# nanleij/ClusteredLowRankSolver.jl

Hardware: AMD Instinct MI355X
Metric: interior-point iterations/sec (higher is better)
Workload: dtype f64x5 (multi-word fp64: 5 limbs per number, ~262 bits; problem data f64x5); 1 GPU; SpherePacking cohnelkies(8,15): d=8, 2d=30; 2 clusters P=32, blocks 16x16 r1 + 1x1 dense, N=31; whole interior-point iterations with the reference's default options at its precision (prec=256 -> 5 limbs), 55 per solve; clusters=2, n_free=31, limbs=5, data_limbs=5, multi_gpu=single GPU

## Files before the change

### clusteredlowranksolver.jl_amd/csrc/clrs_hip.hip

```cpp
#include <hip/hip_runtime.h>

#include <algorithm>
#include <array>
#include <climits>
#include <cmath>
#include <cstdio>
#include <cstdlib>
#include <cstring>
#include <map>
#include <memory>
#include <string>
#include <vector>

#include "../../include/clrs_hip.h"
#include "clrs_kernels.hip.h"
#include "clrs_fused.hip.h"
#include "clrs_assemble_w3.hip.h"
#include "clrs_assemble_w4.hip.h"
#include "clrs_assemble_w5.hip.h"
#include "clrs_solve_small.hip.h"
#include "clrs_factor_small.hip.h"
#include "clrs_ipm.hip.h"

using namespace clrs;
typedef long long i64;

static thread_local std::string g_last_error;
static int fail(int code, const std::string &msg) {
    g_last_error = msg;
    return code;
}
extern "C" void clrs_set_last_error(const char *msg) { g_last_error = msg ? msg : ""; }
#define HIPCHECK(expr)                                                                                   \
    do {                                                                                                 \
        hipError_t e_ = (expr);                                                                          \
        if (e_ != hipSuccess)                                                                            \
            return fail(CLRS_ERR_HIP, std::string(#expr) + ": " + hipGetErrorString(e_));                \
    } while (0)

static const int INFO_NONE = 0x7f7f7f7f;

static int g_cfg_fused_assemble = 1;
static int g_cfg_split_blocks = 1;
static int g_cfg_fused_factor = 1;
static int g_cfg_wave_assemble = 1;
static int g_cfg_wave2_assemble = 1;
static int g_cfg_wave5_assemble = 1;
static int g_cfg_wave4_assemble = 1;
static int g_cfg_wave3_assemble = 1;
static int g_cfg_dense_block = 1;
static int g_cfg_trsm_blockinv = 1;
static int g_cfg_potrf_levels = 1;
static int g_cfg_pairing_tri = 1;
static int g_cfg_factor_aug = 1;
static int g_cfg_dense_wave = 1;
static int g_cfg_factor_small = 1;
static int g_cfg_solve_small_max = 32768;
static int g_cfg_ipm_wmfma = 3;
int g_cfg_mw_stream_words = 1;
int g_cfg_mw_pipeline64 = 1;
int g_cfg_mw_zt_small_maxn = 64;
int g_cfg_modp_minors_chunk_bytes = 0;
int g_cfg_zz_gemm_chunk_bytes = 0;
int g_cfg_liftm_chunk_bytes = 0;
int g_cfg_lrsys_chunk_bytes = 0;
int g_cfg_mw_zi_narrow = 1;
int g_cfg_mw_xinv_product = 1;
int g_cfg_mw_chain_hop = 1;
int g_cfg_mw_y_riders = 1;
int g_cfg_mw_skip_xfb = 1;
int g_cfg_mw_pipeline_x = 1;
int g_cfg_mw_pipeline_x_min = 24;
int g_cfg_mw_sharded_factor_limbs = 1;
int g_cfg_mw_pipeline = 1;
int g_cfg_mw_refine_predictor = 0;
int g_cfg_mw_refine = 1;
int g_cfg_mw_affine_corrector = 1;
int g_cfg_mw_factor_limbs = 0;
int g_cfg_mw_exact_products = 1;
static int g_cfg_solve_small2 = 1;
static const int LDS_BUDGET_DOUBLES = 20000;

enum StepKind { STEP_MEMCPY, STEP_GEMM, STEP_TRSM, STEP_POTRF, STEP_GATHER_S, STEP_GATHER_SCALAR, STEP_SUB, STEP_MEMSET_INFO, STEP_ZERO_UPPER, STEP_FUSED_ASSEMBLE, STEP_SMALL_POTRF, STEP_CLUSTER_FACTOR, STEP_GEMV_T, STEP_CSOLVE_FWD, STEP_Q_SOLVE, STEP_CSOLVE_BWD, STEP_SUM_SLABS, STEP_ASSEMBLE_W1, STEP_GRAM_SMALL, STEP_ASSEMBLE_W2, STEP_SOLVE_SMALL, STEP_DENSE_BLOCK, STEP_ASSEMBLE_W3, STEP_FACTOR_SMALL, STEP_SUM_S_SLABS, STEP_TRTRI32, STEP_DENSE_T32, STEP_TRTRI_DIAG, STEP_COPY2D, STEP_CHOL_LEVEL, STEP_CHOL_PACK, STEP_CHOL_UNPACK, STEP_ASSEMBLE_W4, STEP_ASSEMBLE_W5, STEP_NKINDS };
static const char *const STEP_NAMES[STEP_NKINDS] = {"hipMemcpyAsync(D2D)", "k_gemm_f64_t", "k_trsm_diag", "k_potrf_diag", "k_schur_gather",
                                                    "k_gather_scalar", "k_sub", "hipMemsetAsync", "k_zero_upper", "k_cluster_assemble", "k_small_potrf", "k_cluster_factor", "k_gemv_t",
                                                    "k_cluster_solve_fwd", "k_q_solve", "k_cluster_solve_bwd", "k_sum_slabs", "k_cluster_assemble_w1", "k_gram_small", "k_cluster_assemble_w2", "k_solve_small", "k_dense_block", "k_cluster_assemble_w3", "k_factor_small", "k_sum_S_slabs", "k_trtri32", "k_dense_T32", "k_trtri_diag", "k_copy2d", "k_chol_level", "k_chol_pack", "k_chol_unpack", "k_cluster_assemble_w4", "k_cluster_assemble_w5"};
static const int KT_MAX_EVENTS = 8192;

struct Step {
    StepKind kind;
    int grid = 0;
    void *d0 = nullptr, *d1 = nullptr, *d2 = nullptr;
    void *dst = nullptr;
    const void *src = nullptr;
    size_t bytes = 0;
    i64 n = 0;
    int nmax = 0;
    int aux0 = 0, aux1 = 0;
    bool s_inverse = false;
};

struct Plan {
    std::vector<Step> steps;
    hipGraphExec_t graph = nullptr;
    const void *captured[8] = {nullptr, nullptr, nullptr, nullptr, nullptr, nullptr, nullptr, nullptr};
    int launches() const { return (int)steps.size(); }
};

struct DeviceArena {
    char *base = nullptr;
    size_t size = 0, used = 0;
};

struct TrsmJob {
    const double *L;
    int ldl, n;
    double *B;
    int ldb, nrhs;
};
struct PotrfJob {
    double *A;
    int lda, n, code;
    int stop = 0;
};

struct BlockInfo {
    int j = 0, m = 1, delta = 1, n = 1, kind = 0;
    i64 xyoff = 0, t0 = 0, t1 = 0, d0 = 0, d1 = 0;
    std::vector<int> UR, UL, offR, offL;
    int URt = 0, ULt = 0;
    bool sym = false;
    bool sd_tri = false;
    i64 zr_off = -1, zl_off = -1, ty_off = -1, g_off = -1;
    int cnt = 0;
    i64 w_off = -1, tt_off = -1, sd_off = -1;
    int *d_tptr = nullptr;
    bool fused = false;
};

struct IpmState;

struct clrs_ctx {
    int device = 0;
    int *h_info = nullptr;
    char *pin = nullptr;
    size_t pin_cap = 0, pin_used = 0, pin_demand = 0;
    struct PinOut { void *user; const void *pinned; size_t bytes; };
    std::vector<PinOut> pin_out;
    IpmState *ipm = nullptr;
    std::vector<int> h_term_p, h_dense_p;
    std::vector<double> h_term_lambda;
    int *d_ayL = nullptr, *d_ayR = nullptr;
    hipStream_t stream = nullptr;
    bool own_stream = true;
    int kt_kind = -2;
    std::vector<hipEvent_t> kt_ev;
    std::vector<int> kt_kinds;
    double kt_total[STEP_NKINDS] = {0};
    long long kt_count[STEP_NKINDS] = {0};
    int J = 0, N = 0, NB = 0;
    i64 T = 0, D = 0;
    std::vector<int> P;
    std::vector<i64> coff, Soff;
    i64 xylen = 0, xlen = 0, Slen = 0;
    std::vector<BlockInfo> blk;
    std::vector<void *> allocs;
    std::vector<CholLevelJob> chol_jobs;
    std::map<const double *, std::pair<double *, double *>> s_inv;
    std::vector<std::pair<i64, double *>> trsm_y_pool;
    bool s_inv_valid = false;
    std::vector<CholAugDesc> chol_aug;
    double *d_Xc = nullptr, *d_Y = nullptr;
    double *d_static = nullptr, *d_work = nullptr;
    i64 solve_arena_len = 0;
    double *d_TY = nullptr, *d_G = nullptr, *d_TT = nullptr, *d_Sd = nullptr;
    double *d_S = nullptr, *d_B = nullptr, *d_LB = nullptr, *d_Q = nullptr;
    double *d_t = nullptr, *d_u = nullptr, *d_dy = nullptr, *d_rhsy = nullptr, *d_dx = nullptr, *d_rhsx = nullptr;
    double *d_AY = nullptr;
    i64 *d_ayidx = nullptr;
    int *d_info = nullptr;
    double *d_X = nullptr;
    Plan p_assemble, p_cholS, p_linvB, p_Q, p_cholQ, p_fwd, p_bwd, p_cholX;
    FTables ftables = {};
    W3Tables w3tables = {};
    W4Tables w4tables = {};
    W5Tables w5tables = {};
    CSolve8 solve8 = {};
    struct SolveSmall2 {
        StageJobs jobs = {};
        int rx_job[16] = {0, 0, 0, 0, 0, 0, 0, 0, 0, 0, 0, 0, 0, 0, 0, 0}, ry_job[2] = {-1, -1};
        bool ok = false;
    } ss2[3];
    Plan p_fwd_small, p_bwd_small;
    Plan p_factor_small;
    FSmallArgs fsmall = {};
    StageJobs fsmall_jobs = {};
    const double *bind_X = nullptr, *bind_rhsx = nullptr, *bind_rhsy = nullptr;
    double *bind_Xchol = nullptr, *bind_dx = nullptr, *bind_dy = nullptr;
    double *d_dinvS = nullptr, *d_dinvQ = nullptr, *d_Qslabs = nullptr;
    bool q_slabs = false;
    Plan p_cholQ_slabs, p_solve_all;
    bool fused_fs = false, fused_q = false, fused_x = false, all_assemble_fused = false;
    bool factored = false, assembled = false, local_factored = false;
    bool timing = false, graph_mode = false;
    hipEvent_t ev[10] = {nullptr, nullptr, nullptr, nullptr, nullptr, nullptr, nullptr, nullptr, nullptr, nullptr};
    double times[6] = {0, 0, 0, 0, 0, 0};
    bool times_pending = false, solve_time_pending = false;
    double cnt_bytes = 0, cnt_flops = 0, cnt_factor_flops = 0, cnt_solve_flops = 0;
    std::vector<char> cluster_fused;
    int n_fused_clusters = 0, n_wave_clusters = 0, n_wave2_clusters = 0, n_wave4_clusters = 0, n_wave5_clusters = 0;
    std::vector<int> host_UR, host_UL;
    std::vector<i64> host_U_off;
};

template <class T>
static int upload(clrs_ctx *c, const std::vector<T> &h, T **d) {
    *d = nullptr;
    size_t bytes = std::max<size_t>(h.size(), 1) * sizeof(T);
    HIPCHECK(hipMalloc((void **)d, bytes));
    c->allocs.push_back(*d);
// ... 950 lines not shown
    if (c->N > 0 && (rc = d2h_staged(c, dy, c->d_dy, sizeof(double) * c->N))) return rc;
    return d2h_finish(c);
}

extern "C" int clrs_cholesky_blocks_dev(clrs_ctx *c, const double *d_X, double *d_Xchol) {
    if (!c || !d_X || !d_Xchol) return fail(CLRS_ERR_INVALID, "null argument");
    HIPCHECK(hipSetDevice(c->device));
    if (c->fused_x) {
        c->bind_X = d_X; c->bind_Xchol = d_Xchol;
        return run_plan(c, c->p_cholX);
    }
    if (d_X != c->d_X) HIPCHECK(hipMemcpyAsync(c->d_X, d_X, sizeof(double) * c->xylen, hipMemcpyDeviceToDevice, c->stream));
    int rc = run_plan(c, c->p_cholX);
    if (rc) return rc;
    if (d_Xchol != c->d_X) HIPCHECK(hipMemcpyAsync(d_Xchol, c->d_X, sizeof(double) * c->xylen, hipMemcpyDeviceToDevice, c->stream));
    return 0;
}

extern "C" int clrs_cholesky_blocks(clrs_ctx *c, const double *X, double *Xchol) {
    if (!c || !X || !Xchol) return fail(CLRS_ERR_INVALID, "null argument");
    HIPCHECK(hipSetDevice(c->device));
    int rc;
    pin_reset(c);
    if ((rc = h2d_staged(c, c->d_X, X, sizeof(double) * c->xylen))) return rc;
    if ((rc = clrs_cholesky_blocks_dev(c, c->d_X, c->d_X))) return rc;
    if ((rc = d2h_staged(c, Xchol, c->d_X, sizeof(double) * c->xylen))) return rc;
    int st = 0;
    if ((rc = read_info(c, &st, 1))) return rc;
    if ((rc = d2h_finish(c))) return rc;
    return st;
}

extern "C" double *clrs_q_buffer_dev(clrs_ctx *c) { return c ? c->d_Q : nullptr; }
extern "C" double *clrs_u_buffer_dev(clrs_ctx *c) { return c ? c->d_u : nullptr; }
extern "C" double *clrs_S_buffer_dev(clrs_ctx *c) { return c ? c->d_S : nullptr; }
extern "C" double *clrs_AY_buffer_dev(clrs_ctx *c) { return c ? c->d_AY : nullptr; }
extern "C" void *clrs_stream(clrs_ctx *c) { return c ? (void *)c->stream : nullptr; }

extern "C" int clrs_set_timing(clrs_ctx *c, int enabled) {
    if (!c) return fail(CLRS_ERR_INVALID, "null argument");
    c->timing = enabled != 0;
    return 0;
}
extern "C" int clrs_get_timings(clrs_ctx *c, double t[6]) {
    if (!c || !t) return fail(CLRS_ERR_INVALID, "null argument");
    HIPCHECK(hipStreamSynchronize(c->stream));
    collect_times(c);
    for (int i = 0; i < 6; i++) t[i] = c->times[i];
    return 0;
}
extern "C" int clrs_get_counters(const clrs_ctx *c, double *ab, double *af, double *ff, double *sf) {
    if (!c) return fail(CLRS_ERR_INVALID, "null argument");
    if (ab) *ab = c->cnt_bytes;
    if (af) *af = c->cnt_flops;
    if (ff) *ff = c->cnt_factor_flops;
    if (sf) *sf = c->cnt_solve_flops;
    return 0;
}
extern "C" int clrs_set_graph_mode(clrs_ctx *c, int enabled) {
    if (!c) return fail(CLRS_ERR_INVALID, "null argument");
    c->graph_mode = enabled != 0;
    return 0;
}
extern "C" int clrs_plan_info(const clrs_ctx *c, int32_t *na, int32_t *nf, int32_t *ns) {
    if (!c) return fail(CLRS_ERR_INVALID, "null argument");
    if (na) *na = c->p_assemble.launches();
    if (nf) *nf = c->p_cholS.launches() + c->p_linvB.launches() + c->p_Q.launches() + c->p_cholQ.launches();
    if (ns) *ns = c->p_fwd.launches() + c->p_bwd.launches();
    return 0;
}

extern "C" int clrs_set_stream(clrs_ctx *c, void *stream) {
    if (!c) return fail(CLRS_ERR_INVALID, "null argument");
    HIPCHECK(hipSetDevice(c->device));
    HIPCHECK(hipStreamSynchronize(c->stream));
    Plan *plans[] = {&c->p_assemble, &c->p_cholS, &c->p_linvB, &c->p_Q, &c->p_cholQ, &c->p_fwd, &c->p_bwd, &c->p_cholX, &c->p_cholQ_slabs, &c->p_solve_all, &c->p_fwd_small, &c->p_bwd_small, &c->p_factor_small};
    for (Plan *p : plans)
        if (p->graph) { hipGraphExecDestroy(p->graph); p->graph = nullptr; }
    if (c->own_stream) HIPCHECK(hipStreamDestroy(c->stream));
    c->stream = (hipStream_t)stream;
    c->own_stream = false;
    return 0;
}

static int kt_collect(clrs_ctx *c) {
    if (c->kt_kinds.empty()) return 0;
    HIPCHECK(hipStreamSynchronize(c->stream));
    for (size_t i = 0; i < c->kt_kinds.size(); i++) {
        float ms = 0;
        if (hipEventElapsedTime(&ms, c->kt_ev[2 * i], c->kt_ev[2 * i + 1]) == hipSuccess) {
            c->kt_total[c->kt_kinds[i]] += ms * 1e-3;
            c->kt_count[c->kt_kinds[i]]++;
        }
    }
    c->kt_kinds.clear();
    return 0;
}

extern "C" int clrs_set_kernel_timing(clrs_ctx *c, int kind) {
    if (!c || kind < -2 || kind >= STEP_NKINDS) return fail(CLRS_ERR_INVALID, "bad kernel kind");
    int rc = kt_collect(c);
    if (rc) return rc;
    c->kt_kind = kind;
    for (int k = 0; k < STEP_NKINDS; k++) { c->kt_total[k] = 0; c->kt_count[k] = 0; }
    return 0;
}

extern "C" int clrs_get_kernel_times(clrs_ctx *c, int max_kinds, double *seconds, int64_t *launches) {
    if (!c || !seconds || !launches) return fail(CLRS_ERR_INVALID, "null argument");
    int rc = kt_collect(c);
    if (rc) return rc;
    for (int k = 0; k < max_kinds && k < STEP_NKINDS; k++) { seconds[k] = c->kt_total[k]; launches[k] = c->kt_count[k]; }
    return STEP_NKINDS;
}

extern "C" int clrs_config_set(const char *key, int value) {
    if (!key) return fail(CLRS_ERR_INVALID, "null argument");
    if (!std::strcmp(key, "fused_assemble")) { g_cfg_fused_assemble = value; return 0; }
    if (!std::strcmp(key, "split_blocks")) { g_cfg_split_blocks = value; return 0; }
    if (!std::strcmp(key, "fused_factor")) { g_cfg_fused_factor = value; return 0; }
    if (!std::strcmp(key, "wave_assemble")) { g_cfg_wave_assemble = value; return 0; }
    if (!std::strcmp(key, "wave2_assemble")) { g_cfg_wave2_assemble = value; return 0; }
    if (!std::strcmp(key, "wave3_assemble")) { g_cfg_wave3_assemble = value; return 0; }
    if (!std::strcmp(key, "wave4_assemble")) { g_cfg_wave4_assemble = value; return 0; }
    if (!std::strcmp(key, "wave5_assemble")) { g_cfg_wave5_assemble = value; return 0; }
    if (!std::strcmp(key, "dense_block")) { g_cfg_dense_block = value; return 0; }
    if (!std::strcmp(key, "dense_wave")) { g_cfg_dense_wave = value; return 0; }
    if (!std::strcmp(key, "factor_aug")) { g_cfg_factor_aug = value; return 0; }
    if (!std::strcmp(key, "pairing_tri")) { g_cfg_pairing_tri = value; return 0; }
    if (!std::strcmp(key, "potrf_levels")) { g_cfg_potrf_levels = value; return 0; }
    if (!std::strcmp(key, "trsm_blockinv")) { g_cfg_trsm_blockinv = value; return 0; }
    if (!std::strcmp(key, "solve_small2")) { g_cfg_solve_small2 = value; return 0; }
    if (!std::strcmp(key, "factor_small")) { g_cfg_factor_small = value; return 0; }
    if (!std::strcmp(key, "pin_limit")) { PIN_LIMIT = (size_t)std::max(value, 0); return 0; }
    if (!std::strcmp(key, "ipm_wmfma")) { g_cfg_ipm_wmfma = value; return 0; }
    if (!std::strcmp(key, "solve_small_max")) { g_cfg_solve_small_max = value; return 0; }
    if (!std::strcmp(key, "mw_exact_products")) { g_cfg_mw_exact_products = value; return 0; }
    if (!std::strcmp(key, "mw_refine")) { g_cfg_mw_refine = value; return 0; }
    if (!std::strcmp(key, "mw_factor_limbs")) { g_cfg_mw_factor_limbs = value; return 0; }
    if (!std::strcmp(key, "mw_affine_corrector")) { g_cfg_mw_affine_corrector = value; return 0; }
    if (!std::strcmp(key, "mw_pipeline")) { g_cfg_mw_pipeline = value; return 0; }
    if (!std::strcmp(key, "mw_pipeline64")) { g_cfg_mw_pipeline64 = value; return 0; }
    if (!std::strcmp(key, "mw_zt_small_maxn")) { g_cfg_mw_zt_small_maxn = value; return 0; }
    if (!std::strcmp(key, "mw_pipeline_x")) { g_cfg_mw_pipeline_x = value; return 0; }
    if (!std::strcmp(key, "mw_pipeline_x_min")) { g_cfg_mw_pipeline_x_min = value; return 0; }
    if (!std::strcmp(key, "mw_sharded_factor_limbs")) { g_cfg_mw_sharded_factor_limbs = value; return 0; }
    if (!std::strcmp(key, "mw_stream_words")) { g_cfg_mw_stream_words = value; return 0; }
    if (!std::strcmp(key, "mw_zi_narrow")) { g_cfg_mw_zi_narrow = value; return 0; }
    if (!std::strcmp(key, "modp_minors_chunk_bytes")) { g_cfg_modp_minors_chunk_bytes = value < 0 ? 0 : value; return 0; }
    if (!std::strcmp(key, "zz_gemm_chunk_bytes")) { g_cfg_zz_gemm_chunk_bytes = value < 0 ? 0 : value; return 0; }
    if (!std::strcmp(key, "liftm_chunk_bytes")) { g_cfg_liftm_chunk_bytes = value < 0 ? 0 : value; return 0; }
    if (!std::strcmp(key, "lrsys_chunk_bytes")) { g_cfg_lrsys_chunk_bytes = value < 0 ? 0 : value; return 0; }
    if (!std::strcmp(key, "mw_xinv_product")) { g_cfg_mw_xinv_product = value; return 0; }
    if (!std::strcmp(key, "mw_chain_hop")) { g_cfg_mw_chain_hop = value; return 0; }
    if (!std::strcmp(key, "mw_skip_xfb")) { g_cfg_mw_skip_xfb = value; return 0; }
    if (!std::strcmp(key, "mw_y_riders")) { g_cfg_mw_y_riders = value; return 0; }
    if (!std::strcmp(key, "mw_refine_predictor")) { g_cfg_mw_refine_predictor = value; return 0; }
    return fail(CLRS_ERR_INVALID, std::string("unknown configuration key ") + key);
}

#ifdef CLRS_W3_STAMPS
extern "C" int clrs_debug_cf_stamps(clrs_ctx *c, uint64_t out[16]) {
    if (!c || !out) return fail(CLRS_ERR_INVALID, "null argument");
    HIPCHECK(hipStreamSynchronize(c->stream));
    HIPCHECK(hipMemcpyFromSymbol(out, HIP_SYMBOL(g_cf_stamps), 16 * sizeof(uint64_t)));
    return 0;
}
extern "C" int clrs_debug_ss2_stamps(clrs_ctx *c, uint64_t out[16]) {
    if (!c || !out) return fail(CLRS_ERR_INVALID, "null argument");
    HIPCHECK(hipStreamSynchronize(c->stream));
    HIPCHECK(hipMemcpyFromSymbol(out, HIP_SYMBOL(g_ss2_stamps), 16 * sizeof(uint64_t)));
    return 0;
}
extern "C" int clrs_debug_w3_stamps(clrs_ctx *c, uint64_t out[16]) {
    if (!c || !out) return fail(CLRS_ERR_INVALID, "null argument");
    HIPCHECK(hipStreamSynchronize(c->stream));
    HIPCHECK(hipMemcpyFromSymbol(out, HIP_SYMBOL(g_w3_stamps), 16 * sizeof(uint64_t)));
    return 0;
}
#endif

extern "C" int clrs_debug_stamps(clrs_ctx *c, uint64_t out[64]) {
    if (!c || !out) return fail(CLRS_ERR_INVALID, "null argument");
    if (!c->ftables.stamps) { std::memset(out, 0, 64 * sizeof(uint64_t)); return 0; }
    HIPCHECK(hipStreamSynchronize(c->stream));
    HIPCHECK(hipMemcpy(out, c->ftables.stamps, 64 * sizeof(uint64_t), hipMemcpyDeviceToHost));
    return 0;
}

extern "C" int clrs_fused_clusters(const clrs_ctx *c) { return c ? c->n_fused_clusters : 0; }
extern "C" int clrs_wave_clusters(const clrs_ctx *c) { return c ? c->n_wave_clusters + c->n_wave2_clusters : 0; }
extern "C" int clrs_wave2_clusters(const clrs_ctx *c) { return c ? c->n_wave2_clusters : 0; }
extern "C" int clrs_wave4_clusters(const clrs_ctx *c) { return c ? c->n_wave4_clusters : 0; }
extern "C" int clrs_wave5_clusters(const clrs_ctx *c) { return c ? c->n_wave5_clusters : 0; }

extern "C" const char *clrs_kernel_name(int kind) { return (kind >= 0 && kind < STEP_NKINDS) ? STEP_NAMES[kind] : ""; }

extern "C" const char *clrs_strerror(int code) {
    switch (code) {
        case CLRS_OK: return "ok";
        case CLRS_ERR_INVALID: return "invalid argument or malformed SDP description";
        case CLRS_ERR_HIP: return "HIP runtime error";
        case CLRS_ERR_NO_DEVICE: return "no usable HIP device";
        case CLRS_ERR_STATE: return "call order violated";
        default: return code > 0 ? "factorisation failure (non-positive pivot)" : "unknown error";
    }
}
extern "C" const char *clrs_last_error(void) { return g_last_error.c_str(); }
extern "C" const char *clrs_version(void) { return "clrs-hip 0.1.0 (gfx950)"; }

#include "clrs_ipm_host.inc"

static CtxOwner mini_ctx(int device) {
    CtxOwner c(new clrs_ctx(), clrs_ctx_destroy);
    c->device = device;
    if (hipSetDevice(device) != hipSuccess || hipStreamCreateWithFlags(&c->stream, hipStreamNonBlocking) != hipSuccess) c.reset();
    if (!c) return c;
    (void)hipFuncSetAttribute((const void *)k_gemm_f64_t<128, 128, 0, 0>, hipFuncAttributeMaxDynamicSharedMemorySize, (int)gemm_lds_bytes(128, 128));
    (void)hipFuncSetAttribute((const void *)k_gemm_f64_t<128, 128, 0, 1>, hipFuncAttributeMaxDynamicSharedMemorySize, (int)gemm_lds_bytes(128, 128));
    (void)hipFuncSetAttribute((const void *)k_gemm_f64_t<128, 128, 1, 0>, hipFuncAttributeMaxDynamicSharedMemorySize, (int)gemm_lds_bytes(128, 128));
    (void)hipFuncSetAttribute((const void *)k_gemm_f64_t<128, 128, 1, 1>, hipFuncAttributeMaxDynamicSharedMemorySize, (int)gemm_lds_bytes(128, 128));
    std::vector<int> hi(1, INFO_NONE);
    if (upload(c.get(), hi, &c->d_info)) c.reset();
    return c;
}

extern "C" int clrs_test_gemm(int device, int ta, int tb, int M, int N, int K, double alpha, const double *A, int lda, const double *B,
                              int ldb, double beta, double *C, int ldc) {
    const CtxOwner own = mini_ctx(device);
    clrs_ctx *c = own.get();
    if (!c) return fail(CLRS_ERR_NO_DEVICE, "no device");
    int rc = 0;
    i64 na = (i64)lda * (ta ? M : K), nb = (i64)ldb * (tb ? K : N), nc = (i64)ldc * N;
    std::vector<double> hA(A, A + na), hB(B, B + nb), hC(C, C + nc);
    double *dA, *dB, *dC;
    if ((rc = upload(c, hA, &dA)) || (rc = upload(c, hB, &dB)) || (rc = upload(c, hC, &dC))) return rc;
    Plan pl;
    std::vector<GemmDesc> g;
    g.push_back(mk_gemm(ta, tb, M, N, K, alpha, dA, lda, dB, ldb, beta, dC, ldc));
    if (!(rc = add_gemm_stage(c, pl, g)) && !(rc = run_steps(c, pl))) {
        if (hipStreamSynchronize(c->stream) != hipSuccess || hipMemcpy(C, dC, sizeof(double) * nc, hipMemcpyDeviceToHost) != hipSuccess)
            rc = fail(CLRS_ERR_HIP, "copy back failed");
    }
    return rc;
}

extern "C" int clrs_test_potrf(int device, int n, double *A, int lda) {
    const CtxOwner own = mini_ctx(device);
    clrs_ctx *c = own.get();
    if (!c) return fail(CLRS_ERR_NO_DEVICE, "no device");
    int rc = 0, st = 0;
    std::vector<double> hA(A, A + (i64)lda * n);
    double *dA;
    if ((rc = upload(c, hA, &dA))) return rc;
    Plan pl;
    std::vector<PotrfJob> pj;
    pj.push_back(PotrfJob{dA, lda, n, 1});
    if (!(rc = plan_potrf(c, pl, pj)) && !(rc = run_steps(c, pl)) && !(rc = read_info(c, &st))) {
        if (hipMemcpy(A, dA, sizeof(double) * (i64)lda * n, hipMemcpyDeviceToHost) != hipSuccess) rc = fail(CLRS_ERR_HIP, "copy back failed");
    }
    return rc ? rc : st;
}

typedef double v2d_stream __attribute__((ext_vector_type(2)));
__global__ __launch_bounds__(256) void k_stream_probe(const v2d_stream *__restrict__ a, const v2d_stream *__restrict__ b, v2d_stream *__restrict__ w,
                                                      long long nr, long long nw) {
    const long long stride = (long long)gridDim.x * 256, n = nr > nw ? nr : nw;
    for (long long i = (long long)blockIdx.x * 256 + threadIdx.x; i < n; i += 4 * stride) {
        v2d_stream x[4], y[4];
#pragma unroll
        for (int u = 0; u < 4; u++) {
            const long long k = i + u * stride;
            x[u] = y[u] = (v2d_stream){0.0, 0.0};
            if (k < nr) { x[u] = a[k]; y[u] = b[k]; }
        }
#pragma unroll
        for (int u = 0; u < 4; u++) {
            const long long k = i + u * stride;
            if (k < nw) __builtin_nontemporal_store(x[u] + y[u], w + k);
        }
    }
}

extern "C" int clrs_test_stream(int device, long long read_bytes, long long write_bytes, int reps, double *avg_us) {
    if (read_bytes < 32 || write_bytes < 16 || reps < 1 || !avg_us) return fail(CLRS_ERR_INVALID, "clrs_test_stream: bad arguments");
    if (hipSetDevice(device) != hipSuccess) return fail(CLRS_ERR_NO_DEVICE, "no device");
    const long long nr = read_bytes / 32, nw = write_bytes / 16;
    v2d_stream *a = nullptr, *b = nullptr, *w = nullptr;
    hipEvent_t e0 = nullptr, e1 = nullptr;
    hipStream_t st = nullptr;
    int rc = 0;
    auto ok = [&](hipError_t e, const char *what) { if (e != hipSuccess && !rc) rc = fail(CLRS_ERR_HIP, std::string(what) + ": " + hipGetErrorString(e)); return e == hipSuccess; };
    if (ok(hipMalloc(&a, nr * 16), "hipMalloc") && ok(hipMalloc(&b, nr * 16), "hipMalloc") && ok(hipMalloc(&w, nw * 16), "hipMalloc") &&
        ok(hipMemset(a, 0, nr * 16), "hipMemset") && ok(hipMemset(b, 0, nr * 16), "hipMemset") && ok(hipMemset(w, 0, nw * 16), "hipMemset") &&
        ok(hipStreamSynchronize(nullptr), "hipStreamSynchronize") &&
        ok(hipStreamCreateWithFlags(&st, hipStreamNonBlocking), "hipStreamCreate") && ok(hipEventCreate(&e0), "hipEventCreate") && ok(hipEventCreate(&e1), "hipEventCreate")) {
        hipDeviceProp_t prop;
        int cus = 256;
        if (hipGetDeviceProperties(&prop, device) == hipSuccess) cus = prop.multiProcessorCount;
        const int grid = 2 * cus;
        for (int r = 0; r < 3; r++) hipLaunchKernelGGL(k_stream_probe, dim3(grid), dim3(256), 0, st, a, b, w, nr, nw);
        ok(hipEventRecord(e0, st), "hipEventRecord");
        for (int r = 0; r < reps; r++) hipLaunchKernelGGL(k_stream_probe, dim3(grid), dim3(256), 0, st, a, b, w, nr, nw);
        ok(hipEventRecord(e1, st), "hipEventRecord");
        ok(hipEventSynchronize(e1), "hipEventSynchronize");
        float ms = 0.f;
// ... 29 lines not shown
```

### clusteredlowranksolver.jl_amd/csrc/clrs_mw.hip

```cpp
#include <hip/hip_runtime.h>

#include <dlfcn.h>

#include <algorithm>
#include <condition_variable>
#include <cstdio>
#include <cstring>
#include <memory>
#include <mutex>
#include <string>
#include <vector>

#include "../../include/clrs_hip.h"
#include "clrs_mw_kernels.hip.h"
#include "clrs_mw_pipe.hip.h"
#include "clrs_mw_exact.hip.h"
#include "clrs_mw_ipm.hip.h"
#include "clrs_mw_rank.hip.h"
#include "clrs_mw_gemm.hip.h"
#include "clrs_mw_kernel_vectors.hip.h"
#include "clrs_mw_rational.hip.h"
#include "clrs_mw_inst.h"
#include "clrs_mw_tables.h"
#ifdef MW_SPLIT_UNITS
MW_KERNELS_ALL(extern template, 4)
MW_KERNELS_ALL(extern template, 5)
MW_KERNELS_ALL(extern template, 6)
MW_KERNELS_ALL(extern template, 8)
MW_KERNELS_ALL(extern template, 10)
#endif

typedef long long i64;

extern int g_cfg_mw_zi_narrow;
extern int g_cfg_mw_xinv_product;
extern int g_cfg_mw_chain_hop, g_cfg_mw_skip_xfb, g_cfg_mw_y_riders;
extern int g_cfg_mw_stream_words;
extern int g_cfg_mw_pipeline64;
extern int g_cfg_mw_zt_small_maxn;
extern int g_cfg_mw_pipeline_x, g_cfg_mw_pipeline_x_min;
extern int g_cfg_mw_sharded_factor_limbs;
extern int g_cfg_mw_pipeline;
extern int g_cfg_mw_refine_predictor;
extern int g_cfg_mw_refine;
extern int g_cfg_mw_exact_products;
extern int g_cfg_mw_affine_corrector;
extern int g_cfg_mw_factor_limbs;
extern "C" void clrs_set_last_error(const char *msg);

static int mw_fail(int code, const std::string &msg) {
    clrs_set_last_error(msg.c_str());
    return code;
}
#define MWCHECK(expr)                                                                                    \
    do {                                                                                                 \
        hipError_t e_ = (expr);                                                                          \
        if (e_ != hipSuccess) return mw_fail(CLRS_ERR_HIP, std::string(#expr) + ": " + hipGetErrorString(e_)); \
    } while (0)

typedef struct { char internal[128]; } mw_nccl_id;
struct MwNccl {
    void *lib = nullptr;
    int (*GetUniqueId)(mw_nccl_id *) = nullptr;
    int (*CommInitRank)(void **, int, mw_nccl_id, int) = nullptr;
    int (*CommDestroy)(void *) = nullptr;
    int (*AllGather)(const void *, void *, size_t, int, void *, hipStream_t) = nullptr;
    const char *(*GetErrorString)(int) = nullptr;
};
static MwNccl g_nccl;
static int mw_nccl_load() {
    if (g_nccl.lib) return 0;
    const char *names[] = {"librccl.so.1", "librccl.so", "/opt/rocm/lib/librccl.so.1"};
    void *h = nullptr;
    for (const char *n : names) if ((h = dlopen(n, RTLD_NOW | RTLD_NOLOAD))) break;
    for (const char *n : names) { if (h) break; h = dlopen(n, RTLD_NOW | RTLD_GLOBAL); }
    if (!h) return mw_fail(CLRS_ERR_INVALID, std::string("RCCL is not available: ") + dlerror());
    g_nccl.GetUniqueId = (int (*)(mw_nccl_id *))dlsym(h, "ncclGetUniqueId");
    g_nccl.CommInitRank = (int (*)(void **, int, mw_nccl_id, int))dlsym(h, "ncclCommInitRank");
    g_nccl.CommDestroy = (int (*)(void *))dlsym(h, "ncclCommDestroy");
    g_nccl.AllGather = (int (*)(const void *, void *, size_t, int, void *, hipStream_t))dlsym(h, "ncclAllGather");
    g_nccl.GetErrorString = (const char *(*)(int))dlsym(h, "ncclGetErrorString");
    if (!g_nccl.GetUniqueId || !g_nccl.CommInitRank || !g_nccl.CommDestroy || !g_nccl.AllGather) return mw_fail(CLRS_ERR_INVALID, "RCCL symbols missing");
    g_nccl.lib = h;
    return 0;
}
#define NCCLCHECK(expr)                                                                                                          \
    do {                                                                                                                         \
        int r_ = (expr);                                                                                                         \
        if (r_ != 0) return mw_fail(CLRS_ERR_HIP, std::string(#expr) + ": " + (g_nccl.GetErrorString ? g_nccl.GetErrorString(r_) : "RCCL error")); \
    } while (0)
static const int MW_NCCL_FLOAT64 = 8;

struct clrs_mw_local_group {
    int world = 0;
    int attached = 0;
    std::mutex m;
    std::condition_variable cv;
    struct Chan {
        int arrived = 0;
        long gen = 0;
        std::vector<double *> base;
        std::vector<hipEvent_t> ready, copied;
    } ch[2];
    void barrier(int k) {
        std::unique_lock<std::mutex> lk(m);
        Chan &c = ch[k];
        const long g = c.gen;
        if (++c.arrived == world) { c.arrived = 0; c.gen++; cv.notify_all(); }
        else cv.wait(lk, [&] { return c.gen != g; });
    }
};

static const size_t MW_LDS_MAX = 160 * 1024 - 2048;

struct clrs_mw_ctx {
    int device = 0, K = 4, DK = 1;
    hipStream_t stream = nullptr;
    bool own_stream = true;
    MwDev d = {};
    std::vector<MwBlk> blk;
    std::vector<MwClu> clu;
    std::vector<void *> allocs;
    int maxU = 0, maxP = 0, maxn = 0, maxn_dense = 0;
    bool all_inv = false;
    bool xinv_valid = false;
    bool lds_x = false, lds_q = false, lds_zt_L = false, dense_two = false;
    int nw_factor = 1;
    int maxcnt = 0;
    double *vz = nullptr;
    bool wide_solve = false;
    const double *ride_fwd = nullptr;
    const int *ride_wait = nullptr;
    int ride_wait_value = 0;
    bool fwd_rode = false;
    int n_one_term = 0, n_many_term = 0;
    int sa_lanes = MW_SA_W;
    int maxTb = 0;
    size_t sm_x = 0, sm_zt = 0, sm_dense = 0, sm_factor = 0, sm_q = 0, sm_fwd = 0, sm_mid = 0, sm_bwd = 0;
    int *h_info = nullptr;
    double *d_Xin = nullptr, *d_Xc = nullptr, *d_Y = nullptr, *d_rx = nullptr, *d_ry = nullptr, *d_dx = nullptr, *d_dy = nullptr;
    bool assembled = false, factored = false;
    bool timing = false;
    hipEvent_t ev[8] = {nullptr, nullptr, nullptr, nullptr, nullptr, nullptr, nullptr, nullptr};
    double times[6] = {0, 0, 0, 0, 0, 0};
    double cnt_mul = 0;
    double cnt_factor = 0, cnt_solve = 0;
    struct MwIpm *ipm = nullptr;
    size_t sm_bp_diag = 0, sm_bp_panel = 0, sm_bp_inv = 0;
    std::vector<MwBp> bp_S, bp_Q;
    const MwBp *d_bp = nullptr;
    bool any_lds_cluster = false;
    void *comm = nullptr;
    void *comm_side = nullptr;
    clrs_mw_local_group *lgroup = nullptr;
    bool local_factored = false, fwd_done = false;
    const double *split_rhs_x = nullptr;
    bool refine_ready = false;
    MwdDev mwd = {};
    int mwd_blocks = 0, mwd_tasks = 0;
    size_t sm_mwd = 0;
    MwxDev mwx = {};
    int mwx_blocks = 0, mwx_maxU16 = 0;
    MwsDev mws = {};
    int mws_blocks = 0;
    int mws_turns = 1;
    size_t sm_mws = 0;
    bool pipe_bp = false;
    bool pipe_S64 = false;
    bool pipe_X = false;
    unsigned long long *pipe_pcx = nullptr;
    double *xpipe_L = nullptr, *xpipe_rd = nullptr;
    int *xpipe_info = nullptr;
    bool pipe_S = false, pipe_Q = false;
    unsigned long long *pipe_pc64 = nullptr;
    int pipe_pcQ = 0;
    unsigned pipe_epoch = 0;
    bool stream_words = true;
    bool y_riders = true;
    const double *ride_y = nullptr;
    bool zi_narrow = true;
    bool xinv_product = true;
    int chain_hop = 1;
    bool refine_skip_next = false;
    int refine_predictor = 0;
    int refine = 1;
    bool ipm_arms_info = false;
    int kf_low = 0, kf_entry = 0;
};

template <class T>
static int mw_upload(clrs_mw_ctx *c, const std::vector<T> &h, const T **d) {
    T *p = nullptr;
    size_t bytes = std::max<size_t>(h.size(), 1) * sizeof(T);
    MWCHECK(hipMalloc((void **)&p, bytes));
    c->allocs.push_back(p);
    if (!h.empty()) MWCHECK(hipMemcpy(p, h.data(), h.size() * sizeof(T), hipMemcpyHostToDevice));
    *d = p;
    return 0;
}
static int mw_dmalloc(clrs_mw_ctx *c, double **d, i64 n) {
    size_t bytes = (size_t)std::max<i64>(n, 1) * sizeof(double);
    MWCHECK(hipMalloc((void **)d, bytes));
    c->allocs.push_back(*d);
    MWCHECK(hipMemset(*d, 0, bytes));
    return 0;
}

#define MW_CASE(Kc, Dc, ...) if (c_K_ == Kc && c_D_ == Dc) { constexpr int KK = Kc; constexpr int DD = Dc; __VA_ARGS__; } else
#define MW_DISPATCH(ctx, ...)                                                                                       \
    do {                                                                                                            \
        const int c_K_ = (ctx)->K, c_D_ = (ctx)->DK;                                                                \
        MW_CASE(2, 1, __VA_ARGS__) MW_CASE(2, 2, __VA_ARGS__) MW_CASE(3, 1, __VA_ARGS__) MW_CASE(3, 2, __VA_ARGS__)  \
        MW_CASE(4, 1, __VA_ARGS__) MW_CASE(4, 2, __VA_ARGS__) MW_CASE(5, 1, __VA_ARGS__) MW_CASE(5, 2, __VA_ARGS__)  \
        MW_CASE(6, 1, __VA_ARGS__) MW_CASE(6, 2, __VA_ARGS__) MW_CASE(8, 1, __VA_ARGS__) MW_CASE(8, 2, __VA_ARGS__)  \
        MW_CASE(10, 1, __VA_ARGS__) MW_CASE(10, 2, __VA_ARGS__)                                                      \
        MW_CASE(3, 3, __VA_ARGS__) MW_CASE(4, 4, __VA_ARGS__) MW_CASE(5, 5, __VA_ARGS__) MW_CASE(6, 6, __VA_ARGS__)  \
        MW_CASE(8, 8, __VA_ARGS__) MW_CASE(10, 10, __VA_ARGS__)                                                      \
        return mw_fail(CLRS_ERR_INVALID, "limbs must be 2..6, 8 or 10 and data limbs 1, 2 or the limbs");           \
    } while (0)

template <class F>
static int mw_set_lds(F kernel, size_t bytes) {
    if (bytes > 48 * 1024) MWCHECK(hipFuncSetAttribute((const void *)kernel, hipFuncAttributeMaxDynamicSharedMemorySize, (int)bytes));
    return 0;
}

extern "C" void clrs_mw_destroy(clrs_mw_ctx *c);
static void mw_ipm_free(clrs_mw_ctx *c);
static int mw_launch_xrd(clrs_mw_ctx *c, const double *d_Xc);

extern "C" int clrs_mw_create_opts(const clrs_sdp_desc *d, int data_limbs, int device, int limbs, const clrs_mw_options *opts, clrs_mw_ctx **out);
extern "C" int clrs_mw_create(const clrs_sdp_desc *d, int device, int limbs, clrs_mw_ctx **out) {
    return clrs_mw_create_opts(d, 1, device, limbs, nullptr, out);
}
extern "C" int clrs_mw_create_ex(const clrs_sdp_desc *d, int data_limbs, int device, int limbs, clrs_mw_ctx **out) {
    return clrs_mw_create_opts(d, data_limbs, device, limbs, nullptr, out);
}

#define MW_RET(call) do { if (int rc_ = (call)) return rc_; } while (0)
static int mw_hip(hipError_t e, const char *what) {
    return e == hipSuccess ? 0 : mw_fail(CLRS_ERR_HIP, std::string(what) + ": " + hipGetErrorString(e));
}
template <class T>
static int mw_alloc_fill(clrs_mw_ctx *c, T **p, size_t count, int byte) {
    if (hipMalloc((void **)p, count * sizeof(T)) != hipSuccess) return mw_fail(CLRS_ERR_HIP, "hipMalloc failed");
    c->allocs.push_back(*p);
    if (hipMemset(*p, byte, count * sizeof(T)) != hipSuccess) return mw_fail(CLRS_ERR_HIP, "hipMemset failed");
    return 0;
}

struct MwOpts { int exact, refine, pipe, refine_pred, factor_limbs, km; };
static int mw_resolve_opts(const clrs_mw_options *opts, int limbs, int data_limbs, MwOpts &o) {
    o.exact = opts && opts->exact_products >= 0 ? opts->exact_products : g_cfg_mw_exact_products;
    o.refine = opts && opts->refine >= 0 ? opts->refine : g_cfg_mw_refine;
    o.pipe = opts && opts->pipeline >= 0 ? opts->pipeline : g_cfg_mw_pipeline;
    o.refine_pred = opts && opts->refine_predictor >= 0 ? opts->refine_predictor : g_cfg_mw_refine_predictor;
    o.factor_limbs = opts && opts->factor_limbs >= 0 ? opts->factor_limbs : g_cfg_mw_factor_limbs;
    o.km = opts && opts->matmul_limbs > 0 ? opts->matmul_limbs : limbs;
    if (o.km > limbs) o.km = limbs;
    while (o.km < limbs && !mw_km_ok(limbs, o.km)) o.km++;
    if (data_limbs > 2) o.exact = 0;
    if (o.km < limbs) o.exact = 0;
    if (o.exact > 2 || o.refine > 2) return mw_fail(CLRS_ERR_INVALID, "clrs_mw_options: exact_products and refine are 0, 1 or 2 (or < 0 for the default)");
    if (limbs < 2 || limbs > 10 || limbs == 7 || limbs == 9) return mw_fail(CLRS_ERR_INVALID, "limbs must be 2..6, 8 or 10");
    if (data_limbs < 1 || data_limbs > limbs || (data_limbs > 2 && data_limbs != limbs))
        return mw_fail(CLRS_ERR_INVALID, "data limbs must be 1, 2 or the context's limbs (the problem data at the working precision: src/interface.jl:1078-1112)");
    return 0;
}

static int mw_stage_stream(clrs_mw_ctx *c) {
    {
        int least = 0, greatest = 0;
        if (hipDeviceGetStreamPriorityRange(&least, &greatest) != hipSuccess) { least = greatest = 0; (void)hipGetLastError(); }
        if (hipStreamCreateWithPriority(&c->stream, hipStreamNonBlocking, greatest) != hipSuccess) return mw_fail(CLRS_ERR_HIP, "hipStreamCreateWithPriority failed");
    }
    if (hipHostMalloc((void **)&c->h_info, 2 * sizeof(int), hipHostMallocDefault) != hipSuccess) return mw_fail(CLRS_ERR_HIP, "hipHostMalloc failed");
    return 0;
}

static void mw_adopt_tables(clrs_mw_ctx *c, MwTables &t) {
    c->blk.swap(t.blk); c->clu.swap(t.clu);
    c->maxU = t.maxU; c->maxP = t.maxP; c->maxn = t.maxn; c->maxn_dense = t.maxn_dense; c->maxTb = t.maxTb; c->maxcnt = t.maxcnt;
    c->sa_lanes = t.sa_lanes; c->n_one_term = t.n_one_term; c->n_many_term = t.n_many_term;
    c->cnt_mul = t.cnt_mul; c->cnt_factor = t.cnt_factor; c->cnt_solve = t.cnt_solve;
    c->wide_solve = c->maxP > 64 || t.N > 64;
}

static int mw_stage_lds(clrs_mw_ctx *c, const MwTables &t) {
    const int K = c->K, J = t.J, N = t.N;
    const size_t lim = MW_LDS_MAX / sizeof(double);
    {
        size_t nn = (size_t)c->maxn * c->maxn * K;
        size_t bcw = MW_POTRF_SCR(K, (size_t)c->maxn);
        c->lds_x = nn + bcw <= lim;
        size_t xneed = (c->lds_x ? nn : 0) + bcw;
        for (auto &k : c->blk) {
            const size_t one = (size_t)k.n * k.n * K + MW_POTRF_SCR(K, (size_t)k.n) + (size_t)K * k.n;
            const size_t two = one + (size_t)MW_TRI(k.n) * K;
            k.inv = !c->lds_x ? 0 : two <= lim ? 1 : one <= lim ? 2 : 0;
            if (k.inv) xneed = std::max(xneed, k.inv == 1 ? two : one);
        }
        c->all_inv = !c->blk.empty();
        for (auto &k : c->blk) c->all_inv = c->all_inv && (k.kind != 0 || k.inv != 0);
        c->sm_x = xneed * 8;
        size_t zt = (size_t)c->maxn * MW_CT * K;
        c->lds_zt_L = zt + nn <= lim;
        c->sm_zt = (zt + (c->lds_zt_L ? nn : 0)) * 8;
        if (zt > lim) return mw_fail(CLRS_ERR_INVALID, "PSD block too large for the multi-word kernels");
        size_t maxnd = 0;
        for (auto &k : c->blk) if (k.kind != 0 && k.n > 1) maxnd = std::max(maxnd, (size_t)k.n);
        if (maxnd * maxnd * K > lim) return mw_fail(CLRS_ERR_INVALID, "dense block too large for the multi-word kernels");
        c->dense_two = 2 * maxnd * maxnd * K <= lim;
        c->sm_dense = (c->dense_two ? 2 : 1) * maxnd * maxnd * K * 8;
        size_t fmax = 0;
        for (auto &q : c->clu) {
            const size_t need = ((size_t)q.P * q.P + (size_t)MW_TRI(q.P)) * K + MW_POTRF_SCR(K, (size_t)q.P);
            q.lds = need <= lim ? 1 : 0;
            if (q.lds) fmax = std::max(fmax, need);
        }
        c->sm_factor = std::max<size_t>(fmax, 1) * 8;
        c->nw_factor = std::max(1, std::min(MW_INV_WG, 256 / std::max(J, 1)));
        c->sm_fwd = 2 * (size_t)c->maxP * K * 8;
        c->sm_bwd = 3 * (size_t)c->maxP * K * 8;
        const size_t qn = (size_t)N * N * K;
        const size_t qneed = qn + (size_t)MW_TRI(N) * K + MW_POTRF_SCR(K, (size_t)N);
        c->lds_q = qneed <= lim;
        c->sm_q = (c->lds_q ? qneed : 1) * 8;
        c->sm_mid = 2 * (size_t)std::max(N, 1) * K * 8;
        if (c->sm_fwd > MW_LDS_MAX || c->sm_mid > MW_LDS_MAX) return mw_fail(CLRS_ERR_INVALID, "cluster too large for the multi-word solve kernels");
    }
    MW_DISPATCH(c, {
        MW_RET(mw_set_lds(k_mw_potrf_x<KK>, c->sm_x)); MW_RET(mw_set_lds((k_mw_potrf_x_ride<KK, DD>), c->sm_x)); MW_RET(mw_set_lds(k_mw_zt<KK, DD>, c->sm_zt)); MW_RET(mw_set_lds((k_mw_dense_t<KK, DD>), c->sm_dense));
        constexpr int KC = mw_kc(KK);
        const size_t bw = std::min(c->sm_mid + c->sm_bwd, MW_LDS_MAX);
// ... 7 lines not shown

template <class DATA, class PUT>
static void mw_cut_column(int n, int DK, int S, DATA &&data, int *e_out, PUT &&put) {
    double mx = 0;
    for (int i = 0; i < n; i++) mx = std::max(mx, std::fabs(data(0, i)));
    const int e = *e_out = mwk::mws_exponent(mx);
    for (int i = 0; i < n; i++)
        mw_cut_digits(data(0, i), DK > 1 ? data(1, i) : 0.0, e, S, [&](int s, float dgt) { put(i, s, dgt); });
}

static int mw_stage_mws(clrs_mw_ctx *c, const MwTables &t, const MwOpts &o, std::vector<long long> &mws_off) {
    const int K = c->K, DK = c->DK, NB = t.NB;
    mws_off.assign((size_t)std::max(NB, 1), -1);
    const int S = mws_slices(K);
    std::vector<float> hVs;
    std::vector<int> hVe, hve_off((size_t)std::max(NB, 1), 0), hsv((size_t)std::max(NB, 1), 0);
    for (int b = 0; b < NB; b++) {
        const MwBlk &k = c->blk[b];
        if (k.kind != 0 || !k.inv || k.n > 32) continue;
        const int n = k.n, U = k.U, np = (n + 3) & ~3, n16 = (n + 15) & ~15, U16 = (U + 15) & ~15, rV = mws_rowstride(U16);
        if ((n16 / 16) * (U16 / 16) > 4 || mws_lds_bytes(S, mws_sv_class(S, 1), n, U) > MW_LDS_MAX) continue;
        if (2 * (n16 / 16) * (U16 / 16) > 4) c->mws_turns = 2;
        mws_off[b] = (long long)hVs.size();
        hve_off[b] = (int)hVe.size();
        hVs.resize(hVs.size() + (size_t)S * np * rV, 0.0f);
        hVe.resize(hVe.size() + U16, 0);
        float *dst = hVs.data() + mws_off[b];
        int sv = 0;
        for (int u = 0; u < U; u++)
            mw_cut_column(n, DK, S, [&](int l, int i) { return t.V[(size_t)l * t.Vp + k.v_off + (i64)u * n + i]; }, &hVe[hve_off[b] + u], [&](int i, int s, float dgt) {
                dst[(size_t)s * np * rV + (size_t)i * rV + mws_col(i, u, U16)] = dgt;
                if (dgt != 0.0f) sv = std::max(sv, s + 1);
            });
        if (mws_lds_bytes(S, mws_sv_class(S, sv), n, U) > MW_LDS_MAX) {
            hVs.resize((size_t)mws_off[b]); hVe.resize((size_t)hve_off[b]);
            mws_off[b] = -1;
            continue;
        }
        hsv[b] = sv;
        c->mws_blocks++;
        c->sm_mws = std::max(c->sm_mws, mws_lds_bytes(S, mws_sv_class(S, sv), n, U));
    }
    const bool on = o.exact == 2 ? c->mws_blocks > 0 : (o.exact == 1 && c->mws_blocks >= 256);
    if (!on) { c->mws_blocks = 0; std::fill(mws_off.begin(), mws_off.end(), -1); }
    else {
        MW_RET(mw_upload(c, hVs, &c->mws.Vs)); MW_RET(mw_upload(c, hVe, &c->mws.Vexp));
        MW_RET(mw_upload(c, hve_off, &c->mws.ve_off)); MW_RET(mw_upload(c, hsv, &c->mws.sv));
        MW_DISPATCH(c, { if constexpr (DD <= 2) { MW_RET(mw_set_lds((k_mws_pair<KK, DD, 1>), c->sm_mws)); MW_RET(mw_set_lds((k_mws_pair<KK, DD, 2>), c->sm_mws)); } });
    }
    return mw_upload(c, mws_off, &c->mws.vs_off);
}

static int mw_stage_mwx(clrs_mw_ctx *c, const MwTables &t, const MwOpts &o, const std::vector<long long> &mws_off) {
    const int K = c->K, DK = c->DK, NB = t.NB;
    std::vector<long long> mwx_off((size_t)std::max(NB, 1), -1);
    if (o.exact == 0) return mw_upload(c, mwx_off, &c->mwx.d_off);
    const int S = mws_slices(K);
    std::vector<float> hVd;
    std::vector<int> heV, he_off((size_t)std::max(NB, 1), 0), hsv((size_t)std::max(NB, 1), 0);
    for (int b = 0; b < NB; b++) {
        const MwBlk &k = c->blk[b];
        if (k.kind != 0 || k.m != 1 || mws_off[b] >= 0) continue;
        if (k.U < (o.exact == 2 ? 16 : 64) || k.n < 8) continue;
        const int n = k.n, U = k.U, np = (n + 3) & ~3, U16 = (U + 15) & ~15;
        mwx_off[b] = (long long)hVd.size();
        he_off[b] = (int)heV.size();
        hVd.resize(hVd.size() + (size_t)S * np * U16, 0.0f);
        heV.resize(heV.size() + U16, 0);
        float *dst = hVd.data() + mwx_off[b];
        int sv = 0;
        for (int u = 0; u < U; u++)
            mw_cut_column(n, DK, S, [&](int l, int i) { return t.V[(size_t)l * t.Vp + k.v_off + (i64)u * n + i]; }, &heV[he_off[b] + u], [&](int i, int s, float dgt) {
                dst[(size_t)s * np * U16 + (size_t)i * U16 + u] = dgt;
                if (dgt != 0.0f) sv = std::max(sv, s + 1);
            });
        hsv[b] = sv;
        c->mwx_blocks++;
        c->mwx_maxU16 = std::max(c->mwx_maxU16, U16);
    }
    if (c->mwx_blocks > 0) {
        MW_RET(mw_upload(c, hVd, &c->mwx.Vd)); MW_RET(mw_upload(c, heV, &c->mwx.eV));
        MW_RET(mw_upload(c, he_off, &c->mwx.e_off)); MW_RET(mw_upload(c, hsv, &c->mwx.sv));
        double *zd = nullptr, *td = nullptr, *ez = nullptr, *et = nullptr;
        MW_RET(mw_dmalloc(c, &zd, (i64)(hVd.size() + 1) / 2)); MW_RET(mw_dmalloc(c, &td, (i64)(hVd.size() + 1) / 2));
        MW_RET(mw_dmalloc(c, &ez, (i64)(heV.size() + 1) / 2)); MW_RET(mw_dmalloc(c, &et, (i64)(heV.size() + 1) / 2));
        c->mwx.Zd = (float *)zd; c->mwx.Td = (float *)td; c->mwx.eZ = (int *)ez; c->mwx.eT = (int *)et;
        MW_RET(mw_hip(hipMemset(zd, 0, hVd.size() * sizeof(float)), "hipMemset")); MW_RET(mw_hip(hipMemset(td, 0, hVd.size() * sizeof(float)), "hipMemset"));
        MW_RET(mw_hip(hipMemset(ez, 0, heV.size() * sizeof(int)), "hipMemset")); MW_RET(mw_hip(hipMemset(et, 0, heV.size() * sizeof(int)), "hipMemset"));
    }
    return mw_upload(c, mwx_off, &c->mwx.d_off);
}

static int mw_stage_mwd(clrs_mw_ctx *c, const MwTables &t, const MwOpts &o) {
    const int K = c->K, DK = c->DK, NB = t.NB;
    std::vector<long long> mwd_off((size_t)std::max(NB, 1), -1);
    if (o.exact == 0 || K > 6) return mw_upload(c, mwd_off, &c->mwd.a_off);
    const int S = mws_slices(K), S1 = (S + 1) / 2, sN = 32 * 32;
    std::vector<float> hAd;
    std::vector<int> heA, he_off((size_t)std::max(NB, 1), 0);
    for (int b = 0; b < NB; b++) {
        const MwBlk &k = c->blk[b];
        if (k.kind == 0 || !k.inv || k.n <= 16 || k.n > 32 || k.cnt <= 0) continue;
        const int n = k.n;
        const size_t base = hAd.size(), ebase = heA.size();
        hAd.resize(base + (size_t)k.cnt * S1 * sN, 0.0f);
        heA.resize(ebase + (size_t)k.cnt * 32, 0);
        bool fits = true;
        for (int e = 0; e < k.cnt && fits; e++) {
            float *dst = hAd.data() + base + (size_t)e * S1 * sN;
            const i64 a0 = k.a_off + (i64)e * n * n;
            for (int col = 0; col < n; col++)
                mw_cut_column(n, DK, S, [&](int l, int kk) { return t.dA[(size_t)l * t.dAp + a0 + kk + (i64)col * n]; }, &heA[ebase + (size_t)e * 32 + col], [&](int kk, int s, float dgt) {
                    if (s < S1) dst[(size_t)s * sN + (size_t)kk * 32 + mws_col(kk, col, 32)] = dgt;
                    else if (dgt != 0.0f) fits = false;
                });
        }
        if (!fits) { hAd.resize(base); heA.resize(ebase); continue; }
        mwd_off[b] = (long long)base;
        he_off[b] = (int)ebase;
        c->mwd_blocks++;
    }
    if (c->mwd_blocks > 0) {
        std::vector<int> tasks;
        for (size_t di = 0; di < t.dn_list.size(); di++) {
            const int b = t.dn_list[di];
            if (mwd_off[b] < 0) continue;
            for (int e = 0; e < c->blk[b].cnt; e++) { tasks.push_back((int)di); tasks.push_back(e); }
        }
        c->mwd_tasks = (int)tasks.size() / 2;
        MW_RET(mw_upload(c, tasks, &c->mwd.tasks));
        MW_RET(mw_upload(c, hAd, &c->mwd.Ad)); MW_RET(mw_upload(c, heA, &c->mwd.eA)); MW_RET(mw_upload(c, he_off, &c->mwd.e_off));
        c->sm_mwd = (size_t)2 * S * sN * sizeof(float) + 128 * sizeof(int);
        MW_DISPATCH(c, { if constexpr (DD <= 2) { MW_RET(mw_set_lds((k_mwx_dense<KK, DD>), c->sm_mwd)); } });
    }
    return mw_upload(c, mwd_off, &c->mwd.a_off);
}

static int mw_stage_upload(clrs_mw_ctx *c, const MwTables &t) {
    MwDev &q = c->d;
    q.mws_off = c->mws.vs_off; q.mws_on = c->mws_blocks > 0 ? 1 : 0;
    q.mwx_off = c->mwx.d_off; q.mwx_on = c->mwx_blocks > 0 ? 1 : 0;
    q.mwd_off = c->mwd.a_off; q.mwd_on = 0;
    q.J = t.J; q.N = t.N; q.NB = t.NB; q.nlr = (int)t.lr_list.size(); q.ndn = (int)t.dn_list.size();
    q.xylen = t.xylen; q.xlen = t.xlen; q.Slen = t.Slen; q.T = t.T; q.xrdlen = t.xrdlen;
    q.zlen = std::max<i64>(t.zlen, 1); q.glen = std::max<i64>(t.glen, 1); q.wlen = std::max<i64>(t.wlen, 1); q.sdlen = std::max<i64>(t.sdlen, 1);
    q.Vp = t.Vp; q.dAp = t.dAp; q.lamp = t.lamp; q.Bp = t.Bp;
    MW_RET(mw_upload(c, c->blk, &q.blk)); MW_RET(mw_upload(c, c->clu, &q.clu));
    MW_RET(mw_upload(c, t.lr_list, &q.lr_list)); MW_RET(mw_upload(c, t.dn_list, &q.dn_list));
    MW_RET(mw_upload(c, t.V, &q.V)); MW_RET(mw_upload(c, t.vrow, &q.vrow));
    MW_RET(mw_upload(c, t.st_a, &q.st_a)); MW_RET(mw_upload(c, t.st_b, &q.st_b)); MW_RET(mw_upload(c, t.st_lam, &q.st_lam));
    MW_RET(mw_upload(c, t.tptr, &q.tptr));
    MW_RET(mw_upload(c, t.st_orig, &q.st_orig)); MW_RET(mw_upload(c, t.st_p, &q.st_p)); MW_RET(mw_upload(c, t.st_war, &q.st_war)); MW_RET(mw_upload(c, t.st_wac, &q.st_wac));
    MW_RET(mw_upload(c, t.st_trl, &q.st_trl)); MW_RET(mw_upload(c, t.st_trd, &q.st_trd)); MW_RET(mw_upload(c, t.st_flag, &q.st_flag));
    MW_RET(mw_upload(c, t.ay_a, &q.ay_a)); MW_RET(mw_upload(c, t.ay_b, &q.ay_b)); MW_RET(mw_upload(c, t.ay_blk, &q.ay_blk));
    MW_RET(mw_upload(c, t.dA, &q.dA)); MW_RET(mw_upload(c, t.dmap, &q.dmap)); MW_RET(mw_upload(c, t.dense_p, &q.dense_p));
    MW_RET(mw_upload(c, t.drow_ptr, &q.drow_ptr)); MW_RET(mw_upload(c, t.drow_blk, &q.drow_blk)); MW_RET(mw_upload(c, t.drow_en, &q.drow_en));
    q.dn_big = t.dn_big;
    q.maxcnt = c->maxcnt;
    return mw_upload(c, t.B, &q.B);
}

static int mw_stage_buffers(clrs_mw_ctx *c) {
    MwDev &q = c->d;
    const int K = c->K, J = q.J, N = q.N;
    const i64 xlen = q.xlen, Slen = q.Slen, xyoff = q.xylen, rdoff = q.xrdlen, T = q.T;
    MW_RET(mw_dmalloc(c, &q.Z, q.zlen * K)); MW_RET(mw_dmalloc(c, &q.Tm, q.zlen * K));
    MW_RET(mw_dmalloc(c, &q.GX, q.glen * K)); MW_RET(mw_dmalloc(c, &q.GY, q.glen * K));
    MW_RET(mw_dmalloc(c, &q.W, q.wlen * K)); MW_RET(mw_dmalloc(c, &q.Sd, q.sdlen * K));
    MW_RET(mw_dmalloc(c, &q.S, Slen * K)); MW_RET(mw_dmalloc(c, &q.LB, xlen * (i64)N * K)); MW_RET(mw_dmalloc(c, &q.Q, (i64)N * N * K));
    MW_RET(mw_dmalloc(c, &q.Si, Slen * K)); MW_RET(mw_dmalloc(c, &q.Qi, (i64)N * N * K));

    MW_RET(mw_dmalloc(c, &q.Xf, xyoff * K)); MW_RET(mw_dmalloc(c, &q.Xb, xyoff * K)); MW_RET(mw_dmalloc(c, &q.Xi, xyoff * K));
    MW_RET(mw_dmalloc(c, &q.xrd, rdoff * K)); MW_RET(mw_dmalloc(c, &q.srd, xlen * K)); MW_RET(mw_dmalloc(c, &q.qrd, (i64)N * K));
    MW_RET(mw_dmalloc(c, &q.t, xlen * K)); MW_RET(mw_dmalloc(c, &q.u, (i64)J * N * K)); MW_RET(mw_dmalloc(c, &q.AY, T * K));
    q.AX = nullptr;
    q.aff_mu = q.aff_rhs = q.aff_t = q.aff_u = nullptr; q.aff_wait = nullptr; q.ride2_rhs = nullptr; q.ride2_t = q.ride2_u = nullptr;
    MW_RET(mw_dmalloc(c, &c->vz, 2 * (i64)N * K));
    MW_RET(mw_dmalloc(c, &q.S0, Slen * K)); MW_RET(mw_dmalloc(c, &q.ub, (i64)J * N * K));
    MW_RET(mw_dmalloc(c, &q.rx2, xlen * K)); MW_RET(mw_dmalloc(c, &q.dx2, xlen * K));
    MW_RET(mw_dmalloc(c, &q.u2, (i64)N * K)); MW_RET(mw_dmalloc(c, &q.dy2, (i64)N * K));
    q.uadd = nullptr;
    MW_RET(mw_dmalloc(c, &c->d_Xin, xyoff * K)); MW_RET(mw_dmalloc(c, &c->d_Xc, xyoff * K)); MW_RET(mw_dmalloc(c, &c->d_Y, xyoff * K));
    MW_RET(mw_dmalloc(c, &c->d_rx, xlen * K)); MW_RET(mw_dmalloc(c, &c->d_dx, xlen * K));
    MW_RET(mw_dmalloc(c, &c->d_ry, (i64)N * K)); MW_RET(mw_dmalloc(c, &c->d_dy, (i64)N * K));
    int *info = nullptr;
    MW_RET(mw_hip(hipMalloc((void **)&info, 2 * sizeof(int)), "hipMalloc"));
    c->allocs.push_back(info);
    q.info = info;
    int init[2] = {MW_INFO_NONE, MW_INFO_NONE};
    MW_RET(mw_hip(hipMemcpy(info, init, sizeof(init), hipMemcpyHostToDevice), "hipMemcpy"));
    return mw_alloc_fill(c, &q.pcnt, (size_t)(2 * J + 3), 0);
}

static int mw_stage_blocked(clrs_mw_ctx *c) {
    MwDev &q = c->d;
    const int K = c->K, J = q.J, N = q.N;
    for (int j = 0; j < J; j++) {
        const MwClu &cl = c->clu[j];
        if (cl.lds) { c->any_lds_cluster = true; continue; }
        c->bp_S.push_back(MwBp{q.S + cl.Soff, q.Si + cl.Soff, q.srd + cl.coff, q.Slen, q.xlen, cl.P, cl.P, j + 1, 0, (int)c->bp_S.size(), 0});
    }
    if (N > 0) c->bp_Q.push_back(MwBp{q.Q, q.Qi, q.qrd, (i64)N * N, (i64)N, N, N, J + 1, 0, (int)c->bp_S.size(), 0});
    std::vector<MwBp> all = c->bp_S;
    all.insert(all.end(), c->bp_Q.begin(), c->bp_Q.end());
    MW_RET(mw_upload(c, all, &c->d_bp));
    const int MW_PB = MW_PB_OF(K);
    c->sm_bp_diag = ((size_t)MW_POTRF_SCR(K, MW_PB) + (size_t)K * MW_PB * MW_PB + (size_t)K * MW_TRI(MW_PB) + (size_t)K * MW_PB) * 8;
    c->sm_bp_panel = (size_t)K * MW_BP_PR * MW_PB * 8;
    c->sm_bp_inv = (size_t)K * MW_PB * MW_BP_IC * 8;
    MW_DISPATCH(c, { MW_RET(mw_set_lds(k_mw_bp_diag<KK>, std::max(c->sm_bp_diag, c->sm_factor))); MW_RET(mw_set_lds(k_mw_bp_panel<KK>, c->sm_bp_panel)); MW_RET(mw_set_lds(k_mw_bp_inv<KK>, c->sm_bp_inv)); MW_RET(mw_set_lds(k_mw_bp_inv_row<KK>, c->sm_bp_inv)); });
    return 0;
}

static int mw_stage_pipelines(clrs_mw_ctx *c, const MwOpts &o) {
    MwDev &q = c->d;
    const int K = c->K, J = q.J, N = q.N, cfg_pipe = o.pipe;
    bool small = c->maxP <= MWP_N;
    for (auto &cl : c->clu) small = small && cl.lds;
    c->pipe_S = cfg_pipe != 0 && (K <= 6 || cfg_pipe >= 2) && small && (i64)J * ((MWP_N / MWP_W) + MWP_WW) <= 256;
    c->pipe_Q = (cfg_pipe >= 2 || (cfg_pipe == 1 && K <= 6 && N > MWP_W)) && N > 0 && N <= MWP_N;
    bool lds_all = !c->clu.empty();
    for (auto &cl : c->clu) lds_all = lds_all && cl.lds;
    c->pipe_S64 = cfg_pipe != 0 && K <= 6 && lds_all && c->maxP > MWP_N && c->maxP <= MWP_N64 && (i64)J * 16 <= 256 && g_cfg_mw_pipeline64 != 0 &&
                  (cfg_pipe >= 2 || c->maxP >= 48);
    const size_t nbp = c->bp_S.size() + c->bp_Q.size();
    const bool any_bp = !c->bp_S.empty() || (N > 0 && !c->lds_q);
    c->pipe_bp = cfg_pipe != 0 && any_bp && (i64)std::max<size_t>(c->bp_S.size(), 1) * ((MWP_N / MWP_W) + MWP_WW) <= 256;
    q.pipe_pc = nullptr;
    q.pipe_stamps = nullptr;
    q.pipe_bp = 0;
    {
        bool all_inv = c->d.NB > 0 && c->lds_x;
        int maxn_x = 0;
        i64 working = 0;
        for (auto &kb : c->blk) {
            all_inv = all_inv && kb.inv == 1;
            maxn_x = std::max(maxn_x, kb.n);
            working += 2 * ((kb.n + MWP_W - 1) / MWP_W + (kb.n > MWP_N ? MWP_N64 / MWP_W : MWP_WW));
        }
        q.no_xfb = (all_inv && (!q.dn_big || c->dense_two) && g_cfg_mw_skip_xfb != 0) ? 1 : 0;
        c->pipe_X = cfg_pipe != 0 && K <= 6 && all_inv && maxn_x <= MWP_N64 && g_cfg_mw_pipeline_x != 0 &&
                    (cfg_pipe >= 2 || (maxn_x >= g_cfg_mw_pipeline_x_min && working <= 256));
        if (c->pipe_X) {
            double *pcx = nullptr, *ti = nullptr;
            MW_RET(mw_dmalloc(c, &pcx, (i64)2 * c->d.NB * MWP_PC_WORDS_N(K, MWP_N64)));
            c->pipe_pcx = (unsigned long long *)pcx;
            MW_RET(mw_dmalloc(c, &c->xpipe_L, c->d.xylen * K));
            MW_RET(mw_dmalloc(c, &c->xpipe_rd, c->d.xrdlen * K));
            MW_RET(mw_dmalloc(c, &ti, c->d.NB + 1));
            c->xpipe_info = (int *)ti;
            MW_DISPATCH(c, { if constexpr (KK <= 6) { MW_RET(mw_set_lds(k_mw_potrf_x_pipe<KK>, MWP_LDS_ALONE64)); } });
        }
    }
    if (c->pipe_S64) {
        MW_RET(mw_alloc_fill(c, &c->pipe_pc64, (size_t)J * MWP_PC_WORDS_N(K, MWP_N64), 0xff));
        MW_DISPATCH(c, { if constexpr (KK <= 6) { MW_RET(mw_set_lds(k_mw_factor_pipe64<KK>, MWP_LDS_ALONE64)); } });
    }
    if (c->pipe_S || c->pipe_Q || c->pipe_bp) {
        const size_t own = (size_t)(c->pipe_S ? J : 0) + 1;
        MW_RET(mw_alloc_fill(c, &q.pipe_pc, (own + (c->pipe_bp ? nbp : 0)) * MWP_PC_WORDS(K), 0xff));
        c->pipe_pcQ = c->pipe_S ? J : 0;
        q.pipe_q = c->pipe_pcQ;
        q.pipe_bp = (int)own;
        MW_DISPATCH(c, {
            MW_RET(mw_set_lds(k_mw_factor_pipe<KK>, MWP_LDS_ALONE));
            MW_RET(mw_set_lds(k_mw_potrf_q_pipe<KK>, std::max<size_t>(MWP_LDS_ALONE, c->sm_fwd)));
            MW_RET(mw_set_lds(k_mw_bp_diag_pipe<KK>, std::max<size_t>(MWP_LDS_ALONE, c->sm_factor)));
        });
    }
    return 0;
}

static int mw_stage_reduced_limbs(clrs_mw_ctx *c, const MwOpts &o) {
    MwDev &q = c->d;
    const int K = c->K, N = q.N;
    q.rank = 0; q.world = 1; q.gathered = 0;
    MW_RET(mw_dmalloc(c, &q.Qg, (i64)N * N * K)); MW_RET(mw_dmalloc(c, &q.ug, (i64)N * K));
    const bool may = mw_kf_of(K) < K && c->refine == 1;
    c->kf_low = may ? mw_kf_of(K) : K;
    if (o.factor_limbs != 0 && o.factor_limbs != K && o.factor_limbs != c->kf_low) return mw_fail(CLRS_ERR_INVALID, "factor_limbs: 0 (automatic), the context's limbs, or the reduced count of this limb count where the LDS-resident refined solve runs");
    if (o.factor_limbs == K) c->kf_low = K;
    c->kf_entry = o.factor_limbs == 0 ? K : o.factor_limbs;
    q.kf = c->kf_entry;
    q.km = o.km;
    return mw_alloc_fill(c, &q.refstat, 4, 0);
}

extern "C" int clrs_mw_create_opts(const clrs_sdp_desc *d, int data_limbs, int device, int limbs, const clrs_mw_options *opts, clrs_mw_ctx **out) {
    if (!d || !out) return mw_fail(CLRS_ERR_INVALID, "null argument");
    MwOpts o;
    MW_RET(mw_resolve_opts(opts, limbs, data_limbs, o));
    *out = nullptr;
    int ndev = 0;
    if (hipGetDeviceCount(&ndev) != hipSuccess || ndev <= 0 || device >= ndev) return mw_fail(CLRS_ERR_NO_DEVICE, "no usable HIP device");
    MW_RET(mw_hip(hipSetDevice(device), "hipSetDevice(device)"));
    if (d->n_clusters <= 0 || d->n_free < 0 || d->n_blocks < 0) return mw_fail(CLRS_ERR_INVALID, "bad sizes");
    std::unique_ptr<clrs_mw_ctx, void (*)(clrs_mw_ctx *)> guard(new clrs_mw_ctx(), clrs_mw_destroy);
    clrs_mw_ctx *c = guard.get();
    c->device = device;
    c->K = limbs;
    c->DK = data_limbs;
    c->refine = o.refine;
    c->refine_predictor = o.refine_pred;
    {
        const char *e = std::getenv("CLRS_MW_STREAM_WORDS");
        c->stream_words = e && *e ? std::atoi(e) != 0 : g_cfg_mw_stream_words != 0;
        c->chain_hop = std::min(std::max(g_cfg_mw_chain_hop, 0), 2);
        c->y_riders = g_cfg_mw_y_riders != 0;
        c->zi_narrow = g_cfg_mw_zi_narrow != 0;
        c->xinv_product = g_cfg_mw_xinv_product != 0;
    }
    MW_RET(mw_stage_stream(c));
    MwTables t;
    std::string err;
    if (mw_build_tables(d, data_limbs, t, err)) return mw_fail(CLRS_ERR_INVALID, err);
    mw_adopt_tables(c, t);
    MW_RET(mw_stage_lds(c, t));
    std::vector<long long> mws_off;
    MW_RET(mw_stage_mws(c, t, o, mws_off));
    MW_RET(mw_stage_mwx(c, t, o, mws_off));
    MW_RET(mw_stage_mwd(c, t, o));
    MW_RET(mw_stage_upload(c, t));
    MW_RET(mw_stage_buffers(c));
    MW_RET(mw_stage_blocked(c));
    MW_RET(mw_stage_pipelines(c, o));
    MW_RET(mw_stage_reduced_limbs(c, o));
    for (auto &e : c->ev) MW_RET(mw_hip(hipEventCreate(&e), "hipEventCreate(&e)"));
    *out = guard.release();
    return 0;
}
#undef MW_RET

extern "C" void clrs_mw_destroy(clrs_mw_ctx *c) {
    if (!c) return;
    (void)hipSetDevice(c->device);
    if (c->stream) (void)hipStreamSynchronize(c->stream);
    mw_ipm_free(c);
    if (c->comm && g_nccl.CommDestroy) { (void)g_nccl.CommDestroy(c->comm); c->comm = nullptr; }
    if (c->comm_side && g_nccl.CommDestroy) { (void)g_nccl.CommDestroy(c->comm_side); c->comm_side = nullptr; }
    if (c->lgroup) { std::lock_guard<std::mutex> lk(c->lgroup->m); c->lgroup->attached--; c->lgroup = nullptr; }
    for (void *p : c->allocs) (void)hipFree(p);
    for (auto &e : c->ev) if (e) (void)hipEventDestroy(e);
    if (c->h_info) (void)hipHostFree(c->h_info);
    if (c->stream && c->own_stream) (void)hipStreamDestroy(c->stream);
    delete c;
}

extern "C" int clrs_mw_limbs(const clrs_mw_ctx *c) { return c ? c->K : 0; }
extern "C" void *clrs_mw_stream(clrs_mw_ctx *c) { return c ? (void *)c->stream : nullptr; }
extern "C" int clrs_mw_set_stream(clrs_mw_ctx *c, void *stream) {
    if (!c) return mw_fail(CLRS_ERR_INVALID, "null context");
    if (c->own_stream && c->stream) { (void)hipStreamSynchronize(c->stream); (void)hipStreamDestroy(c->stream); }
    c->stream = (hipStream_t)stream;
    c->own_stream = false;
    return 0;
}
extern "C" int clrs_mw_get_dims(const clrs_mw_ctx *c, clrs_dims *o) {
    if (!c || !o) return mw_fail(CLRS_ERR_INVALID, "null argument");
    o->xy_len = c->d.xylen; o->x_len = c->d.xlen; o->S_len = c->d.Slen; o->n_terms = c->d.T;
    o->n_free = c->d.N; o->n_clusters = c->d.J; o->n_blocks = c->d.NB; o->reserved = c->K;
    return 0;
}
extern "C" int clrs_mw_get_unique_count(const clrs_mw_ctx *c, int32_t block, int32_t *n_unique) {
    if (!c || !n_unique || block < 0 || block >= c->d.NB) return mw_fail(CLRS_ERR_INVALID, "bad argument");
    *n_unique = c->blk[block].U;
    return 0;
}
extern "C" int clrs_mw_set_timing(clrs_mw_ctx *c, int on) {
    if (!c) return mw_fail(CLRS_ERR_INVALID, "null context");
    c->timing = on != 0;
    return 0;
}
extern "C" int clrs_mw_get_counters(const clrs_mw_ctx *c, double *assemble_muladds, double *factor_muladds, double *solve_muladds) {
    if (!c) return mw_fail(CLRS_ERR_INVALID, "null context");
    if (assemble_muladds) *assemble_muladds = c->cnt_mul;
    if (factor_muladds) *factor_muladds = c->cnt_factor;
    if (solve_muladds) *solve_muladds = c->cnt_solve;
    return 0;
}

static bool mw_zt_small(const clrs_mw_ctx *c) { return c->all_inv && (i64)c->d.nlr * c->maxU <= 2048 && c->maxn <= g_cfg_mw_zt_small_maxn; }
static bool mw_y_riders_ok(const clrs_mw_ctx *c) {
    return c->y_riders && mw_zt_small(c) && c->d.nlr > 0 && c->mws_blocks == 0 && c->mwx_blocks == 0 && !c->pipe_X && !c->d.gathered && c->d.world <= 1;
}
static int mw_reset_info(clrs_mw_ctx *c, int which) {
    if (c->ipm_arms_info) return 0;
    MWCHECK(hipMemsetAsync(c->d.info + which, 0x7f, sizeof(int), c->stream));
    return 0;
}
static int mw_read_info(clrs_mw_ctx *c, int which, int *status) {
    MWCHECK(hipMemcpyAsync(c->h_info + which, c->d.info + which, sizeof(int), hipMemcpyDeviceToHost, c->stream));
    MWCHECK(hipStreamSynchronize(c->stream));
    *status = c->h_info[which] == MW_INFO_NONE ? 0 : c->h_info[which];
    return 0;
}

static int mw_cholesky_blocks_dev2(clrs_mw_ctx *c, const double *d_X, double *d_Xchol, const double *d_Y2, double *d_Yi, int *d_yfail) {
    if (!c || !d_X || !d_Xchol) return mw_fail(CLRS_ERR_INVALID, "null argument");
    MWCHECK(hipSetDevice(c->device));
    int rc;
    if ((rc = mw_reset_info(c, 1))) return rc;
    if (c->d.NB == 0) return 0;
    const int grid = d_Y2 ? 2 * c->d.NB : c->d.NB;
    bool in_mem = false;
    for (auto &k : c->blk) in_mem = in_mem || k.inv == 2 || mw_x_shares(k);
    if (c->pipe_X) {
        c->pipe_epoch = (c->pipe_epoch + 1) & 0x3ffffff;
        MW_DISPATCH(c, { if constexpr (KK <= 6) { hipLaunchKernelGGL(k_mw_potrf_x_pipe<KK>, dim3(mwp_blocks64(grid)), dim3(MWP_NT64), MWP_LDS_ALONE64, c->stream, c->d, d_X, d_Xchol, d_Y2, d_Yi, d_yfail,
                                                                     c->xpipe_L, c->xpipe_rd, c->xpipe_info, c->pipe_pcx, c->pipe_epoch); } });
    } else if (c->ride_y && mw_y_riders_ok(c)) {
        const int ntile = (c->maxU + 1) / 2;
        MW_DISPATCH(c, hipLaunchKernelGGL((k_mw_potrf_x_ride<KK, DD>), dim3(grid + c->d.nlr * ntile, in_mem && c->lds_x ? MW_INV_WG : 1), dim3(MW_PT), c->sm_x, c->stream, c->d, d_X, d_Xchol,
                                          c->lds_x ? 1 : 0, d_Y2, d_Yi, d_yfail, c->ride_y, grid, ntile));
    } else
    MW_DISPATCH(c, hipLaunchKernelGGL(k_mw_potrf_x<KK>, dim3(grid, in_mem && c->lds_x ? MW_INV_WG : 1), dim3(MW_PT), c->sm_x, c->stream, c->d, d_X, d_Xchol, c->lds_x ? 1 : 0, d_Y2, d_Yi, d_yfail));
    MWCHECK(hipGetLastError());
    c->xinv_valid = true;
    return 0;
}
extern "C" int clrs_mw_cholesky_blocks_dev(clrs_mw_ctx *c, const double *d_X, double *d_Xchol) { return mw_cholesky_blocks_dev2(c, d_X, d_Xchol, nullptr, nullptr, nullptr); }
extern "C" int clrs_mw_sync_status_cholesky(clrs_mw_ctx *c) {
    if (!c) return mw_fail(CLRS_ERR_INVALID, "null context");
    int st = 0, rc;
    if ((rc = mw_read_info(c, 1, &st))) return rc;
    return st;
}

extern "C" int clrs_mw_schur_assemble_dev(clrs_mw_ctx *c, const double *d_Xchol, const double *d_Y) {
    if (!c || !d_Xchol || !d_Y) return mw_fail(CLRS_ERR_INVALID, "null argument");
    MWCHECK(hipSetDevice(c->device));
    const MwDev &q = c->d;
    if (c->timing) MWCHECK(hipEventRecord(c->ev[0], c->stream));
    MW_DISPATCH(c, {
        const bool exact = c->mws_blocks > 0 && c->xinv_valid;
        bool dense_done = exact && q.ndn && !q.dn_big;
        const int pair_grid = q.nlr + (dense_done ? q.ndn : 0);
        if constexpr (DD <= 2) {
            if (exact && c->mws_turns == 1) hipLaunchKernelGGL((k_mws_pair<KK, DD, 1>), dim3(pair_grid), dim3(MWS_NT), c->sm_mws, c->stream, q, c->mws, d_Y);
            else if (exact) hipLaunchKernelGGL((k_mws_pair<KK, DD, 2>), dim3(pair_grid), dim3(MWS_NT), c->sm_mws, c->stream, q, c->mws, d_Y);
        }
        if (q.nlr && !(exact && c->mws_blocks == q.nlr)) {
            MwDev q2 = q;
            q2.mws_on = exact ? 1 : 0;
            const int gper = MW_NT / MW_GRAM_W;
            const int zt_ct = (c->xinv_valid && mw_zt_small(c)) ? 2 : MW_CT;
            hipLaunchKernelGGL((k_mw_zt<KK, DD>), dim3((c->maxU + zt_ct - 1) / zt_ct, q.nlr), dim3(MW_NT), c->sm_zt, c->stream, q2, d_Y, c->lds_zt_L ? 1 : 0, c->xinv_valid ? 1 : 0, zt_ct);
            const bool ride_gram = !dense_done && q.ndn && !q.dn_big;
            dense_done = dense_done || ride_gram;
            q2.mwx_on = c->mwx_blocks > 0 ? 1 : 0;
            hipLaunchKernelGGL((k_mw_gram<KK, DD>), dim3((c->maxU * (c->maxU + 1) / 2 + gper - 1) / gper, q.nlr + (ride_gram ? q.ndn : 0)), dim3(MW_NT), 0, c->stream, q2, d_Y);
            if (q2.mwx_on) {
                const int nt = c->mwx_maxU16 / 16;
                hipLaunchKernelGGL(k_mwx_slice<KK>, dim3(nt, 2, q.nlr), dim3(MWS_NT), 0, c->stream, q2, c->mwx);
                hipLaunchKernelGGL(k_mwx_gram<KK>, dim3((nt * (nt + 1) / 2 + MWS_NT / 64 - 1) / (MWS_NT / 64), 2, q.nlr), dim3(MWS_NT), 0, c->stream, q2, c->mwx);
            }
        }
        if (q.ndn && !dense_done) {
            const bool panels = c->xinv_valid && c->maxn_dense > 16 && c->maxn_dense <= MW_NT;
            MwDev q3 = q;
            q3.mwd_on = (panels && c->mwd_blocks > 0) ? 1 : 0;
            hipLaunchKernelGGL((k_mw_dense_t<KK, DD>), dim3(q.ndn, q.dn_big ? c->maxcnt : 1), dim3(MW_NT), c->sm_dense, c->stream, q3, d_Y, c->xinv_valid ? 1 : 0, c->dense_two ? 1 : 0, panels ? 1 : 0);
            if (panels) {
                const int pcmin = std::max(1, MW_NT / c->maxn_dense);
// ... 989 lines not shown
```

### clusteredlowranksolver.jl_amd/csrc/clrs_mw_inst.h

```cpp
#ifndef CLRS_MW_INST_H
#define CLRS_MW_INST_H

#define MW_KERNELS_K(X, K)                                                                                             \
    X __global__ void k_mw_potrf_x<K>(const MwDev, const double *, double *, int, const double *, double *, int *);    \
    X __global__ void k_mw_factor<K>(const MwDev);                                                                     \
    X __global__ void k_mw_qgram<K>(const MwDev, int);                                                                 \
    X __global__ void k_mw_potrf_q<K>(const MwDev, int, const double *, const int *, int);                             \
    X __global__ void k_mw_factor_pipe<K>(const MwDev, unsigned);                                                      \
    X __global__ void k_mw_factor_pipe64<K>(const MwDev, unsigned);                                                    \
    X __global__ void k_mw_potrf_x_pipe<K>(const MwDev, const double *, double *, const double *, double *, int *, double *, double *, int *, unsigned long long *, unsigned); \
    X __global__ void k_mw_potrf_q_pipe<K>(const MwDev, unsigned, const double *, const int *, int);                   \
    X __global__ void k_mw_bp_diag_pipe<K>(const MwDev, const MwBp *, int, int, unsigned, int, int);                   \
    X __global__ void k_mw_bp_inv_row<K>(const MwDev, const MwBp *, int);                                               \
    X __global__ void k_mw_qsum<K>(const MwDev);                                                                       \
    X __global__ void k_mw_bp_diag<K>(const MwDev, const MwBp *, int, int);                                             \
    X __global__ void k_mw_bp_panel<K>(const MwDev, const MwBp *, int);                                                \
    X __global__ void k_mw_bp_syrk<K>(const MwDev, const MwBp *, int);                                                 \
    X __global__ void k_mw_bp_inv<K>(const MwDev, const MwBp *, int);                                                  \
    X __global__ void k_mw_bp_finish<K>(const MwDev, const MwBp *);                                                    \
    X __global__ void k_mw_usum<K>(const MwDev);                                                                       \
    X __global__ void k_mw_keep_S<K>(const MwDev);                                                                     \
    X __global__ void k_mw_solve_fwd<K>(const MwDev, const double *);                                                  \
    X __global__ void k_mw_solve_mid<K, K>(const MwDev, const double *, double *);                                     \
    X __global__ void k_mw_solve_mid<K, mw_kc(K)>(const MwDev, const double *, double *);                              \
    X __global__ void k_mw_solve_wide<K>(const MwDev, int, const double *, const double *, double *, double *, double *);\
    X __global__ void k_mw_xrd<K>(const MwDev, const double *);                                                        \
    X __global__ void k_mwi_R<K>(const MwDev, const MwIpmDev, int);                                                    \
    X __global__ void k_mwi_Z<K>(const MwDev, const MwIpmDev, int, int);                                               \
    X __global__ void k_mwi_Zi<K>(const MwDev, const MwIpmDev, int);                                                   \
    X __global__ void k_mwi_Xv<K>(const MwDev, const MwIpmDev);                                                        \
    X __global__ void k_mwi_bmm<K>(const MwDev, const MwIpmDev, int, int);                                             \
    X __global__ void k_mwx_slice<K>(const MwDev, const MwxDev);                                                       \
    X __global__ void k_mwx_gram<K>(const MwDev, const MwxDev);                                                        \
    X __global__ void k_mwi_update<K>(const MwDev, const MwIpmDev);                                                    \
    X __global__ void k_mwi_init<K>(const MwDev, const MwIpmDev, double, double);                                      \
    X __global__ void k_mw_rank_reveal<K>(const MwRankMat *, double *, double *, mwi64, double *, int *, int *, double *, mwi64);     \
    X __global__ void k_mw_gemm<K>(const MwGemmJob *, const int *, const double *, mwi64, const double *, mwi64, double *, mwi64);  \
    X __global__ void k_mw_kv_scatter<K>(const MwKvBlk *, const int *, const double *, double *, mwi64);           \
    X __global__ void k_mw_rationalize<K>(const double *, mwi64, const mwi64 *, int, double, double *, double *, int *, double *);

#define MW_KERNELS_KD(X, K, DK)                                                                                        \
    X __global__ void k_mw_zt<K, DK>(const MwDev, const double *, int, int, int);                                      \
    X __global__ void k_mw_gram<K, DK>(const MwDev, const double *);                                                                   \
    X __global__ void k_mw_potrf_x_ride<K, DK>(const MwDev, const double *, double *, int, const double *, double *, int *, const double *, int, int); \
    X __global__ void k_mw_dense_t<K, DK>(const MwDev, const double *, int, int, int);                                 \
    X __global__ void k_mw_dense_tp<K, DK>(const MwDev, const double *);                                               \
    X __global__ void k_mw_dense_s<K, DK>(const MwDev, int);                                                           \
    X __global__ void k_mw_saccum<K, DK>(const MwDev, int);                                                                 \
    X __global__ void k_mw_saccum_one<K, DK>(const MwDev, int);                                                             \
    X __global__ void k_mw_linvb<K, DK>(const MwDev);                                                                  \
    X __global__ void k_mw_refine<K, DK>(const MwDev, int, const double *, double *, double *);                        \
    X __global__ void k_mw_solve_bwd<K, K, DK, 0>(const MwDev, const double *, double *, const double *, double *, const double *);        \
    X __global__ void k_mw_solve_bwd<K, K, DK, 1>(const MwDev, const double *, double *, const double *, double *, const double *);        \
    X __global__ void k_mw_solve_bwd<K, K, DK, 2>(const MwDev, const double *, double *, const double *, double *, const double *);        \
    X __global__ void k_mw_solve_bwd<K, mw_kc(K), DK, 1>(const MwDev, const double *, double *, const double *, double *, const double *); \
    X __global__ void k_mw_solve_bwd<K, mw_kc(K), DK, 2>(const MwDev, const double *, double *, const double *, double *, const double *); \
    X __global__ void k_mwi_scalar<K, DK>(const MwDev, const MwIpmDev, int, int);                                      \
    X __global__ void k_mwi_dots<K, DK>(const MwDev, const MwIpmDev, int, int);                                             \
    X __global__ void k_mwi_coef<K, DK>(const MwDev, const MwIpmDev, const double *);                                  \
    X __global__ void k_mwi_wA<K, DK>(const MwDev, const MwIpmDev, int, int, int);                                          \
    X __global__ void k_mwi_wB<K, DK>(const MwDev, const MwIpmDev, int);                                                    \
    X __global__ void k_mwi_MV<K, DK>(const MwDev, const double *);                                                    \
    X __global__ void k_mwi_rows_dn<K, DK>(const MwDev, const MwIpmDev, int);                                          \
    X __global__ void k_mwi_rows<K, DK>(const MwDev, const MwIpmDev, int, int);                                        \
    X __global__ void k_mwi_rows_fwd<K, DK>(const MwDev, const MwIpmDev);                                              \
    X __global__ void k_mwi_pv<K, DK>(const MwDev, const MwIpmDev, int);                                               \
    X __global__ void k_mwi_pvfin<K, DK>(const MwDev, const MwIpmDev);                                                 \
    X __global__ void k_mwi_gpack<K, DK>(const MwDev, const MwIpmDev, int);                                               \
    X __global__ void k_mwi_step<K, DK>(const MwDev, const MwIpmDev, int, int, int, int);

#define MW_KERNELS_KDX(X, K, DK)                                                                                       \
    X __global__ void k_mws_pair<K, DK, 1>(const MwDev, const MwsDev, const double *);                                 \
    X __global__ void k_mws_pair<K, DK, 2>(const MwDev, const MwsDev, const double *);                                 \
    X __global__ void k_mwx_dense<K, DK>(const MwDev, const MwdDev, const double *);

#define MW_KERNELS_ALL(X, K) MW_KERNELS_K(X, K) MW_KERNELS_KD(X, K, 1) MW_KERNELS_KDX(X, K, 1) MW_KERNELS_KD(X, K, 2) MW_KERNELS_KDX(X, K, 2) MW_KERNELS_KD(X, K, K)

#endif
```

### clusteredlowranksolver.jl_amd/csrc/clrs_mw_ipm.hip.h

```cpp
#include "clrs_mw_zi_panels.h"

enum { MSC_MU = 0, MSC_MUS, MSC_XY, MSC_XdY, MSC_dXY, MSC_dXdY, MSC_CY, MSC_DOBJ, MSC_POBJ, MSC_GAP, MSC_COUNT = 16 };
enum { MREC_ITER = 0, MREC_MU, MREC_DOBJ, MREC_POBJ, MREC_GAP, MREC_DERR, MREC_PERR, MREC_AD, MREC_AP, MREC_BETA, MREC_MAXP, MREC_MAXp, MREC_MAXd,
       MREC_PDFEAS, MREC_ERR, MREC_FSTAT, MREC_XSTAT, MREC_REFB, MREC_COUNT = 24 };

struct MwIpmDev {
    double *x, *y, *X, *Y, *dx, *dy, *dX, *dY, *R, *Xc, *Pm, *d, *rhsx, *pv, *coef;
    double *Yi;
    int *yfail;
    int wBn;
    double *Zs;
    double *Zt;
    double *Xv;
    double *wB;
    int *zcnt;
    unsigned long long *stamps;
    double *dtr;
    double *sc, *part;
    unsigned long long *fmax;
    double *eig;
    double *Wd;
    int *wcnt;
    double *rec;
    int *flags;
    int klow, hop;
    double *tau, *ttau, *utau;
    int *sync;
    const double *C, *c, *b;
    const int *row_clu;
    double sgn, constant;
    int Ktot, pad;
    double beta_infeasible, beta_feasible, gamma, dual_thr, primal_thr, max_gap, step_thr;
    int safe_step, corrector_only;
    double gap_thr;
    int stop_on, need_dual, need_primal, pad3;
    double *gsM, *gsS;
    int GL, Jglob;
    const int *clu_gid, *blk_gid;
};
#define MWG_S1(K, N) 0
#define MWG_S2(K, N) (K)
#define MWG_BX(K, N) (2 * (K))
#define MWG_D(K, N) (2 * (K) + (K) * (N))
#define MWG_XY(K, N) (MWG_D(K, N) + 8)
#define MWG_LEN(K, N) (MWG_D(K, N) + 8 + (K))

namespace mwk {

template <int K> __device__ __noinline__ mw<K> s_div(const mw<K> a, const mw<K> b) { return div<K>(a, b); }
template <int K> __device__ __noinline__ mw<K> s_mul(const mw<K> a, const mw<K> b) { return mul<K>(a, b); }
template <int K> __device__ __noinline__ mw<K> s_mul_d(const mw<K> a, double b) { return mul_d<K>(a, b); }
template <int K> __device__ __noinline__ mw<K> s_add(const mw<K> a, const mw<K> b) { return add<K>(a, b); }
template <int K> __device__ __noinline__ mw<K> s_sub(const mw<K> a, const mw<K> b) { return sub<K>(a, b); }
template <int K> __device__ __noinline__ mw<K> s_result(const acc<K> s) { return acc_result<K>(s); }
template <int K> __device__ __noinline__ mw<K> s_lanes64(const mw<K> v) { return lanes_sum<K, 64>(v); }
template <int K> __device__ __forceinline__ bool s_less(const mw<K> &a, const mw<K> &b) { return s_sub<K>(a, b).l[0] < 0.0; }

template <int K>
__device__ __noinline__ mw<K> wg_reduce_sum(const mw<K> &v, lds_d *red, int tid) {
    mw<K> w = lanes_sum<K, 64>(v);
    if ((tid & 63) == 0) stx<K>(red, MW_NT / 64, tid >> 6, w);
    __syncthreads();
    acc<K> s;
    acc_zero<K>(s);
#pragma unroll
    for (int i = 0; i < MW_NT / 64; i++) acc_add<K, K>(s, ldx<K>(red, MW_NT / 64, i));
    __syncthreads();
    return acc_result<K>(s);
}
__device__ __forceinline__ void atomic_max_abs(unsigned long long *slot, double v) {
    atomicMax(slot, (unsigned long long)__double_as_longlong(__builtin_fabs(v)));
}

__device__ __forceinline__ double wg_sum_d(double v, lds_d *red, int tid) {
#pragma unroll
    for (int off = 32; off > 0; off >>= 1) v += __shfl_xor(v, off, 64);
    if ((tid & 63) == 0) red[tid >> 6] = v;
    __syncthreads();
    double s = 0;
#pragma unroll
    for (int w = 0; w < MW_NT / 64; w++) s += red[w];
    return s;
}

__device__ double wg_min_eig(lds_d *A, int n, lds_d *work, int tid) {
    if (n == 1) return A[0];
    lds_d *dd = work, *ee = work + n, *v = work + 2 * n, *red = work + 3 * n, *pq = work + 3 * n + MW_NT;
    for (int k = 0; k < n - 2; k++) {
        const int m = n - k - 1;
        double part = 0;
        for (int i = tid; i < m; i += MW_NT) { double t = A[(k + 1 + i) + k * n]; part += t * t; }
        const double nrm2 = wg_sum_d(part, red, tid);
        const double x0 = A[(k + 1) + k * n];
        const double alpha = (x0 > 0 ? -1.0 : 1.0) * __builtin_sqrt(nrm2);
        if (tid == 0) { dd[k] = A[k + k * n]; ee[k] = (nrm2 == 0.0) ? 0.0 : alpha; }
        if (nrm2 == 0.0 || nrm2 == x0 * x0) {
            if (tid == 0) ee[k] = x0;
            __syncthreads();
            continue;
        }
        for (int i = tid; i < m; i += MW_NT) v[i] = A[(k + 1 + i) + k * n] - (i == 0 ? alpha : 0.0);
        __syncthreads();
        const double vtv = nrm2 - 2.0 * alpha * x0 + alpha * alpha;
        const double beta = 2.0 / vtv;
        part = 0;
        for (int i0 = 0; i0 < m; i0 += MW_NT / 4) {
            const int i = i0 + (tid >> 2);
            double sm = 0;
            if (i < m)
                for (int j = tid & 3; j < m; j += 4) sm += A[(k + 1 + i) + (k + 1 + j) * n] * v[j];
            sm += __shfl_xor(sm, 1, 64);
            sm += __shfl_xor(sm, 2, 64);
            if (i < m && (tid & 3) == 0) { pq[i] = beta * sm; part += v[i] * beta * sm; }
        }
        const double Kc = 0.5 * beta * wg_sum_d(part, red + MW_NT / 64, tid);
        for (int e = tid; e < m * m; e += MW_NT) {
            const int i = e % m, j = e / m;
            A[(k + 1 + i) + (k + 1 + j) * n] -= v[i] * (pq[j] - Kc * v[j]) + (pq[i] - Kc * v[i]) * v[j];
        }
        __syncthreads();
    }
    if (tid == 0) {
        dd[n - 2] = A[(n - 2) + (n - 2) * n];
        ee[n - 2] = A[(n - 1) + (n - 2) * n];
        dd[n - 1] = A[(n - 1) + (n - 1) * n];
    }
    __syncthreads();
    double lo = dd[0], hi = dd[0];
    for (int i = 0; i < n; i++) {
        const double r = (i > 0 ? __builtin_fabs(ee[i - 1]) : 0.0) + (i < n - 1 ? __builtin_fabs(ee[i]) : 0.0);
        lo = fmin(lo, dd[i] - r);
        hi = fmax(hi, dd[i] + r);
    }
    const double scale = fmax(__builtin_fabs(lo), __builtin_fabs(hi));
    if (scale == 0.0) return 0.0;
    lo -= 1e-14 * scale;
    hi += 1e-14 * scale;
    int *first = (int *)(double *)red;
    for (int round = 0; round < 8; round++) {
        const double h = (hi - lo) / MW_NT;
        const double sg = lo + (tid + 1) * h;
        int cnt = 0;
        double qv = dd[0] - sg;
        if (qv < 0) cnt++;
        for (int i = 1; i < n; i++) {
            if (qv == 0.0) qv = 1e-300;
            qv = dd[i] - sg - ee[i - 1] * ee[i - 1] / qv;
            if (qv < 0) cnt++;
        }
        if (tid == 0) *first = MW_NT - 1;
        __syncthreads();
        if (cnt >= 1) atomicMin(first, tid);
        __syncthreads();
        const int f = *first;
        __syncthreads();
        const double nlo = lo + f * h, nhi = lo + (f + 1) * h;
        lo = nlo;
        hi = nhi;
        if (hi - lo <= 4e-16 * scale) break;
    }
    return 0.5 * (lo + hi);
}


template <int CTRL>
__device__ __forceinline__ double dpp_mov_zero(double v) {
    int lo = __double2loint(v), hi = __double2hiint(v);
    lo = __builtin_amdgcn_update_dpp(0, lo, CTRL, 0xf, 0xf, true);
    hi = __builtin_amdgcn_update_dpp(0, hi, CTRL, 0xf, 0xf, true);
    return __hiloint2double(hi, lo);
}
__device__ __forceinline__ double readlane_f64(double v, int lane) {
    return __hiloint2double(__builtin_amdgcn_readlane(__double2hiint(v), lane), __builtin_amdgcn_readlane(__double2loint(v), lane));
}
__device__ __forceinline__ double wave_sum_d(double v) {
    v += dpp_mov_zero<0x111>(v);
    v += dpp_mov_zero<0x112>(v);
    v += dpp_mov_zero<0x114>(v);
    v += dpp_mov_zero<0x118>(v);
    return (readlane_f64(v, 15) + readlane_f64(v, 31)) + (readlane_f64(v, 47) + readlane_f64(v, 63));
}
template <int NC>
__device__ __forceinline__ void householder_regs(lds_d *A, int n, lds_d *dd, lds_d *ee, int lane) {
    double a[NC];
    const int r = lane < n ? lane : 0;
#pragma unroll
    for (int j = 0; j < NC; j++) a[j] = A[r * n + (j < n ? j : 0)];
    const bool rowok = lane < n;
#pragma unroll
    for (int j = 0; j < NC; j++) a[j] = (rowok && j < n) ? a[j] : 0.0;
#pragma unroll
    for (int c = 0; c < NC - 2; c++) {
// ... 256 lines not shown
        p.flags[0] = (q.info[1] == MW_INFO_NONE && fmax(maxp, maxP) < p.dual_thr && maxd < p.primal_thr) ? 1 : 0;
        p.fmax[0] = p.fmax[1] = p.fmax[2] = 0ull;
        q.info[0] = MW_INFO_NONE;
        q.info[1] = MW_INFO_NONE;
        return;
    }
    const bool xy_merged = stage == 10;
    if (xy_merged) stage = 0;
    if (stage == 0) {
        mw<K> xy = q.world > 1 ? mwi_gsum<K>(q, p.gsS, p.GL, xy_merged ? MWG_XY(K, q.N) : MWG_S1(K, q.N)) : mwi_sum_part<K>(q, p, 0);
        mw<K> mu = s_div<K>(xy, from_double<K>((double)p.Ktot));
        stx<K>(p.sc, SP, MSC_XY, xy);
        stx<K>(p.sc, SP, MSC_MU, mu);
        stx<K>(p.sc, SP, MSC_MUS, p.corrector_only ? mu : p.flags[0] ? zero<K>() : s_mul_d<K>(mu, p.beta_infeasible));
        p.flags[1] = 0;
        p.flags[2] = 0;
        p.fmax[0] = p.fmax[1] = p.fmax[2] = 0ull;
        for (int i = 0; i < MREC_COUNT; i++) p.rec[i] = 0.0;
        p.rec[MREC_ITER] = iter;
        p.rec[MREC_MU] = mu.l[0];
        if (mu.l[0] > p.max_gap) p.flags[1] = 3;
    }
    mw<K> pre_xy = zero<K>(), pre_mu = zero<K>(), pre_sum = zero<K>();
    int pre_flag0 = 0;
    if (stage == 2) {
        pre_xy = ldx<K>(p.sc, SP, MSC_XY);
        pre_mu = ldx<K>(p.sc, SP, MSC_MU);
        pre_flag0 = p.flags[0];
        if (q.world <= 1 && q.NB <= 8) {
            mw<K> part[8];
#pragma unroll
            for (int b = 0; b < 8; b++) part[b] = b < q.NB ? ldx<K>(p.part, 5L * q.NB, 1L * q.NB + b) : zero<K>();
            acc<K> s;
            acc_zero<K>(s);
#pragma unroll
            for (int b = 0; b < 8; b++) if (b < q.NB) acc_add<K, K>(s, part[b]);
            pre_sum = acc_result<K>(s);
        }
    }
    if (stage == 1 || stage == 2) {
        const double maxP = __longlong_as_double((long long)p.fmax[0]), maxp = __longlong_as_double((long long)p.fmax[2]);
        double maxd = __longlong_as_double((long long)p.fmax[1]);
        if (q.world > 1 && stage == 2) {
            for (int r = 0; r < q.world; r++) maxd = fmax(maxd, p.gsM[(long)r * p.GL + MWG_D(K, q.N) + 1]);
        }
        p.fmax[0] = 0ull;
        p.rec[MREC_MAXP] = maxP; p.rec[MREC_MAXd] = maxd; p.rec[MREC_MAXp] = maxp;
        p.rec[MREC_DERR] = fmax(maxp, maxP);
        p.rec[MREC_PERR] = maxd;
        int fs = q.info[0], xs = q.info[1];
        if (q.world > 1) {
            fs = xs = MW_INFO_NONE;
            for (int r = q.world - 1; r >= 0; r--) {
                const double *D = p.gsM + (long)r * p.GL + MWG_D(K, q.N);
                if ((int)D[4] != MW_INFO_NONE) fs = (int)D[4];
                if ((int)D[5] != MW_INFO_NONE) xs = (int)D[5];
            }
        }
        p.rec[MREC_FSTAT] = fs == MW_INFO_NONE ? 0 : fs;
        p.rec[MREC_XSTAT] = xs == MW_INFO_NONE ? 0 : xs;
        if ((fs != MW_INFO_NONE || xs != MW_INFO_NONE) && p.flags[1] == 0) p.flags[1] = (fs == MW_INFO_TIMEOUT || xs == MW_INFO_TIMEOUT) ? 5 : 1;
        q.info[0] = MW_INFO_NONE;
        q.info[1] = MW_INFO_NONE;
    }
    if (stage == 2) {
        acc<K> s;
        acc_zero<K>(s);
        acc_add<K, K>(s, pre_xy);
        acc_add<K, K>(s, q.world > 1 ? mwi_gsum<K>(q, p.gsM, p.GL, MWG_S1(K, q.N)) : q.NB <= 8 ? pre_sum : mwi_sum_part<K>(q, p, 1));
        mw<K> mu = pre_mu;
        mw<K> r = s_div<K>(s_result<K>(s), s_mul_d<K>(mu, (double)p.Ktot));
        mw<K> beta = s_less<K>(r, from_double<K>(1.0)) ? s_mul<K>(r, r) : r;
        mw<K> beta_c;
        if (pre_flag0) {
            beta_c = s_less<K>(from_double<K>(p.beta_feasible), beta) ? beta : from_double<K>(p.beta_feasible);
            if (s_less<K>(from_double<K>(1.0), beta_c)) beta_c = from_double<K>(1.0);
        } else {
            beta_c = s_less<K>(from_double<K>(p.beta_infeasible), beta) ? beta : from_double<K>(p.beta_infeasible);
        }
        stx<K>(p.sc, SP, MSC_MUS, s_mul<K>(beta_c, mu));
        p.rec[MREC_BETA] = beta_c.l[0];
        p.flags[0] = (p.rec[MREC_DERR] < p.dual_thr && p.rec[MREC_PERR] < p.primal_thr) ? 1 : 0;
        p.rec[MREC_PDFEAS] = p.flags[0];
    }
    if (stage == 3) mwi_scalar_stage3<K>(q, p);
}
template <int K, int DK>
__global__ void k_mwi_scalar(const MwDev q, const MwIpmDev p, int stage, int iter) {
    if (blockIdx.x == 0 && threadIdx.x < 64) mwi_scalar_stage<K, DK>(q, p, stage, iter);
}


#define MWI_EW 4
template <int K, int EW>
__device__ __forceinline__ void mwi_R_body(const MwDev &q, const MwIpmDev &p, int corrector, int bx, int by) {
    using namespace mwk;
    const MwBlk &k = q.blk[by];
    const int n = k.n;
    if (bx * (MW_NT / EW) >= n * n) return;
    const int e = bx * (MW_NT / EW) + threadIdx.x / EW, sub = threadIdx.x % EW;
    const bool live = e < n * n;
    const int ee = live ? e : 0, i = ee % n, c = ee / n;
    acc<K> s;
    acc_zero<K>(s);
    for (int kk = sub; kk < n; kk += EW) acc_fma<K, K, K>(s, ldx<K>(p.X + k.xyoff, q.xylen, i + (long)kk * n), ldx<K>(p.Y + k.xyoff, q.xylen, kk + (long)c * n), -1.0);
    if (corrector)
        for (int kk = sub; kk < n; kk += EW) acc_fma<K, K, K>(s, ldx<K>(p.dX + k.xyoff, q.xylen, i + (long)kk * n), ldx<K>(p.dY + k.xyoff, q.xylen, kk + (long)c * n), -1.0);
    const mw<K> v = lanes_sum<K, EW>(acc_result<K>(s));
    if (live && sub == 0) stx<K>(p.R + k.xyoff, q.xylen, e, v);
}
template <int K>
__global__ __launch_bounds__(MW_NT) void k_mwi_R(const MwDev q, const MwIpmDev p, int corrector) { mwi_R_body<K, MWI_EW>(q, p, corrector, blockIdx.x, blockIdx.y); }

template <int K, int KA, int DK>
__device__ __forceinline__ void mwi_dots_body(const MwDev &q, const MwIpmDev &p, int sel) {
    using namespace mwk;
    const MwBlk &k = q.blk[blockIdx.x];
    const int tid = threadIdx.x;
    const long nn = (long)k.n * k.n;
    acc<KA> a0, a1, a4;
    acc_zero<KA>(a0); acc_zero<KA>(a1); acc_zero<KA>(a4);
    for (long i = tid; i < nn; i += MW_NT) {
        const long e = k.xyoff + i;
        mw<KA> Y = ldx<KA>(p.Y, q.xylen, e);
        if (sel & 1) acc_fma<KA, KA, KA>(a0, ldx<KA>(p.X, q.xylen, e), Y);
        if (sel & 2) {
            mw<KA> X = ldx<KA>(p.X, q.xylen, e), dX = ldx<KA>(p.dX, q.xylen, e), dY = ldx<KA>(p.dY, q.xylen, e);
            acc_fma<KA, KA, KA>(a1, X, dY);
            acc_fma<KA, KA, KA>(a1, dX, Y);
            acc_fma<KA, KA, KA>(a1, dX, dY);
        }
        if (sel & 4) acc_fma<KA, KA, DK>(a4, Y, ldx<DK>(p.C, q.xylen, e));
    }
    lds_d *red = MW_LDS;
    if (sel & 1) { mw<KA> r = wg_reduce_sum<KA>(acc_result<KA>(a0), red, tid); if (tid == 0) stx<K>(p.part, 5L * q.NB, 0L * q.NB + blockIdx.x, cvt<K, KA>(r)); }
    if (sel & 2) {
        mw<KA> r = wg_reduce_sum<KA>(acc_result<KA>(a1), red, tid); if (tid == 0) stx<K>(p.part, 5L * q.NB, 1L * q.NB + blockIdx.x, cvt<K, KA>(r));
    }
    if (sel & 4) { mw<KA> r = wg_reduce_sum<KA>(acc_result<KA>(a4), red, tid); if (tid == 0) stx<K>(p.part, 5L * q.NB, 4L * q.NB + blockIdx.x, cvt<K, KA>(r)); }
}
template <int K, int DK>
__global__ __launch_bounds__(MW_NT) void k_mwi_dots(const MwDev q, const MwIpmDev p, int sel, int r_tiles) {
    using namespace mwk;
    if ((int)blockIdx.x >= q.NB) {
        const int w = blockIdx.x - q.NB;
        if (r_tiles < 0) mwi_R_body<K, 16>(q, p, 1, w % (-r_tiles), w / (-r_tiles));
        else mwi_R_body<K, MWI_EW>(q, p, 1, w % r_tiles, w / r_tiles);
        return;
    }
    if constexpr (mw_kf_of(K) < K) { if (p.klow < K) { mwi_dots_body<K, mw_kf_of(K), DK>(q, p, sel); return; } }
    mwi_dots_body<K, K, DK>(q, p, sel);
}


template <int K, int DK>
__global__ __launch_bounds__(MW_NT) void k_mwi_coef(const MwDev q, const MwIpmDev p, const double *__restrict__ a) {
    using namespace mwk;
    const mwi64 t = (mwi64)blockIdx.x * MW_NT + threadIdx.x;
    if (t >= q.T) return;
    const int b = q.ay_blk[t];
    if (b < 0) return;
    const MwClu &c = q.clu[q.blk[b].j];
    stx<K>(p.coef, q.T, t, mulx<K, K, DK>(ldx<K>(a, q.xlen, c.coff + q.st_p[t]), ldx<DK>(q.st_lam, q.lamp, t)));
}

template <int K, int KA, int DK, int EW>
__device__ __forceinline__ void mwi_wA_body_ka(const MwDev &q, const MwIpmDev &p, int mode, int coef_lds, int use_B) {
    using namespace mwk;
    const MwBlk &k = q.blk[blockIdx.y];
    const int n = k.n;
    if (blockIdx.x * (MW_NT / EW) >= n * n) return;
    lds_d *cf = MW_LDS;
    int t_first = 0, t_cnt = 0;
    if (coef_lds && k.kind == 0) {
        const int *tp0 = q.tptr + k.tptr_off;
        t_first = tp0[0]; t_cnt = tp0[k.P] - tp0[0];
        const double *av = mode == 0 ? p.x : p.dx;
        const MwClu &cl0 = q.clu[k.j];
        for (int t = threadIdx.x; t < t_cnt; t += MW_NT)
            stx<KA>(cf, t_cnt, t, mulx<KA, KA, DK>(ldx<KA>(av, q.xlen, cl0.coff + q.st_p[t_first + t]), ldx<DK>(q.st_lam, q.lamp, t_first + t)));
        __syncthreads();
    }
    const int e = blockIdx.x * (MW_NT / EW) + threadIdx.x / EW, sub = threadIdx.x % EW;
    const int ee = e < n * n ? e : 0, i = ee % n, c = ee / n;
    const double *a = mode == 0 ? p.x : p.dx;
    const bool mirror = (k.kind == 0 && k.m > 1);
    const bool live = e < n * n && !(mirror && c > i);
    acc<KA> s;
    acc_zero<KA>(s);
    if (k.kind == 0) {
        const double *V = q.V + k.v_off;
        const int *tp = q.tptr + k.tptr_off;
        for (int t = tp[0] + sub; t < tp[k.P]; t += EW) {
            if (!(q.st_flag[t] & 1)) continue;
            if (use_B) {
                const mw<DK> vi = ldx<DK>(V, q.Vp, i + (long)q.st_war[t] * n);
                if (vi.l[0] == 0.0) continue;
                acc_fma<KA, KA, DK>(s, ldx<KA>(p.wB, q.T * (long)p.wBn, (long)t * p.wBn + c), vi);
                continue;
            }
            const mw<DK> vi = ldx<DK>(V, q.Vp, i + (long)q.st_war[t] * n), vc = ldx<DK>(V, q.Vp, c + (long)q.st_wac[t] * n);
            if (vi.l[0] == 0.0 || vc.l[0] == 0.0) continue;
            constexpr int LL = (2 * DK + 1 < KA) ? 2 * DK + 1 : KA;
            acc_fma<KA, KA, LL>(s, coef_lds ? ldx<KA>(cf, t_cnt, t - t_first) : ldx<KA>(p.coef, q.T, t), mulx<LL, DK, DK>(vi, vc));
        }
    } else {
        const MwClu &cl = q.clu[k.j];
        const long nn = (long)n * n;
        for (int en = sub; en < k.cnt; en += EW)
            acc_fma<KA, KA, DK>(s, ldx<KA>(a, q.xlen, cl.coff + q.dense_p[k.d0 + en]), ldx<DK>(q.dA, q.dAp, k.a_off + en * nn + ee));
    }
    if (sub == 0) {
        if (mode == 0) {
            acc_add<KA, KA>(s, ldx<KA>(p.X + k.xyoff, q.xylen, ee), -1.0);
            acc_add<KA, DK>(s, ldx<DK>(p.C, q.xylen, k.xyoff + ee), -p.sgn);
        } else {
            acc_add<KA, KA>(s, ldx<KA>(p.Pm + k.xyoff, q.xylen, ee));
        }
    }
    const mw<K> v = cvt<K, KA>(lanes_sum<KA, EW>(acc_result<KA>(s)));
    if (!live || sub != 0) return;
    if (mode == 0) {
        atomic_max_abs(&p.fmax[0], v.l[0]);
        stx<K>(p.Pm + k.xyoff, q.xylen, e, v);
        if (mirror && c != i) stx<K>(p.Pm + k.xyoff, q.xylen, c + (long)i * n, v);
    } else {
        stx<K>(p.dX + k.xyoff, q.xylen, e, v);
        if (mirror && c != i) stx<K>(p.dX + k.xyoff, q.xylen, c + (long)i * n, v);
    }
}
template <int K, int DK, int EW>
__device__ __forceinline__ void mwi_wA_body(const MwDev &q, const MwIpmDev &p, int mode, int coef_lds, int use_B) {
    if constexpr (mw_kf_of(K) < K) { if (p.klow < K) { mwi_wA_body_ka<K, mw_kf_of(K), DK, EW>(q, p, mode, coef_lds, use_B); return; } }
    mwi_wA_body_ka<K, K, DK, EW>(q, p, mode, coef_lds, use_B);
}
template <int K, int DK>
__global__ __launch_bounds__(MW_NT) void k_mwi_wA(const MwDev q, const MwIpmDev p, int mode, int coef_lds, int ew) {
    if (ew == 17) mwi_wA_body<K, DK, 16>(q, p, mode, 0, 1);
    else if (ew == 16) mwi_wA_body<K, DK, 16>(q, p, mode, coef_lds, 0);
    else mwi_wA_body<K, DK, MWI_EW>(q, p, mode, coef_lds, 0);
}
template <int K, int DK>
__global__ __launch_bounds__(MW_NT) void k_mwi_wB(const MwDev q, const MwIpmDev p, int mode) {
    using namespace mwk;
    const mwi64 e = (mwi64)blockIdx.x * MW_NT + threadIdx.x;
    const mwi64 t = e / p.wBn;
    const int c = (int)(e % p.wBn);
    if (t >= q.T) return;
    const int b = q.ay_blk[t];
    if (b < 0 || !(q.st_flag[t] & 1)) return;
    const MwBlk &k = q.blk[b];
    if (c >= k.n) return;
    const MwClu &cl = q.clu[k.j];
    const double *a = mode == 0 ? p.x : p.dx;
    const mw<K> cf = mulx<K, K, DK>(ldx<K>(a, q.xlen, cl.coff + q.st_p[t]), ldx<DK>(q.st_lam, q.lamp, t));
    const mw<DK> vc = ldx<DK>(q.V + k.v_off, q.Vp, c + (long)q.st_wac[t] * k.n);
    stx<K>(p.wB, q.T * (long)p.wBn, t * p.wBn + c, mulx<K, K, DK>(cf, vc));
}

template <int K, int DK>
__global__ __launch_bounds__(MW_NT) void k_mwi_MV(const MwDev q, const double *__restrict__ M) {
    using namespace mwk;
    const MwBlk &k = q.blk[q.lr_list[blockIdx.y]];
    const int n = k.n, dl = k.delta;
    if (blockIdx.x * (MW_NT / MWI_EW) >= n * k.U) return;
    const int e = blockIdx.x * (MW_NT / MWI_EW) + threadIdx.x / MWI_EW, sub = threadIdx.x % MWI_EW;
    const bool live = e < n * k.U;
    const int ee = live ? e : 0, i = ee % n, c = ee / n;
    const double *V = q.V + k.v_off;
    const int r0 = q.vrow[k.vrow_off + c];
    acc<K> s;
    acc_zero<K>(s);
    for (int kk = r0 + sub; kk < r0 + dl; kk += MWI_EW) acc_fma<K, K, DK>(s, ldx<K>(M + k.xyoff, q.xylen, i + (long)kk * n), ldx<DK>(V, q.Vp, kk + (long)c * n));
    const mw<K> v = lanes_sum<K, MWI_EW>(acc_result<K>(s));
    if (live && sub == 0) stx<K>(q.Tm + k.z_off, q.zlen, e, v);
}

template <int K, int DK>
__global__ __launch_bounds__(MW_NT) void k_mwi_rows_dn(const MwDev q, const MwIpmDev p, int mode) {
    using namespace mwk;
    const mwi64 g = (mwi64)blockIdx.x * (MW_NT / 64) + (threadIdx.x >> 6);
    if (g >= q.xlen) return;
    const int lane = threadIdx.x & 63;
    const double *M = mode == 0 ? p.Y : p.dY;
    acc<K> s;
    acc_zero<K>(s);
    for (int t = q.drow_ptr[g]; t < q.drow_ptr[g + 1]; t++) {
        const MwBlk &k = q.blk[q.drow_blk[t]];
        const long nn = (long)k.n * k.n, a0 = k.a_off + (long)q.drow_en[t] * nn;
        for (long i = lane; i < nn; i += 64) acc_fma<K, K, DK>(s, ldx<K>(M + k.xyoff, q.xylen, i), ldx<DK>(q.dA, q.dAp, a0 + i));
    }
    const mw<K> v = lanes_sum<K, 64>(acc_result<K>(s));
    if (lane == 0) stx<K>(p.dtr, q.xlen, g, v);
}

#define MWI_RW 8
template <int K, int DK, int BG>
__device__ __forceinline__ void mwi_rows_body(const MwDev &q, const MwIpmDev &p, int mode, mwi64 g0, bool live) {
    using namespace mwk;
    constexpr int RWT = MWI_RW * BG;
    const int sub = threadIdx.x % MWI_RW, grp = (threadIdx.x % RWT) / MWI_RW, sub_all = threadIdx.x % RWT;
    const mwi64 g = live ? g0 : 0;
    const int j = p.row_clu[g];
    const MwClu &cl = q.clu[j];
    const int pp = (int)(g - cl.coff);
    const double *M = mode == 0 ? p.Y : p.dY;
    acc<K> s;
    acc_zero<K>(s);
    const bool with_tau = mode == 0 && p.tau != nullptr && q.AX != nullptr;
    acc<K> st;
    acc_zero<K>(st);
    for (int b = cl.b0 + grp; b < cl.b1; b += BG) {
        const MwBlk &k = q.blk[b];
        const int n = k.n;
        if (k.kind == 0) {
            const int *tp = q.tptr + k.tptr_off;
            if (mode == 0) {
                for (int t = tp[pp] + sub; t < tp[pp + 1]; t += MWI_RW) {
                    const int fl = q.st_flag[t];
                    if (!(fl & 1)) continue;
                    const mw<DK> w = mul_pow2<DK>(ldx<DK>(q.st_lam, q.lamp, t), (fl & 2) ? 2.0 : 1.0);
                    acc_fma<K, K, DK>(s, ldx<K>(q.AY, q.T, q.st_orig[t]), w, -1.0);
                    if (with_tau) acc_fma<K, K, DK>(st, ldx<K>(q.AX, q.T, q.st_orig[t]), w);
                }
            } else {
                const double *V = q.V + k.v_off;
                for (int t = tp[pp]; t < tp[pp + 1]; t++) {
                    const int fl = q.st_flag[t];
                    if (!(fl & 1)) continue;
                    const mw<DK> w = mul_pow2<DK>(ldx<DK>(q.st_lam, q.lamp, t), (fl & 2) ? 2.0 : 1.0);
                    const int l = q.st_trl[t], dcol = q.st_trd[t], r0 = q.vrow[k.vrow_off + l];
                    acc<K> z;
                    acc_zero<K>(z);
                    for (int ii = r0 + sub; ii < r0 + k.delta; ii += MWI_RW) acc_fma<K, K, DK>(z, ldx<K>(q.Tm + k.z_off, q.zlen, ii + (long)dcol * n), ldx<DK>(V, q.Vp, ii + (long)l * n));
                    acc_fma<K, K, DK>(s, acc_result<K>(z), w, -1.0);
                }
            }
        } else if (!q.dn_big) {
            const int en = q.dmap[k.dmap_off + pp];
            if (en >= 0) {
                const long nn = (long)n * n;
                for (long i = sub; i < nn; i += MWI_RW) acc_fma<K, K, DK>(s, ldx<K>(M + k.xyoff, q.xylen, i), ldx<DK>(q.dA, q.dAp, k.a_off + en * nn + i), -1.0);
                if (with_tau && sub == 0) {
                    const mw<K> xi = ldx<K>(q.Xi + k.xyoff, q.xylen, 0);
                    acc_fma<K, K, DK>(st, mul<K>(xi, xi), ldx<DK>(q.dA, q.dAp, k.a_off + en * nn));
                }
            }
        }
    }
    if (q.dn_big && sub_all == 0) acc_add<K, K>(s, ldx<K>(p.dtr, q.xlen, g), -1.0);
    if (mode == 0) {
        if (sub_all == 0) acc_add<K, DK>(s, ldx<DK>(p.c, q.xlen, g));
        for (int a = sub_all; a < q.N; a += RWT) acc_fma<K, K, DK>(s, ldx<K>(p.y, q.N, a), ldx<DK>(q.B, q.Bp, g + (long)a * q.xlen), -1.0);
        const mw<K> dv = lanes_sum<K, RWT>(acc_result<K>(s));
        if (live && sub_all == 0) {
            atomic_max_abs(&p.fmax[1], dv.l[0]);
            stx<K>(p.d, q.xlen, g, dv);
        }
        if (with_tau) {
            const mw<K> tv = lanes_sum<K, RWT>(acc_result<K>(st));
            if (live && sub_all == 0) stx<K>(p.tau, q.xlen, g, tv);
        }
    } else {
        if (sub_all == 0) acc_add<K, K>(s, ldx<K>(p.d, q.xlen, g), -1.0);
        const mw<K> r = lanes_sum<K, RWT>(acc_result<K>(s));
        if (live && sub_all == 0) stx<K>(p.rhsx, q.xlen, g, r);
    }
}
template <int K, int DK>
__global__ __launch_bounds__(MW_NT) void k_mwi_rows(const MwDev q, const MwIpmDev p, int mode, int groups) {
    if (groups == 8) { const mwi64 g0 = (mwi64)blockIdx.x * (MW_NT / (MWI_RW * 8)) + threadIdx.x / (MWI_RW * 8); mwi_rows_body<K, DK, 8>(q, p, mode, g0, g0 < q.xlen); }
    else { const mwi64 g0 = (mwi64)blockIdx.x * (MW_NT / MWI_RW) + threadIdx.x / MWI_RW; mwi_rows_body<K, DK, 1>(q, p, mode, g0, g0 < q.xlen); }
}
template <int K, int DK>
__global__ __launch_bounds__(MW_NT) void k_mwi_rows_fwd(const MwDev q, const MwIpmDev p) {
    const MwClu &c = q.clu[blockIdx.x];
    for (int r0 = 0; r0 < c.P; r0 += MW_NT / MWI_RW) {
        const int r = r0 + threadIdx.x / MWI_RW;
        mwi_rows_body<K, DK, 1>(q, p, 1, c.coff + r, r < c.P);
    }
    __threadfence_block();
    __syncthreads();
    mw_solve_fwd_cluster<K>(q, blockIdx.x, p.rhsx);
}

template <int UNIT>
__global__ void k_mwi_mark(int *word, int iter) {
    if (blockIdx.x == 0 && threadIdx.x == 0) {
        __builtin_amdgcn_fence(__ATOMIC_RELEASE, "agent");
        __hip_atomic_store(word, iter, __ATOMIC_RELAXED, __HIP_MEMORY_SCOPE_AGENT);
    }
}

template <int UNIT>
__global__ void k_mwi_wait(const int *word, int value, int *info, int code) {
    (void)code;
    if (blockIdx.x == 0 && threadIdx.x == 0) {
        unsigned spins = 0;
        unsigned long long t0 = 0;
        while (__hip_atomic_load(word, __ATOMIC_RELAXED, __HIP_MEMORY_SCOPE_AGENT) < value) {
            __builtin_amdgcn_s_sleep(32);
            if ((++spins & 1023u) == 0) {
                const unsigned long long now = wall_clock64();
                if (t0 == 0) t0 = now;
                else if (now - t0 > MW_WAIT_TICKS) { atomicMin(info, MW_INFO_TIMEOUT); break; }
            }
        }
    }
}

template <int K, int DK>
__global__ void k_mwi_gpack(const MwDev q, const MwIpmDev p, int stage) {
    using namespace mwk;
    if (blockIdx.x != 0 || threadIdx.x >= 64) return;
    const int lane = threadIdx.x, N = q.N;
    double *slot = ((stage == 2 || stage == 3) ? p.gsM : p.gsS) + (long)q.rank * p.GL, *D = slot + MWG_D(K, N);
    const bool with_xy = stage == 15;
    if (with_xy) stage = 4;
    if (stage == 4) {
        acc<K> s;
        acc_zero<K>(s);
        for (long i = lane; i < q.xlen; i += 64) acc_fma<K, K, DK>(s, ldx<K>(p.x, q.xlen, i), ldx<DK>(p.c, q.xlen, i), p.sgn);
        const mw<K> cx = s_lanes64<K>(s_result<K>(s));
        if (lane == 0) {
#pragma unroll
            for (int l = 0; l < K; l++) slot[MWG_S2(K, N) + l] = cx.l[l];
        }
    }
    if (lane != 0) return;
    if (stage == 0 || stage == 2 || stage == 4) {
        const mw<K> v = mwi_sum_part<K>(q, p, stage == 0 ? 0 : stage == 2 ? 1 : 4);
#pragma unroll
        for (int l = 0; l < K; l++) slot[MWG_S1(K, N) + l] = v.l[l];
    }
    if (with_xy) {
        const mw<K> v = mwi_sum_part<K>(q, p, 0);
#pragma unroll
        for (int l = 0; l < K; l++) slot[MWG_XY(K, N) + l] = v.l[l];
        D[0] = __longlong_as_double((long long)p.fmax[0]);
        D[1] = 0.0;
    }
    if (stage == 1) {
        D[0] = __longlong_as_double((long long)p.fmax[0]);
        D[1] = __longlong_as_double((long long)p.fmax[1]);
    }
    if (stage == 2) {
        D[1] = __longlong_as_double((long long)p.fmax[1]);
        const int fs = q.info[0], xs = q.info[1];
        D[4] = fs == MW_INFO_NONE ? MW_INFO_NONE : fs > q.J ? p.Jglob + 1 : p.clu_gid ? p.clu_gid[fs - 1] + 1 : fs;
        D[5] = xs == MW_INFO_NONE ? MW_INFO_NONE : p.blk_gid ? p.blk_gid[xs - 1] + 1 : xs;
    }
    if (stage == 3) {
        for (int w = 0; w < 2; w++) {
            double mn = p.eig[(long)w * q.NB];
            for (int b = 1; b < q.NB; b++) mn = fmin(mn, p.eig[(long)w * q.NB + b]);
            D[2 + w] = mn;
        }
        D[6] = p.flags[2];
        if (q.refstat) {
#pragma unroll
            for (int i = 0; i < 4; i++) slot[MWG_S1(K, N) + i] = __longlong_as_double((long long)q.refstat[i]);
        }
    }
}
template <int K, int DK>
__global__ __launch_bounds__(MW_NT) void k_mwi_pvfin(const MwDev q, const MwIpmDev p) {
    using namespace mwk;
    const int N = q.N;
    for (int a = blockIdx.x * MW_NT + threadIdx.x; a < N; a += gridDim.x * MW_NT) {
        acc<K> s;
        acc_zero<K>(s);
        acc_add<K, DK>(s, ldx<DK>(p.b, N, a), p.sgn);
        for (int r = 0; r < q.world; r++) acc_add<K, K>(s, ldx<K>(p.gsS + (long)r * p.GL + MWG_BX(K, N), N, a));
        const mw<K> v = acc_result<K>(s);
        atomic_max_abs(&p.fmax[2], v.l[0]);
        stx<K>(p.pv, N, a, v);
    }
    if (blockIdx.x == 0 && threadIdx.x == 0) {
        double mP = 0, md = 0;
        for (int r = 0; r < q.world; r++) {
            const double *D = p.gsS + (long)r * p.GL + MWG_D(K, N);
            mP = fmax(mP, D[0]); md = fmax(md, D[1]);
        }
        p.fmax[0] = (unsigned long long)__double_as_longlong(mP);
        p.fmax[1] = (unsigned long long)__double_as_longlong(md);
    }
}

template <int K, int DK>
__global__ __launch_bounds__(MW_NT) void k_mwi_pv(const MwDev q, const MwIpmDev p, int iter) {
    using namespace mwk;
    const int a = blockIdx.x * (MW_NT / 8) + threadIdx.x / 8, sub = threadIdx.x % 8;
    const bool live = a < q.N;
    const int aa = live ? a : 0;
    acc<K> s;
    acc_zero<K>(s);
    const bool part = q.world > 1;
    if (sub == 0 && !part) acc_add<K, DK>(s, ldx<DK>(p.b, q.N, aa), p.sgn);
    for (long g = sub; g < q.xlen; g += 8) acc_fma<K, K, DK>(s, ldx<K>(p.x, q.xlen, g), ldx<DK>(q.B, q.Bp, g + (long)aa * q.xlen), -1.0);
    mw<K> v = lanes_sum<K, 8>(acc_result<K>(s));
    if (live && sub == 0) {
        if (part) stx<K>(p.gsS + (long)q.rank * p.GL + MWG_BX(K, q.N), q.N, a, v);
        else {
            atomic_max_abs(&p.fmax[2], v.l[0]);
            stx<K>(p.pv, q.N, a, v);
        }
    }
    (void)iter;
}

template <int K>
__global__ __launch_bounds__(MW_NT) void k_mwi_Z(const MwDev q, const MwIpmDev p, int which, int lds_L) {
    using namespace mwk;
    const MwBlk &k = q.blk[blockIdx.x];
    if (k.inv) return;
    const int n = k.n, tid = threadIdx.x;
    const long nn = (long)n * n;
    lds_d *M = MW_LDS;
    const double *A = (which == 0 ? p.Pm : p.dX) + k.xyoff;
    const double sg = which == 0 ? 1.0 : -1.0;
    for (int e = tid; e < nn; e += MW_NT) {
        const int i = e % n, c = e / n;
        acc<K> s;
        acc_zero<K>(s);
        for (int kk = 0; kk < n; kk++) acc_fma<K, K, K>(s, ldx<K>(A, q.xylen, i + (long)kk * n), ldx<K>(p.Y + k.xyoff, q.xylen, kk + (long)c * n), sg);
        acc_add<K, K>(s, ldx<K>(p.R + k.xyoff, q.xylen, e), -sg);
        if (i == c) acc_add<K, K>(s, ldx<K>(p.sc, MSC_COUNT, MSC_MUS), -sg);
        stx<K>(M, nn, e, acc_result<K>(s));
    }
    if (lds_L) {
        lds_d *Lf = MW_LDS + (long)K * nn, *Lb = Lf + (long)K * nn;
        wg_copy<K>(Lf, nn, n, q.Xf + k.xyoff, q.xylen, n, n, n, tid);
// ... 456 lines not shown
```

### clusteredlowranksolver.jl_amd/csrc/clrs_mw_ipm_host.inc

```
struct MwIpm {
    MwIpmDev d = {};
    bool ready = false;
    int iter = 0;
    bool xy_with_tail = false;
    bool upd_recorded = false;
    int sync_seq = 0;
    bool global_set = false;
    int gs_world = 0;
    bool forked = false, tail_pending = false;
    bool frozen = false;
    int held_refine_bits = 0;
    bool aff_ok = false;
    double *AX = nullptr;
    int kf_now = 0;
    double *h_rec = nullptr;
    double *d_rec = nullptr;
    size_t sm_Z = 0, sm_Zi = 0, sm_step = 0;
    int zs = MWI_ZS;
    int zt = MW_PT;
    int zs_step = MWI_ZS;
    size_t sm_bmm = 0;
    bool z_tiled = false;
    size_t maxn_inv = 0;
    bool lds_ZL = false, step_w_lds = true, step_inv = false, y_with_x = false, any_xinv = false, any_xsub = false;
    hipStream_t side = nullptr;
    enum { E_ASM, E_PREP, E_UPD, E_REC0, E_REC1, E_COUNT };
    hipEvent_t ev[E_COUNT] = {};
    ~MwIpm() {
        if (h_rec) (void)hipHostFree(h_rec);
        for (auto &e : ev) if (e) (void)hipEventDestroy(e);
        if (side) (void)hipStreamDestroy(side);
    }
};

static void mw_ipm_free(clrs_mw_ctx *c) {
    delete c->ipm;
    c->ipm = nullptr;
}

extern "C" int clrs_mw_ipm_create_ex(clrs_mw_ctx *c, const clrs_ipm_data *data, int data_limbs);
extern "C" int clrs_mw_ipm_create(clrs_mw_ctx *c, const clrs_ipm_data *data) { return clrs_mw_ipm_create_ex(c, data, 1); }

extern "C" int clrs_mw_ipm_create_ex(clrs_mw_ctx *c, const clrs_ipm_data *data, int data_limbs) {
    if (!c || !data) return mw_fail(CLRS_ERR_INVALID, "null argument");
    if (data_limbs < 1 || data_limbs > c->DK) return mw_fail(CLRS_ERR_INVALID, "data limbs of the objective exceed those of the context");
    MWCHECK(hipSetDevice(c->device));
    const MwDev &q = c->d;
    const int K = c->K, N = q.N, NB = q.NB;
    if (NB == 0) return mw_fail(CLRS_ERR_INVALID, "no PSD blocks");
    if (!c->ipm) c->ipm = new MwIpm();
    MwIpm *st = c->ipm;
    MwIpmDev &p = st->d;
    int rc;
    if (!st->ready) {
        double **xy[] = {&p.X, &p.Y, &p.dX, &p.dY, &p.R, &p.Xc, &p.Pm};
        for (double **b : xy) if ((rc = mw_dmalloc(c, b, q.xylen * K))) return rc;
        double **xs[] = {&p.x, &p.dx, &p.d, &p.rhsx};
        for (double **b : xs) if ((rc = mw_dmalloc(c, b, q.xlen * K))) return rc;
        double **ys[] = {&p.y, &p.dy, &p.pv};
        for (double **b : ys) if ((rc = mw_dmalloc(c, b, (i64)N * K))) return rc;
        if ((rc = mw_dmalloc(c, &p.coef, q.T * K)) || (rc = mw_dmalloc(c, &p.dtr, q.xlen * K))) return rc;
        p.wBn = 0; p.wB = nullptr;
        if (c->maxTb >= 128) {
            int maxn_lr = 1;
            for (auto &k : c->blk) if (k.kind == 0) maxn_lr = std::max(maxn_lr, k.n);
            p.wBn = maxn_lr;
            if ((rc = mw_dmalloc(c, &p.wB, q.T * (i64)maxn_lr * K))) return rc;
        }
        if ((rc = mw_dmalloc(c, &p.Yi, q.xylen * K)) || (rc = mw_dmalloc(c, &p.Zs, q.xylen * K))) return rc;
        if ((rc = mw_dmalloc(c, &p.Zt, q.xylen * K))) return rc;
        { double *t3 = nullptr; if ((rc = mw_dmalloc(c, &t3, (NB + 1) / 2 + 1))) return rc; p.zcnt = (int *)t3; }
        { double *t2 = nullptr; if ((rc = mw_dmalloc(c, &t2, (NB + 1) / 2 + 1))) return rc; p.yfail = (int *)t2; }
        if ((rc = mw_dmalloc(c, &p.sc, (i64)MSC_COUNT * K))) return rc;
        if ((rc = mw_dmalloc(c, &p.part, 5LL * NB * K))) return rc;
        if ((rc = mw_dmalloc(c, &p.eig, 2LL * NB))) return rc;
        if ((rc = mw_dmalloc(c, &p.Wd, 2LL * q.xylen))) return rc;
        { double *t4 = nullptr; if ((rc = mw_dmalloc(c, &t4, NB + 1))) return rc; p.wcnt = (int *)t4; }
        if ((rc = mw_dmalloc(c, &st->d_rec, 2 * MREC_COUNT))) return rc;
        p.rec = st->d_rec;
        double *tmp = nullptr;
        if ((rc = mw_dmalloc(c, &tmp, 4))) return rc;
        p.fmax = (unsigned long long *)tmp;
        if ((rc = mw_dmalloc(c, &tmp, 4))) return rc;
        p.flags = (int *)tmp;
        if ((rc = mw_dmalloc(c, &tmp, 4))) return rc;
        p.sync = (int *)tmp;
        p.tau = p.ttau = p.utau = nullptr;
        p.klow = K;
        p.hop = c->chain_hop;
        std::vector<int> row_clu((size_t)q.xlen);
        for (int j = 0; j < q.J; j++)
            for (int r = 0; r < c->clu[j].P; r++) row_clu[c->clu[j].coff + r] = j;
        if ((rc = mw_upload(c, row_clu, &p.row_clu))) return rc;
        double *dC, *dc, *db;
        if ((rc = mw_dmalloc(c, &dC, q.xylen * c->DK)) || (rc = mw_dmalloc(c, &dc, q.xlen * c->DK)) || (rc = mw_dmalloc(c, &db, (i64)N * c->DK))) return rc;
        p.C = dC; p.c = dc; p.b = db;
        MWCHECK(hipHostMalloc((void **)&st->h_rec, sizeof(double) * 2 * MREC_COUNT, hipHostMallocDefault));
        MWCHECK(hipStreamCreateWithFlags(&st->side, hipStreamNonBlocking));
        for (int e = 0; e < MwIpm::E_COUNT; e++)
            MWCHECK(hipEventCreateWithFlags(&st->ev[e], e < MwIpm::E_REC0 ? (hipEventDisableTiming | hipEventDisableSystemFence) : hipEventDisableTiming));
        p.Ktot = 0;
        size_t maxn = 0;
        for (auto &k : c->blk) { p.Ktot += k.n; maxn = std::max(maxn, (size_t)k.n); }
        const size_t lim = MW_LDS_MAX / sizeof(double), nnK = maxn * maxn * K;
        if (nnK > lim) return mw_fail(CLRS_ERR_INVALID, "device-resident multi-word iteration needs PSD blocks that fit in LDS");
        st->lds_ZL = 3 * nnK <= lim;
        st->sm_Z = (st->lds_ZL ? 3 : 1) * nnK * 8;
        const size_t step_rest = (size_t)K * maxn + maxn * maxn + 3 * maxn + 2 * MW_NT + MW_POTRF_SCR(K, maxn) + 8;
        st->step_w_lds = 2 * nnK + step_rest <= lim;
        const size_t stepd = (st->step_w_lds ? 2 : 1) * nnK + step_rest;
        if (stepd > lim) return mw_fail(CLRS_ERR_INVALID, "device-resident multi-word iteration needs PSD blocks that fit in LDS");
        st->sm_step = stepd * 8;
        size_t &maxn_inv = st->maxn_inv;
        maxn_inv = 0;
        for (auto &k : c->blk) {
            if (k.inv) { st->any_xinv = true; maxn_inv = std::max(maxn_inv, (size_t)k.n); }
            else st->any_xsub = true;
        }
        {
            const MwZiPanels zp = mw_zi_panels((int)maxn_inv, q.NB, K, c->zi_narrow && maxn_inv <= 24);
            st->zs = zp.zs; st->zt = zp.threads; st->sm_Zi = zp.sm;
            const int old_rule = std::max<int>(MWI_ZS, (int)((maxn_inv + 7) / 8));
            {
                const int pcs = std::max<int>(1, 64 / (int)std::max<size_t>(maxn_inv, 1)), wants = ((int)maxn_inv + pcs - 1) / pcs;
                st->zs_step = std::max<int>(old_rule, std::min<int>(wants, 320 / std::max(q.NB, 1)));
            }
        }
        st->z_tiled = maxn_inv > 24;
        p.Xv = nullptr;
        if (st->any_xinv && !st->z_tiled && c->xinv_product && (rc = mw_dmalloc(c, &p.Xv, q.xylen * K))) return rc;
        st->sm_bmm = (size_t)2 * K * MWI_BT * maxn_inv * 8;
        const size_t step_inv_need = 3 * maxn_inv * maxn_inv * K + step_rest;
        bool all_lds_inv = st->any_xinv;
        for (auto &k : c->blk) all_lds_inv = all_lds_inv && k.inv == 1;
        st->step_inv = all_lds_inv && step_inv_need <= lim;
        const size_t step_need2 = nnK + maxn * maxn + 3 * maxn + 2 * MW_NT + 8;
        st->y_with_x = st->any_xinv && !st->any_xsub && step_need2 <= lim;
        if (!st->y_with_x && !st->step_inv) c->d.no_xfb = 0;
        if (st->step_inv) st->sm_step = std::max(st->sm_step, step_inv_need * 8);
        if (st->y_with_x) st->sm_step = std::max(st->sm_step, step_need2 * 8);
        MW_DISPATCH(c, {
            if ((rc = mw_set_lds(k_mwi_Zi<KK>, st->sm_Zi))) return rc;
            if ((rc = mw_set_lds((k_mwi_rows_fwd<KK, DD>), c->sm_fwd))) return rc;
            if ((rc = mw_set_lds(k_mwi_bmm<KK>, st->sm_bmm))) return rc;
            if ((rc = mw_set_lds(k_mwi_Z<KK>, st->sm_Z))) return rc;
            if ((rc = mw_set_lds((k_mwi_step<KK, DD>), st->sm_step))) return rc;
        });
        {
            int mostb = 1;
            for (int j = 0; j < q.J; j++) mostb = std::max(mostb, c->clu[j].b1 - c->clu[j].b0);
            st->aff_ok = N > 0 && !c->wide_solve && (c->lds_q || c->pipe_Q) && mostb < 16 && q.J <= 4 && !q.dn_big && st->any_xinv && !st->any_xsub && !st->z_tiled &&
                         !q.mws_on && !q.mwx_on && c->refine != 0 && g_cfg_mw_affine_corrector != 0;
            if (st->aff_ok) {
                if ((rc = mw_dmalloc(c, &st->AX, q.T * K)) || (rc = mw_dmalloc(c, &p.tau, q.xlen * K)) || (rc = mw_dmalloc(c, &p.ttau, q.xlen * K)) ||
                    (rc = mw_dmalloc(c, &p.utau, (i64)q.J * N * K))) return rc;
            }
        }
        p.beta_infeasible = 0.3; p.beta_feasible = 0.1; p.gamma = 0.9; p.dual_thr = 1e-30; p.primal_thr = 1e-30;
        p.max_gap = 1e100; p.step_thr = 1e-7; p.safe_step = 1; p.corrector_only = 0;
        p.gap_thr = 0.0; p.stop_on = 0; p.need_dual = 0; p.need_primal = 0;
        st->ready = true;
    }
    MWCHECK(hipMemset((void *)p.C, 0, sizeof(double) * q.xylen * c->DK));
    MWCHECK(hipMemset((void *)p.c, 0, sizeof(double) * q.xlen * c->DK));
    if (N) MWCHECK(hipMemset((void *)p.b, 0, sizeof(double) * N * c->DK));
    MWCHECK(hipMemcpy((void *)p.C, data->C, sizeof(double) * q.xylen * data_limbs, hipMemcpyHostToDevice));
    MWCHECK(hipMemcpy((void *)p.c, data->c, sizeof(double) * q.xlen * data_limbs, hipMemcpyHostToDevice));
    if (N) MWCHECK(hipMemcpy((void *)p.b, data->b, sizeof(double) * N * data_limbs, hipMemcpyHostToDevice));
    p.sgn = data->maximize ? 1.0 : -1.0;
    p.constant = data->constant;
    return 0;
}

extern "C" int clrs_mw_ipm_set_params(clrs_mw_ctx *c, const clrs_ipm_params *prm) {
    if (!c || !prm || !c->ipm || !c->ipm->ready) return mw_fail(CLRS_ERR_STATE, "clrs_mw_ipm_create first");
    MwIpmDev &p = c->ipm->d;
    p.beta_infeasible = prm->beta_infeasible; p.beta_feasible = prm->beta_feasible; p.gamma = prm->gamma;
    p.dual_thr = prm->dual_error_threshold; p.primal_thr = prm->primal_error_threshold; p.max_gap = prm->max_complementary_gap;
    p.step_thr = prm->step_length_threshold; p.safe_step = prm->safe_step; p.corrector_only = prm->corrector_only != 0;
    return 0;
}

static int mw_ipm_exchange(clrs_mw_ctx *c, hipStream_t stream, int stage) {
    const MwDev &q = c->d;
    if (q.world <= 1) return 0;
    MwIpm *st = c->ipm;
    const MwIpmDev &p = st->d;
    if (!st->global_set || st->gs_world != q.world) return mw_fail(CLRS_ERR_STATE, "sharded interior-point iteration: clrs_mw_ipm_set_global first");
    const bool onM = stage == 2 || stage == 3;
    MW_DISPATCH(c, hipLaunchKernelGGL((k_mwi_gpack<KK, DD>), dim3(1), dim3(64), 0, stream, q, p, stage));
    MWCHECK(hipGetLastError());
    return mw_allgather(c, stream == c->stream ? 0 : 1, onM ? p.gsM : p.gsS, (size_t)p.GL, stream);
}
static int mw_ipm_wA(clrs_mw_ctx *c, hipStream_t stream, int mode);
static int mw_ipm_objectives(clrs_mw_ctx *c, hipStream_t stream, bool with_xy = false) {
    const MwDev &q = c->d;
    const MwIpmDev &p = c->ipm->d;
    int rc;
    if (with_xy && q.world > 1) {
        if ((rc = mw_ipm_wA(c, stream, 0))) return rc;
        MW_DISPATCH(c, {
            if (q.N) hipLaunchKernelGGL((k_mwi_pv<KK, DD>), dim3((q.N + MW_NT / 8 - 1) / (MW_NT / 8)), dim3(MW_NT), 0, stream, q, p, c->ipm->iter);
        });
    }
    MW_DISPATCH(c, hipLaunchKernelGGL((k_mwi_dots<KK, DD>), dim3(q.NB), dim3(MW_NT), (size_t)KK * 8 * 8, stream, q, p, with_xy ? 5 : 4, 0));
    if ((rc = mw_ipm_exchange(c, stream, with_xy ? 15 : 4))) return rc;
    MW_DISPATCH(c, hipLaunchKernelGGL((k_mwi_scalar<KK, DD>), dim3(1), dim3(64), 0, stream, q, p, 4, c->ipm->iter));
    MWCHECK(hipGetLastError());
    return 0;
}
#define MW_KF_MARGIN 14
static void mw_ipm_reset_kf(clrs_mw_ctx *c) {
    c->ipm->kf_now = (c->kf_low < c->K && (!c->d.gathered || g_cfg_mw_sharded_factor_limbs != 0)) ? c->kf_low : c->K;
    c->ipm->held_refine_bits = 0;
    (void)hipMemsetAsync(c->d.refstat, 0, 4 * sizeof(unsigned long long), c->stream);
}
static void mw_ipm_note_bits(clrs_mw_ctx *c, int refine_bits) {
    MwIpm *st = c->ipm;
    if (st->kf_now < c->K && refine_bits > 0 && refine_bits < 53 * (c->K - st->kf_now) + MW_KF_MARGIN) st->kf_now = c->K;
}
static int mw_ipm_arm(clrs_mw_ctx *c) {
    MWCHECK(hipMemsetAsync(c->d.info, 0x7f, 2 * sizeof(int), c->stream));
    MWCHECK(hipMemsetAsync(c->ipm->d.flags, 0, 4 * sizeof(double), c->stream));
    return 0;
}

extern "C" int clrs_mw_ipm_init(clrs_mw_ctx *c, double omega_p, double omega_d) {
    if (!c || !c->ipm || !c->ipm->ready) return mw_fail(CLRS_ERR_STATE, "clrs_mw_ipm_create first");
    MWCHECK(hipSetDevice(c->device));
    const MwDev &q = c->d;
    MwIpm *st = c->ipm;
    const MwIpmDev &p = st->d;
    const int K = c->K;
    MWCHECK(hipMemsetAsync(p.x, 0, sizeof(double) * q.xlen * K, c->stream));
    if (q.N) MWCHECK(hipMemsetAsync(p.y, 0, sizeof(double) * q.N * K, c->stream));
    int rc;
    if ((rc = mw_ipm_arm(c))) return rc;
    MWCHECK(hipMemsetAsync(p.sc, 0, sizeof(double) * MSC_COUNT * K, c->stream));
    MW_DISPATCH(c, hipLaunchKernelGGL(k_mwi_init<KK>, dim3(q.NB), dim3(MW_NT), 0, c->stream, q, p, omega_p, omega_d));
    MWCHECK(hipGetLastError());
    st->iter = 0;
    st->forked = false; st->tail_pending = false;
    mw_ipm_reset_kf(c);
    if ((rc = mw_ipm_objectives(c, c->stream))) return rc;
    MWCHECK(hipStreamSynchronize(c->stream));
    return 0;
}

static int mw_ipm_rows(clrs_mw_ctx *c, hipStream_t stream, int mode);
static int mw_ipm_wA(clrs_mw_ctx *c, hipStream_t stream, int mode);
static int mw_ipm_drain(clrs_mw_ctx *c);
extern "C" int clrs_mw_ipm_set(clrs_mw_ctx *c, const double *x, const double *y, const double *X, const double *Y) {
    if (!c || !c->ipm || !c->ipm->ready) return mw_fail(CLRS_ERR_STATE, "clrs_mw_ipm_create first");
    MWCHECK(hipSetDevice(c->device));
    const MwDev &q = c->d;
    MwIpm *st = c->ipm;
    const MwIpmDev &p = st->d;
    const int K = c->K;
    { int rc_ = mw_ipm_drain(c); if (rc_) return rc_; }
    if (x) MWCHECK(hipMemcpy(p.x, x, sizeof(double) * q.xlen * K, hipMemcpyHostToDevice));
    if (y && q.N) MWCHECK(hipMemcpy(p.y, y, sizeof(double) * q.N * K, hipMemcpyHostToDevice));
    if (X) MWCHECK(hipMemcpy(p.X, X, sizeof(double) * q.xylen * K, hipMemcpyHostToDevice));
    if (Y) MWCHECK(hipMemcpy(p.Y, Y, sizeof(double) * q.xylen * K, hipMemcpyHostToDevice));
    int rc;
    if ((rc = mw_ipm_arm(c))) return rc;
    MWCHECK(hipMemsetAsync(p.fmax, 0, 3 * sizeof(unsigned long long), c->stream));
    hipStream_t M = c->stream;
    if ((rc = mw_cholesky_blocks_dev2(c, p.X, p.Xc, nullptr, nullptr, nullptr))) return rc;
    if ((rc = clrs_mw_schur_assemble_dev(c, p.Xc, p.Y))) return rc;
    if ((rc = mw_ipm_wA(c, M, 0))) return rc;
    MW_DISPATCH(c, {
        if (q.dn_big) hipLaunchKernelGGL((k_mwi_rows_dn<KK, DD>), dim3((unsigned)((q.xlen + MW_NT / 64 - 1) / (MW_NT / 64))), dim3(MW_NT), 0, M, q, p, 0);
    });
    if ((rc = mw_ipm_rows(c, M, 0))) return rc;
    MW_DISPATCH(c, {
        if (q.N) hipLaunchKernelGGL((k_mwi_pv<KK, DD>), dim3((q.N + MW_NT / 8 - 1) / (MW_NT / 8)), dim3(MW_NT), 0, M, q, p, 0);
    });
    if ((rc = mw_ipm_exchange(c, M, 1))) return rc;
    MW_DISPATCH(c, {
        if (q.world > 1) hipLaunchKernelGGL((k_mwi_pvfin<KK, DD>), dim3(1), dim3(MW_NT), 0, M, q, p);
        hipLaunchKernelGGL((k_mwi_scalar<KK, DD>), dim3(1), dim3(1), 0, M, q, p, 5, 0);
    });
    MWCHECK(hipGetLastError());
    c->assembled = false;
    st->iter = 0;
    st->forked = false; st->tail_pending = false; st->frozen = false;
    mw_ipm_reset_kf(c);
    if ((rc = mw_ipm_objectives(c, c->stream))) return rc;
    MWCHECK(hipStreamSynchronize(c->stream));
    return 0;
}

static int mw_ipm_rhs(clrs_mw_ctx *c, hipStream_t stream, int which) {
    const MwDev &q = c->d;
    MwIpm *st = c->ipm;
    st->d.stamps = c->mws.stamps;
    const MwIpmDev &p = st->d;
    MW_DISPATCH(c, {
        if (st->any_xinv && st->z_tiled) {
            const int nt = ((int)st->maxn_inv + MWI_BT - 1) / MWI_BT;
            for (int op = 0; op < 4; op++) hipLaunchKernelGGL(k_mwi_bmm<KK>, dim3(nt * nt, q.NB), dim3(MW_NT), st->sm_bmm, stream, q, p, op, which);
        } else if (st->any_xinv) hipLaunchKernelGGL(k_mwi_Zi<KK>, dim3(q.NB, st->zs), dim3(st->zt), st->sm_Zi, stream, q, p, which);
        if (st->any_xsub) hipLaunchKernelGGL(k_mwi_Z<KK>, dim3(q.NB), dim3(MW_NT), st->sm_Z, stream, q, p, which, st->lds_ZL ? 1 : 0);
    });
    MWCHECK(hipGetLastError());
    return 0;
}
static int mw_ipm_trace_rhs(clrs_mw_ctx *c, hipStream_t stream) {
    const MwDev &q = c->d;
    const MwIpmDev &p = c->ipm->d;
    MW_DISPATCH(c, {
        if (q.nlr) hipLaunchKernelGGL((k_mwi_MV<KK, DD>), dim3((c->maxn * c->maxU * MWI_EW + MW_NT - 1) / MW_NT, q.nlr), dim3(MW_NT), 0, stream, q, (const double *)p.dY);
        if (q.dn_big) hipLaunchKernelGGL((k_mwi_rows_dn<KK, DD>), dim3((unsigned)((q.xlen + MW_NT / 64 - 1) / (MW_NT / 64))), dim3(MW_NT), 0, stream, q, p, 1);
    });
    MWCHECK(hipGetLastError());
    return 0;
}
static int mw_ipm_rows(clrs_mw_ctx *c, hipStream_t stream, int mode) {
    const MwDev &q = c->d;
    const MwIpmDev &p = c->ipm->d;
    int mostb = 1;
    for (int j = 0; j < q.J; j++) mostb = std::max(mostb, c->clu[j].b1 - c->clu[j].b0);
    const int groups = mostb >= 16 ? 8 : 1;
    MW_DISPATCH(c, hipLaunchKernelGGL((k_mwi_rows<KK, DD>), dim3((unsigned)((q.xlen * MWI_RW * groups + MW_NT - 1) / MW_NT)), dim3(MW_NT), 0, stream, q, p, mode, groups));
    MWCHECK(hipGetLastError());
    return 0;
}
static int mw_ipm_wA(clrs_mw_ctx *c, hipStream_t stream, int mode) {
    const MwDev &q = c->d;
    const MwIpmDev &p = c->ipm->d;
    const int maxnn = c->maxn * c->maxn;
    const size_t sm = (size_t)c->maxTb * c->K * 8;
    const bool in_lds = sm <= 48 * 1024;
    MW_DISPATCH(c, {
        if (q.T && !in_lds) hipLaunchKernelGGL((k_mwi_coef<KK, DD>), dim3((unsigned)((q.T + MW_NT - 1) / MW_NT)), dim3(MW_NT), 0, stream, q, p, (const double *)(mode == 0 ? p.x : p.dx));
        const int ew = c->maxTb >= 24 ? 16 : MWI_EW;
        if (p.wBn) hipLaunchKernelGGL((k_mwi_wB<KK, DD>), dim3((unsigned)((q.T * (i64)p.wBn + MW_NT - 1) / MW_NT)), dim3(MW_NT), 0, stream, q, p, mode);
        hipLaunchKernelGGL((k_mwi_wA<KK, DD>), dim3((maxnn * ew + MW_NT - 1) / MW_NT, q.NB), dim3(MW_NT), in_lds && !p.wBn ? sm : 0, stream, q, p, mode, in_lds && !p.wBn ? 1 : 0, p.wBn ? 17 : ew);
    });
    MWCHECK(hipGetLastError());
    return 0;
}
static int mw_ipm_solve_dX(clrs_mw_ctx *c, bool predictor = false) {
    const MwIpmDev &p = c->ipm->d;
    int rc;
    c->refine_skip_next = predictor && !c->refine_predictor;
    if ((rc = clrs_mw_schur_solve_dev(c, p.rhsx, p.pv, p.dx, p.dy))) return rc;
    return mw_ipm_wA(c, c->stream, 1);
}

static int mw_ipm_tail(clrs_mw_ctx *c, int word_value = 0, bool with_next = false) {
    MwIpm *st = c->ipm;
    if (!st->tail_pending) return 0;
    const int par = st->iter & 1;
    int rc;
    if (word_value > 0) hipLaunchKernelGGL(k_mwi_wait<0>, dim3(1), dim3(64), 0, st->side, (const int *)(st->d.sync + 2), word_value, c->d.info, c->d.J + 1);
    else {
        if (!st->upd_recorded) MWCHECK(hipEventRecord(st->ev[MwIpm::E_UPD], c->stream));
        MWCHECK(hipStreamWaitEvent(st->side, st->ev[MwIpm::E_UPD], 0));
    }
    if ((rc = mw_ipm_objectives(c, st->side, word_value != 0 || with_next))) return rc;
    st->xy_with_tail = word_value != 0 || with_next;
    MWCHECK(hipMemcpyAsync(st->h_rec + (size_t)par * MREC_COUNT, st->d.rec, sizeof(double) * MREC_COUNT, hipMemcpyDeviceToHost, st->side));
    MWCHECK(hipEventRecord(st->ev[MwIpm::E_REC0 + par], st->side));
    st->tail_pending = false;
    return 0;
}
static int mw_ipm_enqueue_body(clrs_mw_ctx *c) {
    const MwDev &q = c->d;
    MwIpm *st = c->ipm;
    const int maxnn = c->maxn * c->maxn;
    const size_t sm_red = (size_t)c->K * 8 * 8;
    hipStream_t M = c->stream, S = st->side;
    int rc;
    const bool words = !q.gathered && c->stream_words;
    c->d.kf = st->kf_now;
    const int seq = ++st->sync_seq;
    const MwIpmDev &p = st->d;
    c->ipm_arms_info = true;
    c->d.mark_word = words ? p.sync + 2 : nullptr;
    c->d.mark_value = seq;
    const bool y_rides = mw_y_riders_ok(c);
    c->ride_y = y_rides ? p.Y : nullptr;
    rc = mw_cholesky_blocks_dev2(c, p.X, p.Xc, st->y_with_x ? p.Y : nullptr, p.Yi, p.yfail);
    c->ride_y = nullptr;
    c->d.mark_word = nullptr;
    if (rc) return rc;
    st->xy_with_tail = false;
    if ((rc = mw_ipm_tail(c, words ? seq : 0, true))) return rc;
    if (!st->forked) {
        MWCHECK(hipEventRecord(st->ev[MwIpm::E_UPD], M));
        MWCHECK(hipStreamWaitEvent(S, st->ev[MwIpm::E_UPD], 0));
        st->forked = true;
    }
    st->iter++;
    st->d.rec = st->d_rec + (size_t)(st->iter & 1) * MREC_COUNT;
    const bool aff = st->aff_ok && !q.gathered;
    c->d.AX = aff ? st->AX : nullptr;
    c->d.skip_y = y_rides ? 1 : 0;
    rc = clrs_mw_schur_assemble_dev(c, p.Xc, p.Y);
    c->d.skip_y = 0;
    if (rc) return rc;
    if (!words) MWCHECK(hipEventRecord(st->ev[MwIpm::E_ASM], M));
    c->d.mark_word = words ? p.sync + 1 : nullptr;
    const bool split_factor = q.N > 0;
    rc = split_factor ? clrs_mw_schur_factor_local_dev(c) : clrs_mw_schur_factor_dev(c);
    c->d.mark_word = nullptr;
    if (rc) return rc;
    if (split_factor && q.gathered && (rc = mw_allgather(c, 0, q.Qg, (size_t)q.N * q.N * c->K, M))) return rc;
    c->ipm_arms_info = false;
    if (!st->xy_with_tail) {
        MW_DISPATCH(c, hipLaunchKernelGGL((k_mwi_dots<KK, DD>), dim3(q.NB), dim3(MW_NT), sm_red, S, q, p, 1, 0));
        if ((rc = mw_ipm_exchange(c, S, 0))) return rc;
    }
    MW_DISPATCH(c, hipLaunchKernelGGL((k_mwi_scalar<KK, DD>), dim3(1), dim3(1), 0, S, q, p, st->xy_with_tail ? 10 : 0, st->iter));
    MWCHECK(hipGetLastError());
    const bool res_with_tail = st->xy_with_tail && q.world > 1;
    if (res_with_tail) {
        MW_DISPATCH(c, hipLaunchKernelGGL((k_mwi_pvfin<KK, DD>), dim3(1), dim3(MW_NT), 0, S, q, p));
        MWCHECK(hipGetLastError());
    } else if ((rc = mw_ipm_wA(c, S, 0))) return rc;
    MW_DISPATCH(c, hipLaunchKernelGGL(k_mwi_R<KK>, dim3((maxnn * MWI_EW + MW_NT - 1) / MW_NT, q.NB), dim3(MW_NT), 0, S, q, p, 0));
    MWCHECK(hipGetLastError());
    if (words) hipLaunchKernelGGL(k_mwi_wait<0>, dim3(1), dim3(64), 0, S, (const int *)(p.sync + 1), seq, q.info, q.J + 1);
    else MWCHECK(hipStreamWaitEvent(S, st->ev[MwIpm::E_ASM], 0));
    if (p.Xv) {
        const int xv_tiles = ((int)(st->maxn_inv * st->maxn_inv) * MWI_ZL + MW_NT - 1) / MW_NT;
        MW_DISPATCH(c, hipLaunchKernelGGL(k_mwi_Xv<KK>, dim3(xv_tiles, q.NB), dim3(MW_NT), 0, S, q, p));
        MWCHECK(hipGetLastError());
    }
    if ((rc = mw_ipm_rhs(c, S, 0))) return rc;
    if ((rc = mw_ipm_trace_rhs(c, S))) return rc;
    MW_DISPATCH(c, {
        if (q.dn_big) hipLaunchKernelGGL((k_mwi_rows_dn<KK, DD>), dim3((unsigned)((q.xlen + MW_NT / 64 - 1) / (MW_NT / 64))), dim3(MW_NT), 0, S, q, p, 0);
    });
    {
        double *const keep_tau = st->d.tau;
        if (!aff) st->d.tau = nullptr;
        rc = mw_ipm_rows(c, S, 0);
        st->d.tau = keep_tau;
        if (rc) return rc;
    }
    if (!res_with_tail) {
        MW_DISPATCH(c, {
            if (q.N) hipLaunchKernelGGL((k_mwi_pv<KK, DD>), dim3((q.N + MW_NT / 8 - 1) / (MW_NT / 8)), dim3(MW_NT), 0, S, q, p, st->iter);
        });
        if ((rc = mw_ipm_exchange(c, S, 1))) return rc;
    }
    MW_DISPATCH(c, {
        if (q.world > 1 && !res_with_tail) hipLaunchKernelGGL((k_mwi_pvfin<KK, DD>), dim3(1), dim3(MW_NT), 0, S, q, p);
        if (q.dn_big) hipLaunchKernelGGL((k_mwi_rows_dn<KK, DD>), dim3((unsigned)((q.xlen + MW_NT / 64 - 1) / (MW_NT / 64))), dim3(MW_NT), 0, S, q, p, 1);
    });
    MWCHECK(hipGetLastError());
    if ((rc = mw_ipm_rows(c, S, 1))) return rc;
    const bool word_sync = words && split_factor && !c->wide_solve && (c->lds_q || c->pipe_Q);
    if (word_sync) hipLaunchKernelGGL(k_mwi_mark<0>, dim3(1), dim3(1), 0, S, p.sync, seq);
    else {
        MWCHECK(hipEventRecord(st->ev[MwIpm::E_PREP], S));
        MWCHECK(hipStreamWaitEvent(M, st->ev[MwIpm::E_PREP], 0));
    }
    if (split_factor) {
        c->ride_wait = word_sync ? p.sync : nullptr;
        c->ride_wait_value = seq;
        c->ride_fwd = p.rhsx;
        c->ipm_arms_info = true;
        if (aff) { c->d.ride2_rhs = p.tau; c->d.ride2_t = p.ttau; c->d.ride2_u = p.utau; }
        rc = clrs_mw_schur_factor_finish_dev(c);
        c->d.ride2_rhs = nullptr;
        c->ipm_arms_info = false;
        c->ride_fwd = nullptr;
        c->ride_wait = nullptr;
        if (rc) return rc;
    }
    st->d.klow = c->refine_predictor ? c->K : c->d.kf;
    rc = mw_ipm_solve_dX(c, true);
    if (!rc) rc = mw_ipm_rhs(c, M, 1);
    if (rc) { st->d.klow = c->K; return rc; }
    const bool r16 = (i64)maxnn * 16 * q.NB <= 65536;
    const int r_tiles = (maxnn * (r16 ? 16 : MWI_EW) + MW_NT - 1) / MW_NT;
    MW_DISPATCH(c, hipLaunchKernelGGL((k_mwi_dots<KK, DD>), dim3(q.NB + r_tiles * q.NB), dim3(MW_NT), sm_red, M, q, p, 2, r16 ? -r_tiles : r_tiles));
    st->d.klow = c->K;
    if ((rc = mw_ipm_exchange(c, M, 2))) return rc;
    const bool aff_async = aff && word_sync;
    if (aff_async) {
        c->d.mark_word = p.sync + 3; c->d.mark_value = seq;
        rc = mw_ipm_rhs(c, M, 2);
        c->d.mark_word = nullptr;
        if (rc) return rc;
        hipLaunchKernelGGL(k_mwi_wait<0>, dim3(1), dim3(64), 0, S, (const int *)(p.sync + 3), seq, q.info, q.J + 1);
        MW_DISPATCH(c, hipLaunchKernelGGL((k_mwi_scalar<KK, DD>), dim3(1), dim3(1), 0, S, q, p, 2, st->iter));
        hipLaunchKernelGGL(k_mwi_mark<0>, dim3(1), dim3(1), 0, S, p.sync + 4, seq);
        MWCHECK(hipGetLastError());
    } else {
        MW_DISPATCH(c, hipLaunchKernelGGL((k_mwi_scalar<KK, DD>), dim3(1), dim3(1), 0, M, q, p, 2, st->iter));
        MWCHECK(hipGetLastError());
        if ((rc = mw_ipm_rhs(c, M, aff ? 2 : 0))) return rc;
    }
    if ((rc = mw_ipm_trace_rhs(c, M))) return rc;
    {
        int mostb = 1;
        for (int j = 0; j < q.J; j++) mostb = std::max(mostb, c->clu[j].b1 - c->clu[j].b0);
        if (!c->wide_solve && mostb < 16 && q.J <= 64) {
            MW_DISPATCH(c, hipLaunchKernelGGL((k_mwi_rows_fwd<KK, DD>), dim3(q.J), dim3(MW_NT), c->sm_fwd, M, q, p));
            MWCHECK(hipGetLastError());
            c->fwd_rode = true;
        } else if ((rc = mw_ipm_rows(c, M, 1))) return rc;
    }
    if (aff) {
        if (!c->fwd_rode) return mw_fail(CLRS_ERR_STATE, "affine corrector without the fused forward half");
        c->d.aff_mu = p.sc + MSC_MUS; c->d.aff_mu_plane = MSC_COUNT; c->d.aff_rhs = p.tau; c->d.aff_t = p.ttau; c->d.aff_u = p.utau;
        c->d.aff_wait = aff_async ? p.sync + 4 : nullptr; c->d.aff_wait_value = seq;
    }
    rc = mw_ipm_solve_dX(c);
    c->d.aff_mu = nullptr;
    if (rc) return rc;
    if ((rc = mw_ipm_rhs(c, M, 1))) return rc;
    const int ip = st->y_with_x ? 2 : st->step_inv ? 1 : 0, wl = st->step_w_lds ? 1 : 0;
    if (ip == 2 && st->z_tiled) {
        const int nt = ((int)st->maxn_inv + MWI_BT - 1) / MWI_BT;
        MW_DISPATCH(c, {
            hipLaunchKernelGGL(k_mwi_bmm<KK>, dim3(nt * nt, q.NB, 2), dim3(MW_NT), st->sm_bmm, M, q, p, 4, 0);
            hipLaunchKernelGGL(k_mwi_bmm<KK>, dim3(nt * nt, q.NB, 2), dim3(MW_NT), st->sm_bmm, M, q, p, 5, 0);
            hipLaunchKernelGGL((k_mwi_step<KK, DD>), dim3(q.NB, 2, 1), dim3(MW_NT), st->sm_step, M, q, p, wl, 3, st->iter, 0);
        });
    } else
    MW_DISPATCH(c, hipLaunchKernelGGL((k_mwi_step<KK, DD>), dim3(q.NB, 2, ip == 2 ? st->zs_step : 1), dim3(MW_NT), st->sm_step, M, q, p, wl, ip, st->iter, 0));
    if ((rc = mw_ipm_exchange(c, M, 3))) return rc;
    MW_DISPATCH(c, {
        if (q.world > 1) hipLaunchKernelGGL((k_mwi_scalar<KK, DD>), dim3(1), dim3(1), 0, M, q, p, 3, st->iter);
        hipLaunchKernelGGL(k_mwi_update<KK>, dim3((unsigned)std::min<i64>(1024, (q.xylen + q.xlen + q.N + MW_NT - 1) / MW_NT)), dim3(MW_NT), 0, M, q, p);
    });
    MWCHECK(hipGetLastError());
    if (!words) MWCHECK(hipEventRecord(st->ev[MwIpm::E_UPD], M));
    st->upd_recorded = !words;
    st->tail_pending = true;
    return 0;
}
static int mw_ipm_enqueue(clrs_mw_ctx *c) {
    const int rc = mw_ipm_enqueue_body(c);
    c->d.kf = c->kf_entry;
    c->ipm->d.klow = c->K;
    c->d.AX = nullptr; c->d.aff_mu = nullptr; c->d.ride2_rhs = nullptr;
    c->ipm_arms_info = false;
    c->ride_fwd = nullptr;
    c->ride_wait = nullptr;
    c->ride_y = nullptr;
    c->d.skip_y = 0;
    c->d.mark_word = nullptr;
    if (rc) { c->fwd_rode = false; c->ipm->tail_pending = false; }
    return rc;
}
static int mw_ipm_finish(clrs_mw_ctx *c) { return mw_ipm_tail(c); }
static void mw_ipm_read_record(const double *r, clrs_ipm_record *out) {
    out->iter = (int)r[MREC_ITER]; out->pd_feas = (int)r[MREC_PDFEAS]; out->error_code = (int)r[MREC_ERR];
    out->factor_status = (int)r[MREC_FSTAT]; out->cholesky_status = (int)r[MREC_XSTAT]; out->refine_bits = (int)r[MREC_REFB];
    out->mu = r[MREC_MU]; out->d_obj = r[MREC_DOBJ]; out->p_obj = r[MREC_POBJ]; out->gap = r[MREC_GAP];
    out->dual_error = r[MREC_DERR]; out->primal_error = r[MREC_PERR]; out->alpha_d = r[MREC_AD]; out->alpha_p = r[MREC_AP];
    out->beta_c = r[MREC_BETA]; out->max_P = r[MREC_MAXP]; out->max_p = r[MREC_MAXp]; out->max_d = r[MREC_MAXd];
}
static int mw_ipm_drain(clrs_mw_ctx *c) {
    MWCHECK(hipStreamSynchronize(c->stream));
    MWCHECK(hipStreamSynchronize(c->ipm->side));
    return 0;
}

extern "C" int clrs_mw_ipm_iterate(clrs_mw_ctx *c, clrs_ipm_record *out) {
    if (!c || !out || !c->ipm || !c->ipm->ready) return mw_fail(CLRS_ERR_STATE, "clrs_mw_ipm_create first");
    MWCHECK(hipSetDevice(c->device));
    MwIpm *st = c->ipm;
    st->d.stop_on = 0;
    int rc;
    if (st->frozen) { MWCHECK(hipMemsetAsync(st->d.flags + 6, 0, sizeof(int), c->stream)); st->frozen = false; }
    const int held = st->held_refine_bits;
    if ((rc = mw_ipm_enqueue(c))) return rc;
    mw_ipm_note_bits(c, held);
    if ((rc = mw_ipm_finish(c))) return rc;
    MWCHECK(hipEventSynchronize(st->ev[MwIpm::E_REC0 + (st->iter & 1)]));
    mw_ipm_read_record(st->h_rec + (size_t)(st->iter & 1) * MREC_COUNT, out);
    st->held_refine_bits = out->refine_bits;
    return 0;
}

static int mw_ipm_solve_body(clrs_mw_ctx *c, const clrs_ipm_stop *stop, clrs_ipm_record_fn on_record, void *user, clrs_ipm_record *records, int max_records, int *n_iter, int *error_code);
extern "C" int clrs_mw_ipm_solve_cb(clrs_mw_ctx *c, const clrs_ipm_stop *stop, clrs_ipm_record_fn on_record, void *user, clrs_ipm_record *records, int max_records,
                                    int *n_iter, int *error_code) {
    if (!c || !stop || !n_iter || !error_code || !c->ipm || !c->ipm->ready) return mw_fail(CLRS_ERR_STATE, "clrs_mw_ipm_create first");
    MWCHECK(hipSetDevice(c->device));
    const int rc = mw_ipm_solve_body(c, stop, on_record, user, records, max_records, n_iter, error_code);
    c->ipm->d.stop_on = 0;
    if (rc) c->ipm->frozen = true;
    return rc;
}
extern "C" int clrs_mw_ipm_solve(clrs_mw_ctx *c, const clrs_ipm_stop *stop, clrs_ipm_record *records, int max_records, int *n_iter, int *error_code) {
    return clrs_mw_ipm_solve_cb(c, stop, nullptr, nullptr, records, max_records, n_iter, error_code);
}
static int mw_ipm_solve_body(clrs_mw_ctx *c, const clrs_ipm_stop *stop, clrs_ipm_record_fn on_record, void *user, clrs_ipm_record *records, int max_records, int *n_iter,
                             int *error_code) {
    MwIpm *st = c->ipm;
    MwIpmDev &p = st->d;
    p.stop_on = 1; p.gap_thr = stop->duality_gap_threshold; p.need_dual = stop->need_dual_feasible; p.need_primal = stop->need_primal_feasible;
    MWCHECK(hipMemsetAsync(p.flags + 6, 0, sizeof(int), c->stream));
    st->frozen = false;
    *n_iter = 0; *error_code = 0;
    const int first = st->iter + 1, last = st->iter + stop->max_iterations;
    int rc, enq = st->iter;
    if (stop->max_iterations <= 0) { *error_code = 2; return 0; }
    mw_ipm_note_bits(c, st->held_refine_bits);
    st->held_refine_bits = 0;
    if ((rc = mw_ipm_enqueue(c))) return rc;
    enq = st->iter;
    for (int k = first;; k++) {
        if (k < last) { if ((rc = mw_ipm_enqueue(c))) return rc; enq = st->iter; }
        else if ((rc = mw_ipm_finish(c))) return rc;
        MWCHECK(hipEventSynchronize(st->ev[MwIpm::E_REC0 + (k & 1)]));
        clrs_ipm_record r;
        mw_ipm_read_record(st->h_rec + (size_t)(k & 1) * MREC_COUNT, &r);
        mw_ipm_note_bits(c, r.refine_bits);
        if (records && *n_iter < max_records) records[*n_iter] = r;
        (*n_iter)++;
        if (on_record) on_record(&r, user);
        const bool df = r.dual_error < p.dual_thr, pf = r.primal_error < p.primal_thr;
        bool done = r.error_code != 0 || (p.need_dual && df) || (p.need_primal && pf) || (!p.corrector_only && df && pf && r.gap < p.gap_thr);
        if (r.error_code != 0) *error_code = r.error_code;
        if (!done && k == last) { *error_code = 2; done = true; }
        if (done) break;
    }
    st->frozen = true;
    st->tail_pending = false;
    if ((rc = mw_ipm_drain(c))) return rc;
    st->iter = *n_iter + first - 1;
    (void)enq;
    p.stop_on = 0;
    return 0;
}

extern "C" int clrs_mw_ipm_set_global(clrs_mw_ctx *c, int rows_of_X_global, int clusters_global, const int32_t *cluster_ids, const int32_t *block_ids) {
    if (!c || !c->ipm || !c->ipm->ready) return mw_fail(CLRS_ERR_STATE, "clrs_mw_ipm_create first");
    if (rows_of_X_global <= 0 || clusters_global < c->d.J) return mw_fail(CLRS_ERR_INVALID, "bad global sizes");
    MWCHECK(hipSetDevice(c->device));
    MwIpm *st = c->ipm;
    MwIpmDev &p = st->d;
    const MwDev &q = c->d;
    int rc;
    p.Ktot = rows_of_X_global;
    p.Jglob = clusters_global;
    p.GL = MWG_LEN(c->K, q.N);
    if (st->gs_world != q.world) {
        if ((rc = mw_dmalloc(c, &p.gsM, (i64)q.world * p.GL)) || (rc = mw_dmalloc(c, &p.gsS, (i64)q.world * p.GL))) return rc;
        st->gs_world = q.world;
    }
    p.clu_gid = p.blk_gid = nullptr;
    if (cluster_ids) { std::vector<int> v(cluster_ids, cluster_ids + q.J); if ((rc = mw_upload(c, v, &p.clu_gid))) return rc; }
// ... 33 lines not shown
```

### clusteredlowranksolver.jl_amd/csrc/clrs_mw_tables.h

```cpp
#ifndef CLRS_MW_TABLES_H
#define CLRS_MW_TABLES_H

#include <algorithm>
#include <cmath>
#include <cstring>
#include <map>
#include <string>
#include <tuple>
#include <vector>

#include "../../include/clrs_hip.h"
#include "clrs_mw_slices.h"
#include "clrs_mw_types.h"

struct MwTables {
    int J = 0, N = 0, NB = 0, DK = 1;
    mwi64 T = 0, D = 0;
    mwi64 xlen = 0, Slen = 0, xylen = 0, xrdlen = 0;
    mwi64 zlen = 0, glen = 0, sdlen = 0, wlen = 0;
    mwi64 Vp = 1, dAp = 1, lamp = 1, Bp = 1;
    std::vector<MwBlk> blk;
    std::vector<MwClu> clu;
    std::vector<int> lr_list, dn_list;
    std::vector<double> V, dA, st_lam, B;
    std::vector<int> vrow, tptr, st_a, st_b, st_orig, st_p, st_war, st_wac, st_trl, st_trd, st_flag, ay_a, ay_b, ay_blk;
    std::vector<int> dmap, dense_p, drow_ptr, drow_blk, drow_en;
    int maxU = 0, maxP = 0, maxn = 0, maxn_dense = 0, maxTb = 0, maxcnt = 0, dn_big = 0;
    int sa_lanes = 1;
    int n_one_term = 0, n_many_term = 0;
    double cnt_mul = 0, cnt_factor = 0, cnt_solve = 0;
};

inline int mw_build_tables(const clrs_sdp_desc *d, int data_limbs, MwTables &o, std::string &err) {
    typedef mwi64 i64;
#define MWT_FAIL(msg) do { err = (msg); return CLRS_ERR_INVALID; } while (0)
    o = MwTables();
    const int DK = o.DK = data_limbs;
    const int J = o.J = d->n_clusters, N = o.N = d->n_free, NB = o.NB = d->n_blocks;
    if (J <= 0 || N < 0 || NB < 0) MWT_FAIL("bad sizes");
    o.clu.resize(J);
    i64 xlen = 0, Slen = 0;
    for (int j = 0; j < J; j++) {
        MwClu &q = o.clu[j];
        q.P = d->cluster_P[j];
        if (q.P <= 0) MWT_FAIL("cluster without constraints");
        q.coff = xlen; q.Soff = Slen; q.b0 = NB; q.b1 = 0;
        xlen += q.P; Slen += (i64)q.P * q.P;
        o.maxP = std::max(o.maxP, q.P);
    }
    o.xlen = xlen; o.Slen = Slen;
    o.blk.resize(NB);
    const i64 T = o.T = NB ? d->term_ptr[NB] : 0, D = o.D = NB ? d->dense_ptr[NB] : 0;
    const i64 vec_plane = T ? d->term_vec_ptr[T] : 0, dA_plane = D ? d->dense_A_ptr[D] : 0;
    const size_t T1 = (size_t)std::max<i64>(T, 1);
    o.st_a.resize(T1); o.st_b.resize(T1); o.ay_a.assign(T1, 0); o.ay_b.assign(T1, 0); o.ay_blk.assign(T1, -1);
    o.st_lam.resize(T1 * DK);
    o.st_orig.resize(T1); o.st_war.resize(T1); o.st_wac.resize(T1); o.st_trl.resize(T1); o.st_trd.resize(T1); o.st_flag.resize(T1); o.st_p.resize(T1);
    std::vector<std::tuple<i64, int, int>> drow_pairs;
    std::vector<std::vector<double>> hVl(DK), hdAl(DK);
    i64 xyoff = 0, rdoff = 0, zoff = 0, goff = 0, sdoff = 0, woff = 0;
    for (int b = 0; b < NB; b++) {
        MwBlk &k = o.blk[b];
        std::memset(&k, 0, sizeof(k));
        k.j = d->block_cluster[b];
        if (k.j < 0 || k.j >= J || (b > 0 && k.j < o.blk[b - 1].j)) MWT_FAIL("block_cluster must be non-decreasing and within range");
        const int m = d->block_m[b];
        k.delta = d->block_delta[b];
        k.n = m * k.delta;
        k.kind = d->block_kind[b];
        k.m = m;
        k.P = o.clu[k.j].P;
        if (k.n <= 0 || (k.kind != 0 && m != 1)) MWT_FAIL("bad block shape");
        k.xyoff = xyoff; xyoff += (i64)k.n * k.n;
        k.rd_off = rdoff; rdoff += k.n;
        o.clu[k.j].b0 = std::min(o.clu[k.j].b0, b);
        o.clu[k.j].b1 = std::max(o.clu[k.j].b1, b + 1);
        o.maxn = std::max(o.maxn, k.n);
        if (k.kind != 0) o.maxn_dense = std::max(o.maxn_dense, k.n);
        const int P = k.P, n = k.n, dl = k.delta;
        if (k.kind == 0) {
            o.lr_list.push_back(b);
            const i64 t0 = d->term_ptr[b], t1 = d->term_ptr[b + 1];
            k.t0 = t0;
            o.maxTb = std::max(o.maxTb, (int)(t1 - t0));
            std::vector<std::pair<int, const double *>> uniq;
            auto find_or_add = [&](int r, const double *v) -> int {
                for (size_t u = 0; u < uniq.size(); u++) {
                    if (uniq[u].first != r) continue;
                    bool eq = true;
                    for (int l = 0; l < DK && eq; l++)
                        for (int i = 0; i < dl && eq; i++) eq = uniq[u].second[(i64)l * vec_plane + i] == v[(i64)l * vec_plane + i];
                    if (eq) return (int)u;
                }
                uniq.push_back({r, v});
                return (int)uniq.size() - 1;
            };
            std::map<std::tuple<int, int, int, int>, i64> index;
            for (i64 t = t0; t < t1; t++) {
                if (d->term_p[t] < 0 || d->term_p[t] >= P || d->term_r[t] < 0 || d->term_r[t] >= m || d->term_s[t] < 0 || d->term_s[t] >= m)
                    MWT_FAIL("term index out of range");
                if (d->term_vec_ptr[t + 1] - d->term_vec_ptr[t] != dl) MWT_FAIL("term vectors must have delta entries");
                index[std::make_tuple(d->term_p[t], d->term_r[t], d->term_s[t], d->term_rank[t])] = t;
            }
            std::vector<int> Rt(t1 - t0), Ls(t1 - t0), Cs(t1 - t0), Ds(t1 - t0);
            std::vector<i64> partner(t1 - t0);
            for (i64 t = t0; t < t1; t++) {
                Rt[t - t0] = find_or_add(d->term_r[t], d->term_vs + d->term_vec_ptr[t]);
                Ls[t - t0] = find_or_add(d->term_r[t], d->term_ws + d->term_vec_ptr[t]);
                Cs[t - t0] = find_or_add(d->term_s[t], d->term_ws + d->term_vec_ptr[t]);
                Ds[t - t0] = find_or_add(d->term_s[t], d->term_vs + d->term_vec_ptr[t]);
                auto it = index.find(std::make_tuple(d->term_p[t], d->term_s[t], d->term_r[t], d->term_rank[t]));
                if (it == index.end()) MWT_FAIL("term without transposed partner: A[r,s][p] must equal A[s,r][p]^T");
                partner[t - t0] = it->second;
            }
            k.U = (int)uniq.size();
            o.maxU = std::max(o.maxU, k.U);
            k.v_off = (i64)hVl[0].size();
            k.vrow_off = (i64)o.vrow.size();
            for (int l = 0; l < DK; l++) hVl[l].resize(hVl[l].size() + (size_t)n * k.U, 0.0);
            for (int u = 0; u < k.U; u++) {
                o.vrow.push_back(uniq[u].first * dl);
                for (int l = 0; l < DK; l++)
                    for (int i = 0; i < dl; i++) hVl[l][k.v_off + (i64)u * n + uniq[u].first * dl + i] = uniq[u].second[(i64)l * vec_plane + i];
            }
            k.z_off = zoff; zoff += (i64)n * k.U;
            k.g_off = goff; goff += (i64)k.U * k.U;
            std::vector<i64> order(t1 - t0);
            for (i64 t = t0; t < t1; t++) order[t - t0] = t;
            std::stable_sort(order.begin(), order.end(), [&](i64 a, i64 b2) { return d->term_p[a] < d->term_p[b2]; });
            k.tptr_off = (i64)o.tptr.size();
            o.tptr.resize(o.tptr.size() + P + 1, 0);
            int *tp = o.tptr.data() + k.tptr_off;
            for (i64 i = 0; i < t1 - t0; i++) tp[d->term_p[order[i]] + 1]++;
            tp[0] = (int)t0;
            for (int p = 0; p < P; p++) tp[p + 1] += tp[p];
            for (i64 i = 0; i < t1 - t0; i++) {
                const i64 t = order[i];
                o.st_a[t0 + i] = Ls[partner[t - t0] - t0];
                o.st_b[t0 + i] = Rt[t - t0];
                for (int l = 0; l < DK; l++) o.st_lam[(size_t)l * T1 + t0 + i] = d->term_lambda[(i64)l * T + t];
                o.st_orig[t0 + i] = (int)t;
                o.st_p[t0 + i] = d->term_p[t];
                o.st_war[t0 + i] = Rt[t - t0]; o.st_wac[t0 + i] = Cs[t - t0];
                o.st_trl[t0 + i] = Ls[t - t0]; o.st_trd[t0 + i] = Ds[t - t0];
                o.st_flag[t0 + i] = (d->term_s[t] <= d->term_r[t] ? 1 : 0) | (d->term_s[t] != d->term_r[t] ? 2 : 0);
            }
            for (i64 t = t0; t < t1; t++) {
                o.ay_blk[t] = b;
                o.ay_a[t] = Ls[t - t0];
                o.ay_b[t] = Rt[partner[t - t0] - t0];
            }
            o.cnt_mul += (double)n * dl * k.U + 0.5 * (double)n * n * k.U + 0.5 * (double)k.U * k.U * (n + dl);
            for (int p = 0; p < P; p++)
                for (int q2 = p; q2 < P; q2++) o.cnt_mul += (double)(tp[p + 1] - tp[p]) * (tp[q2 + 1] - tp[q2]);
        } else {
            o.dn_list.push_back(b);
            const i64 d0 = d->dense_ptr[b], d1 = d->dense_ptr[b + 1];
            k.cnt = (int)(d1 - d0);
            k.d0 = d0;
            k.a_off = (i64)hdAl[0].size();
            k.dmap_off = (i64)o.dmap.size();
            o.dmap.resize(o.dmap.size() + P, -1);
            for (i64 e = d0; e < d1; e++) {
                const int p = d->dense_p[e];
                if (p < 0 || p >= P) MWT_FAIL("dense constraint index out of range");
                if (d->dense_A_ptr[e + 1] - d->dense_A_ptr[e] != (i64)n * n) MWT_FAIL("dense matrix must have n*n entries");
                for (int l = 0; l < DK; l++) {
                    const double *Ae = d->dense_A + (i64)l * dA_plane + d->dense_A_ptr[e];
                    for (int cc = 0; cc < n; cc++)
                        for (int rr = cc + 1; rr < n; rr++)
                            if (Ae[rr + (i64)cc * n] != Ae[cc + (i64)rr * n]) MWT_FAIL("dense constraint matrices must be symmetric");
                }
                o.dmap[k.dmap_off + p] = (int)(e - d0);
                drow_pairs.push_back(std::make_tuple(o.clu[k.j].coff + p, b, (int)(e - d0)));
                for (int l = 0; l < DK; l++)
                    hdAl[l].insert(hdAl[l].end(), d->dense_A + (i64)l * dA_plane + d->dense_A_ptr[e], d->dense_A + (i64)l * dA_plane + d->dense_A_ptr[e + 1]);
            }
            k.sd_off = sdoff; sdoff += (i64)k.cnt * k.cnt;
            k.w_off = woff; woff += (i64)k.cnt * n * n;
            o.cnt_mul += (double)k.cnt * (2.0 * n * n * n + 0.5 * (double)k.cnt * n * n);
            o.maxcnt = std::max(o.maxcnt, k.cnt);
            if (n > 1) o.dn_big = 1;
        }
    }
    o.xylen = xyoff; o.xrdlen = rdoff; o.zlen = zoff; o.glen = goff; o.sdlen = sdoff; o.wlen = woff;
    for (int j = 0; j < J; j++)
        if (o.clu[j].b0 > o.clu[j].b1) { o.clu[j].b0 = o.clu[j].b1 = 0; }
    {
        int mostb = 1;
        for (int j = 0; j < J; j++) mostb = std::max(mostb, o.clu[j].b1 - o.clu[j].b0);
        o.sa_lanes = mostb >= 3 ? 4 : mostb;
        for (int j = 0; j < J; j++) {
            MwClu &cl = o.clu[j];
            bool one = J >= 32 && cl.b1 - cl.b0 >= 1 && cl.b1 - cl.b0 <= 4;
            for (int b = cl.b0; b < cl.b1 && one; b++) {
                const MwBlk &k = o.blk[b];
                if (k.kind != 0) continue;
                const int *tp = o.tptr.data() + k.tptr_off;
                for (int p = 0; p < cl.P && one; p++) one = tp[p + 1] - tp[p] <= 1;
            }
            cl.one_term = one ? 1 : 0;
            (one ? o.n_one_term : o.n_many_term)++;
        }
    }
    for (int j = 0; j < J; j++) {
        const double P = o.clu[j].P;
        o.cnt_factor += P * P * P / 6.0 + 0.5 * P * P * N + 0.5 * P * (double)N * N;
        o.cnt_solve += P * P + 2.0 * P * N;
    }
    o.cnt_factor += (double)N * N * N / 6.0;
    o.cnt_solve += (double)N * N;
    o.Vp = std::max<i64>((i64)hVl[0].size(), 1); o.dAp = std::max<i64>((i64)hdAl[0].size(), 1); o.lamp = std::max<i64>(T, 1);
    o.V.assign((size_t)o.Vp * DK, 0.0);
    o.dA.assign((size_t)o.dAp * DK, 0.0);
    for (int l = 0; l < DK; l++) {
        std::copy(hVl[l].begin(), hVl[l].end(), o.V.begin() + (size_t)l * o.Vp);
        std::copy(hdAl[l].begin(), hdAl[l].end(), o.dA.begin() + (size_t)l * o.dAp);
    }
    o.dense_p.assign(d->dense_p, d->dense_p + D);
    std::sort(drow_pairs.begin(), drow_pairs.end());
    o.drow_ptr.assign((size_t)xlen + 1, 0);
    for (auto &t : drow_pairs) o.drow_ptr[(size_t)std::get<0>(t) + 1]++;
    for (i64 g = 0; g < xlen; g++) o.drow_ptr[(size_t)g + 1] += o.drow_ptr[(size_t)g];
    for (auto &t : drow_pairs) { o.drow_blk.push_back(std::get<1>(t)); o.drow_en.push_back(std::get<2>(t)); }
    const i64 Bp = xlen * (i64)N;
    o.Bp = std::max<i64>(Bp, 1);
    o.B.assign((size_t)o.Bp * DK, 0.0);
    for (int l = 0; l < DK; l++) {
        i64 off = 0;
        for (int j = 0; j < J; j++) {
            const int P = o.clu[j].P;
            for (int a = 0; a < N; a++)
                for (int r = 0; r < P; r++) o.B[(size_t)l * o.Bp + o.clu[j].coff + r + (i64)a * xlen] = d->B[(i64)l * Bp + off + r + (i64)a * P];
            off += (i64)P * N;
        }
    }
    return 0;
#undef MWT_FAIL
}

template <class PUT>
inline void mw_cut_digits(double x0, double x1, int e, int S, PUT &&put) {
    double r0 = std::ldexp(x0, -e), r1 = std::ldexp(x1, -e);
    for (int s = 0; s < S; s++) {
        const double g = std::ldexp(1.0, -(s + 1) * MWS_BETA), C = 0x1.8p52 * g;
        volatile double tv = r0 + C;
        const double t = tv - C;
        put(s, (float)(t * std::ldexp(1.0, (s + 1) * MWS_BETA)));
        r0 -= t;
        double sm, er;
        mwa::two_sum(r0, r1, sm, er);
        r0 = sm; r1 = er;
    }
}

#endif
```

Baseline: 2397 iterations/s.

## Compute corrector RHS via second-order low-rank update instead of full recompute

Adds a second-order corrector path. It precomputes U = Xinv·V per low-rank block, then forms DU = dX·U and DV = dY·V alongside the predictor dot kernel. The corrector right-hand side is built as the saved predictor RHS minus the low-rank bilinear correction terms, in a new fused rows+forward-solve kernel. This replaces the full mw_ipm_rhs and trace_rhs recomputation on the corrector stream. It adds the buffers U, DU, DV and rhs0 plus extra predictor-side work, and relies on the algebraic identity holding at multiword precision.

```diff
diff --git a/clusteredlowranksolver.jl_amd/csrc/clrs_hip.hip b/clusteredlowranksolver.jl_amd/csrc/clrs_hip.hip
--- a/clusteredlowranksolver.jl_amd/csrc/clrs_hip.hip
+++ b/clusteredlowranksolver.jl_amd/csrc/clrs_hip.hip
@@ -66,6 +66,7 @@
 int g_cfg_lrsys_chunk_bytes = 0;
 int g_cfg_mw_zi_narrow = 1;
 int g_cfg_mw_xinv_product = 1;
+int g_cfg_mw_corr_second_order = 1;
 int g_cfg_mw_chain_hop = 1;
 int g_cfg_mw_y_riders = 1;
 int g_cfg_mw_skip_xfb = 1;
@@ -1322,6 +1323,7 @@
     if (!std::strcmp(key, "liftm_chunk_bytes")) { g_cfg_liftm_chunk_bytes = value < 0 ? 0 : value; return 0; }
     if (!std::strcmp(key, "lrsys_chunk_bytes")) { g_cfg_lrsys_chunk_bytes = value < 0 ? 0 : value; return 0; }
     if (!std::strcmp(key, "mw_xinv_product")) { g_cfg_mw_xinv_product = value; return 0; }
+    if (!std::strcmp(key, "mw_corr_second_order")) { g_cfg_mw_corr_second_order = value; return 0; }
     if (!std::strcmp(key, "mw_chain_hop")) { g_cfg_mw_chain_hop = value; return 0; }
     if (!std::strcmp(key, "mw_skip_xfb")) { g_cfg_mw_skip_xfb = value; return 0; }
     if (!std::strcmp(key, "mw_y_riders")) { g_cfg_mw_y_riders = value; return 0; }
diff --git a/clusteredlowranksolver.jl_amd/csrc/clrs_mw.hip b/clusteredlowranksolver.jl_amd/csrc/clrs_mw.hip
--- a/clusteredlowranksolver.jl_amd/csrc/clrs_mw.hip
+++ b/clusteredlowranksolver.jl_amd/csrc/clrs_mw.hip
@@ -34,6 +34,7 @@
 
 extern int g_cfg_mw_zi_narrow;
 extern int g_cfg_mw_xinv_product;
+extern int g_cfg_mw_corr_second_order;
 extern int g_cfg_mw_chain_hop, g_cfg_mw_skip_xfb, g_cfg_mw_y_riders;
 extern int g_cfg_mw_stream_words;
 extern int g_cfg_mw_pipeline64;
@@ -180,6 +181,8 @@
     const double *ride_y = nullptr;
     bool zi_narrow = true;
     bool xinv_product = true;
+    bool corr_second_order = true;
+    std::vector<int> st_same;
     int chain_hop = 1;
     bool refine_skip_next = false;
     int refine_predictor = 0;
@@ -493,6 +496,7 @@
     MW_RET(mw_upload(c, t.tptr, &q.tptr));
     MW_RET(mw_upload(c, t.st_orig, &q.st_orig)); MW_RET(mw_upload(c, t.st_p, &q.st_p)); MW_RET(mw_upload(c, t.st_war, &q.st_war)); MW_RET(mw_upload(c, t.st_wac, &q.st_wac));
     MW_RET(mw_upload(c, t.st_trl, &q.st_trl)); MW_RET(mw_upload(c, t.st_trd, &q.st_trd)); MW_RET(mw_upload(c, t.st_flag, &q.st_flag));
+    c->st_same = t.st_same;
     MW_RET(mw_upload(c, t.ay_a, &q.ay_a)); MW_RET(mw_upload(c, t.ay_b, &q.ay_b)); MW_RET(mw_upload(c, t.ay_blk, &q.ay_blk));
     MW_RET(mw_upload(c, t.dA, &q.dA)); MW_RET(mw_upload(c, t.dmap, &q.dmap)); MW_RET(mw_upload(c, t.dense_p, &q.dense_p));
     MW_RET(mw_upload(c, t.drow_ptr, &q.drow_ptr)); MW_RET(mw_upload(c, t.drow_blk, &q.drow_blk)); MW_RET(mw_upload(c, t.drow_en, &q.drow_en));
@@ -650,6 +654,7 @@
         c->y_riders = g_cfg_mw_y_riders != 0;
         c->zi_narrow = g_cfg_mw_zi_narrow != 0;
         c->xinv_product = g_cfg_mw_xinv_product != 0;
+        c->corr_second_order = g_cfg_mw_corr_second_order != 0;
     }
     MW_RET(mw_stage_stream(c));
     MwTables t;
diff --git a/clusteredlowranksolver.jl_amd/csrc/clrs_mw_inst.h b/clusteredlowranksolver.jl_amd/csrc/clrs_mw_inst.h
--- a/clusteredlowranksolver.jl_amd/csrc/clrs_mw_inst.h
+++ b/clusteredlowranksolver.jl_amd/csrc/clrs_mw_inst.h
@@ -64,6 +64,10 @@
     X __global__ void k_mwi_rows_dn<K, DK>(const MwDev, const MwIpmDev, int);                                          \
     X __global__ void k_mwi_rows<K, DK>(const MwDev, const MwIpmDev, int, int);                                        \
     X __global__ void k_mwi_rows_fwd<K, DK>(const MwDev, const MwIpmDev);                                              \
+    X __global__ void k_mwi_dots_so<K, DK>(const MwDev, const MwIpmDev, const MwSoDev, int, int, int);                 \
+    X __global__ void k_mwi_UV<K, DK>(const MwDev, const double *, double *);                                          \
+    X __global__ void k_mwi_rows_so<K, DK>(const MwDev, const MwIpmDev, const MwSoDev);                                \
+    X __global__ void k_mwi_rows_fwd_so<K, DK>(const MwDev, const MwIpmDev, const MwSoDev);                            \
     X __global__ void k_mwi_pv<K, DK>(const MwDev, const MwIpmDev, int);                                               \
     X __global__ void k_mwi_pvfin<K, DK>(const MwDev, const MwIpmDev);                                                 \
     X __global__ void k_mwi_gpack<K, DK>(const MwDev, const MwIpmDev, int);                                               \
diff --git a/clusteredlowranksolver.jl_amd/csrc/clrs_mw_ipm.hip.h b/clusteredlowranksolver.jl_amd/csrc/clrs_mw_ipm.hip.h
--- a/clusteredlowranksolver.jl_amd/csrc/clrs_mw_ipm.hip.h
+++ b/clusteredlowranksolver.jl_amd/csrc/clrs_mw_ipm.hip.h
@@ -38,6 +38,12 @@
     int GL, Jglob;
     const int *clu_gid, *blk_gid;
 };
+struct MwSoDev {
+    double *U;
+    double *DU, *DV;
+    double *rhs0;
+    const int *st_same;
+};
 #define MWG_S1(K, N) 0
 #define MWG_S2(K, N) (K)
 #define MWG_BX(K, N) (2 * (K))
@@ -600,6 +606,53 @@
     mwi_dots_body<K, K, DK>(q, p, sel);
 }
 
+template <int K, int DK, int EW, bool FULL>
+__device__ __forceinline__ void mwi_MV_body(const MwDev &q, const MwBlk &k, const double *__restrict__ M, const double *__restrict__ W, double *__restrict__ out, int bx) {
+    using namespace mwk;
+    const int n = k.n, dl = k.delta;
+    if (bx * (MW_NT / EW) >= n * k.U) return;
+    const int e = bx * (MW_NT / EW) + threadIdx.x / EW, sub = threadIdx.x % EW;
+    const bool live = e < n * k.U;
+    const int ee = live ? e : 0, i = ee % n, c = ee / n;
+    acc<K> s;
+    acc_zero<K>(s);
+    if constexpr (FULL) {
+        for (int kk = sub; kk < n; kk += EW) acc_fma<K, K, K>(s, ldx<K>(M + k.xyoff, q.xylen, i + (long)kk * n), ldx<K>(W + k.z_off, q.zlen, kk + (long)c * n));
+    } else {
+        const double *V = q.V + k.v_off;
+        const int r0 = q.vrow[k.vrow_off + c];
+        for (int kk = r0 + sub; kk < r0 + dl; kk += EW) acc_fma<K, K, DK>(s, ldx<K>(M + k.xyoff, q.xylen, i + (long)kk * n), ldx<DK>(V, q.Vp, kk + (long)c * n));
+    }
+    const mw<K> v = lanes_sum<K, EW>(acc_result<K>(s));
+    if (live && sub == 0) stx<K>(out + k.z_off, q.zlen, e, v);
+}
+template <int K, int DK, int EW>
+__device__ __forceinline__ void mwi_DUDV_body(const MwDev &q, const MwIpmDev &p, const MwSoDev &o, int w, int uv_tiles) {
+    const int per = uv_tiles * q.nlr, rem = w % per;
+    const MwBlk &k = q.blk[q.lr_list[rem / uv_tiles]];
+    if (w < per) mwi_MV_body<K, DK, EW, true>(q, k, p.dX, o.U, o.DU, rem % uv_tiles);
+    else mwi_MV_body<K, DK, EW, false>(q, k, p.dY, nullptr, o.DV, rem % uv_tiles);
+}
+template <int K, int DK>
+__global__ __launch_bounds__(MW_NT) void k_mwi_dots_so(const MwDev q, const MwIpmDev p, const MwSoDev o, int sel, int r_tiles, int uv_tiles) {
+    using namespace mwk;
+    if ((int)blockIdx.x >= q.NB) {
+        const int w = blockIdx.x - q.NB, nr = (r_tiles < 0 ? -r_tiles : r_tiles) * q.NB;
+        if (w >= nr) {
+            if (r_tiles < 0) mwi_DUDV_body<K, DK, 16>(q, p, o, w - nr, uv_tiles);
+            else mwi_DUDV_body<K, DK, MWI_EW>(q, p, o, w - nr, uv_tiles);
+        } else if (r_tiles < 0) mwi_R_body<K, 16>(q, p, 1, w % (-r_tiles), w / (-r_tiles));
+        else mwi_R_body<K, MWI_EW>(q, p, 1, w % r_tiles, w / r_tiles);
+        return;
+    }
+    if constexpr (mw_kf_of(K) < K) { if (p.klow < K) { mwi_dots_body<K, mw_kf_of(K), DK>(q, p, sel); return; } }
+    mwi_dots_body<K, K, DK>(q, p, sel);
+}
+template <int K, int DK>
+__global__ __launch_bounds__(MW_NT) void k_mwi_UV(const MwDev q, const double *__restrict__ M, double *__restrict__ out) {
+    mwi_MV_body<K, DK, MWI_EW, false>(q, q.blk[q.lr_list[blockIdx.y]], M, nullptr, out, blockIdx.x);
+}
+
 
 template <int K, int DK>
 __global__ __launch_bounds__(MW_NT) void k_mwi_coef(const MwDev q, const MwIpmDev p, const double *__restrict__ a) {
@@ -743,9 +796,10 @@
 }
 
 #define MWI_RW 8
-template <int K, int DK, int BG>
-__device__ __forceinline__ void mwi_rows_body(const MwDev &q, const MwIpmDev &p, int mode, mwi64 g0, bool live) {
-    using namespace mwk;
+template <int K, int DK, int BG, bool SO = false>
+__device__ __forceinline__ void mwi_rows_body(const MwDev &q, const MwIpmDev &p, int mode, mwi64 g0, bool live, const MwSoDev *o = nullptr) {
+    using namespace mwk;
+    const bool so2 = SO && mode == 2;
     constexpr int RWT = MWI_RW * BG;
     const int sub = threadIdx.x % MWI_RW, grp = (threadIdx.x % RWT) / MWI_RW, sub_all = threadIdx.x % RWT;
     const mwi64 g = live ? g0 : 0;
@@ -771,6 +825,23 @@
                     acc_fma<K, K, DK>(s, ldx<K>(q.AY, q.T, q.st_orig[t]), w, -1.0);
                     if (with_tau) acc_fma<K, K, DK>(st, ldx<K>(q.AX, q.T, q.st_orig[t]), w);
                 }
+            } else if (so2) {
+                if constexpr (SO) {
+                    for (int t = tp[pp]; t < tp[pp + 1]; t++) {
+                        const int fl = q.st_flag[t];
+                        if (!(fl & 1)) continue;
+                        const bool same = o->st_same[t] != 0;
+                        const mw<DK> w = mul_pow2<DK>(ldx<DK>(q.st_lam, q.lamp, t), ((fl & 2) ? 2.0 : 1.0) * (same ? 1.0 : 0.5));
+                        const long lo = (long)q.st_trl[t] * n, dco = (long)q.st_trd[t] * n;
+                        acc<K> z;
+                        acc_zero<K>(z);
+                        for (int ii = sub; ii < n; ii += MWI_RW) {
+                            acc_fma<K, K, K>(z, ldx<K>(o->DU + k.z_off, q.zlen, ii + lo), ldx<K>(o->DV + k.z_off, q.zlen, ii + dco));
+                            if (!same) acc_fma<K, K, K>(z, ldx<K>(o->DU + k.z_off, q.zlen, ii + dco), ldx<K>(o->DV + k.z_off, q.zlen, ii + lo));
+                        }
+                        acc_fma<K, K, DK>(s, acc_result<K>(z), w, -1.0);
+                    }
+                }
             } else {
                 const double *V = q.V + k.v_off;
                 for (int t = tp[pp]; t < tp[pp + 1]; t++) {
@@ -786,7 +857,12 @@
             }
         } else if (!q.dn_big) {
             const int en = q.dmap[k.dmap_off + pp];
-            if (en >= 0) {
+            if (en >= 0 && so2) {
+                if (sub == 0) {
+                    const mw<K> xdx = mul<K>(ldx<K>(p.Xv + k.xyoff, q.xylen, 0), ldx<K>(p.dX + k.xyoff, q.xylen, 0));
+                    acc_fma<K, K, DK>(s, mul<K>(xdx, ldx<K>(p.dY + k.xyoff, q.xylen, 0)), ldx<DK>(q.dA, q.dAp, k.a_off + en), -1.0);
+                }
+            } else if (en >= 0) {
                 const long nn = (long)n * n;
                 for (long i = sub; i < nn; i += MWI_RW) acc_fma<K, K, DK>(s, ldx<K>(M + k.xyoff, q.xylen, i), ldx<DK>(q.dA, q.dAp, k.a_off + en * nn + i), -1.0);
                 if (with_tau && sub == 0) {
@@ -794,6 +870,14 @@
                     acc_fma<K, K, DK>(st, mul<K>(xi, xi), ldx<DK>(q.dA, q.dAp, k.a_off + en * nn));
                 }
             }
+        }
+    }
+    if constexpr (SO) {
+        if (so2) {
+            if (sub_all == 0) acc_add<K, K>(s, ldx<K>(o->rhs0, q.xlen, g));
+            const mw<K> r = lanes_sum<K, RWT>(acc_result<K>(s));
+            if (live && sub_all == 0) stx<K>(p.rhsx, q.xlen, g, r);
+            return;
         }
     }
     if (q.dn_big && sub_all == 0) acc_add<K, K>(s, ldx<K>(p.dtr, q.xlen, g), -1.0);
@@ -813,6 +897,11 @@
         if (sub_all == 0) acc_add<K, K>(s, ldx<K>(p.d, q.xlen, g), -1.0);
         const mw<K> r = lanes_sum<K, RWT>(acc_result<K>(s));
         if (live && sub_all == 0) stx<K>(p.rhsx, q.xlen, g, r);
+        if constexpr (SO) {
+            if (sub_all == 0) acc_fma<K, K, K>(s, ldx<K>(p.sc, MSC_COUNT, MSC_MUS), ldx<K>(p.tau, q.xlen, g), -1.0);
+            const mw<K> r0 = lanes_sum<K, RWT>(acc_result<K>(s));
+            if (live && sub_all == 0) stx<K>(o->rhs0, q.xlen, g, r0);
+        }
     }
 }
 template <int K, int DK>
@@ -826,6 +915,23 @@
     for (int r0 = 0; r0 < c.P; r0 += MW_NT / MWI_RW) {
         const int r = r0 + threadIdx.x / MWI_RW;
         mwi_rows_body<K, DK, 1>(q, p, 1, c.coff + r, r < c.P);
+    }
+    __threadfence_block();
+    __syncthreads();
+    mw_solve_fwd_cluster<K>(q, blockIdx.x, p.rhsx);
+}
+template <int K, int DK>
+__global__ __launch_bounds__(MW_NT) void k_mwi_rows_so(const MwDev q, const MwIpmDev p, const MwSoDev o) {
+    const mwi64 g0 = (mwi64)blockIdx.x * (MW_NT / MWI_RW) + threadIdx.x / MWI_RW;
+    mwi_rows_body<K, DK, 1, true>(q, p, 1, g0, g0 < q.xlen, &o);
+}
+template <int K, int DK>
+__global__ __launch_bounds__(MW_NT) void k_mwi_rows_fwd_so(const MwDev q, const MwIpmDev p, const MwSoDev o) {
+    mw_mark(q);
+    const MwClu &c = q.clu[blockIdx.x];
+    for (int r0 = 0; r0 < c.P; r0 += MW_NT / MWI_RW) {
+        const int r = r0 + threadIdx.x / MWI_RW;
+        mwi_rows_body<K, DK, 1, true>(q, p, 2, c.coff + r, r < c.P, &o);
     }
     __threadfence_block();
     __syncthreads();
diff --git a/clusteredlowranksolver.jl_amd/csrc/clrs_mw_ipm_host.inc b/clusteredlowranksolver.jl_amd/csrc/clrs_mw_ipm_host.inc
--- a/clusteredlowranksolver.jl_amd/csrc/clrs_mw_ipm_host.inc
+++ b/clusteredlowranksolver.jl_amd/csrc/clrs_mw_ipm_host.inc
@@ -12,6 +12,8 @@
     int held_refine_bits = 0;
     bool aff_ok = false;
     double *AX = nullptr;
+    bool so_ok = false;
+    MwSoDev so = {};
     int kf_now = 0;
     double *h_rec = nullptr;
     double *d_rec = nullptr;
@@ -142,6 +144,7 @@
         MW_DISPATCH(c, {
             if ((rc = mw_set_lds(k_mwi_Zi<KK>, st->sm_Zi))) return rc;
             if ((rc = mw_set_lds((k_mwi_rows_fwd<KK, DD>), c->sm_fwd))) return rc;
+            if ((rc = mw_set_lds((k_mwi_rows_fwd_so<KK, DD>), c->sm_fwd))) return rc;
             if ((rc = mw_set_lds(k_mwi_bmm<KK>, st->sm_bmm))) return rc;
             if ((rc = mw_set_lds(k_mwi_Z<KK>, st->sm_Z))) return rc;
             if ((rc = mw_set_lds((k_mwi_step<KK, DD>), st->sm_step))) return rc;
@@ -154,6 +157,12 @@
             if (st->aff_ok) {
                 if ((rc = mw_dmalloc(c, &st->AX, q.T * K)) || (rc = mw_dmalloc(c, &p.tau, q.xlen * K)) || (rc = mw_dmalloc(c, &p.ttau, q.xlen * K)) ||
                     (rc = mw_dmalloc(c, &p.utau, (i64)q.J * N * K))) return rc;
+            }
+            st->so_ok = st->aff_ok && p.Xv != nullptr && q.world <= 1 && c->corr_second_order && !c->wide_solve && mostb < 16 && q.J <= 64 && !q.dn_big;
+            if (st->so_ok) {
+                if ((rc = mw_upload(c, c->st_same, &st->so.st_same))) return rc;
+                if ((rc = mw_dmalloc(c, &st->so.U, q.zlen * K)) || (rc = mw_dmalloc(c, &st->so.DU, q.zlen * K)) || (rc = mw_dmalloc(c, &st->so.DV, q.zlen * K)) ||
+                    (rc = mw_dmalloc(c, &st->so.rhs0, q.xlen * K))) return rc;
             }
         }
         p.beta_infeasible = 0.3; p.beta_feasible = 0.1; p.gamma = 0.9; p.dual_thr = 1e-30; p.primal_thr = 1e-30;
@@ -397,6 +406,8 @@
     st->d.rec = st->d_rec + (size_t)(st->iter & 1) * MREC_COUNT;
     const bool aff = st->aff_ok && !q.gathered;
     c->d.AX = aff ? st->AX : nullptr;
+    const bool so = aff && st->so_ok;
+    const MwSoDev &o = st->so;
     c->d.skip_y = y_rides ? 1 : 0;
     rc = clrs_mw_schur_assemble_dev(c, p.Xc, p.Y);
     c->d.skip_y = 0;
@@ -428,6 +439,10 @@
         const int xv_tiles = ((int)(st->maxn_inv * st->maxn_inv) * MWI_ZL + MW_NT - 1) / MW_NT;
         MW_DISPATCH(c, hipLaunchKernelGGL(k_mwi_Xv<KK>, dim3(xv_tiles, q.NB), dim3(MW_NT), 0, S, q, p));
         MWCHECK(hipGetLastError());
+        if (so && q.nlr) {
+            MW_DISPATCH(c, hipLaunchKernelGGL((k_mwi_UV<KK, DD>), dim3((c->maxn * c->maxU * MWI_EW + MW_NT - 1) / MW_NT, q.nlr), dim3(MW_NT), 0, S, q, (const double *)p.Xv, o.U));
+            MWCHECK(hipGetLastError());
+        }
     }
     if ((rc = mw_ipm_rhs(c, S, 0))) return rc;
     if ((rc = mw_ipm_trace_rhs(c, S))) return rc;
@@ -452,7 +467,10 @@
         if (q.dn_big) hipLaunchKernelGGL((k_mwi_rows_dn<KK, DD>), dim3((unsigned)((q.xlen + MW_NT / 64 - 1) / (MW_NT / 64))), dim3(MW_NT), 0, S, q, p, 1);
     });
     MWCHECK(hipGetLastError());
-    if ((rc = mw_ipm_rows(c, S, 1))) return rc;
+    if (so) {
+        MW_DISPATCH(c, hipLaunchKernelGGL((k_mwi_rows_so<KK, DD>), dim3((unsigned)((q.xlen * MWI_RW + MW_NT - 1) / MW_NT)), dim3(MW_NT), 0, S, q, p, o));
+        MWCHECK(hipGetLastError());
+    } else if ((rc = mw_ipm_rows(c, S, 1))) return rc;
     const bool word_sync = words && split_factor && !c->wide_solve && (c->lds_q || c->pipe_Q);
     if (word_sync) hipLaunchKernelGGL(k_mwi_mark<0>, dim3(1), dim3(1), 0, S, p.sync, seq);
     else {
@@ -478,11 +496,28 @@
     if (rc) { st->d.klow = c->K; return rc; }
     const bool r16 = (i64)maxnn * 16 * q.NB <= 65536;
     const int r_tiles = (maxnn * (r16 ? 16 : MWI_EW) + MW_NT - 1) / MW_NT;
+    if (so) {
+        const int uv_tiles = (c->maxn * c->maxU * (r16 ? 16 : MWI_EW) + MW_NT - 1) / MW_NT;
+        MW_DISPATCH(c, hipLaunchKernelGGL((k_mwi_dots_so<KK, DD>), dim3(q.NB + r_tiles * q.NB + 2 * q.nlr * uv_tiles), dim3(MW_NT), sm_red, M, q, p, o, 2, r16 ? -r_tiles : r_tiles, uv_tiles));
+    } else
     MW_DISPATCH(c, hipLaunchKernelGGL((k_mwi_dots<KK, DD>), dim3(q.NB + r_tiles * q.NB), dim3(MW_NT), sm_red, M, q, p, 2, r16 ? -r_tiles : r_tiles));
     st->d.klow = c->K;
     if ((rc = mw_ipm_exchange(c, M, 2))) return rc;
     const bool aff_async = aff && word_sync;
-    if (aff_async) {
+    if (so) {
+        if (aff_async) { c->d.mark_word = p.sync + 3; c->d.mark_value = seq; }
+        else MW_DISPATCH(c, hipLaunchKernelGGL((k_mwi_scalar<KK, DD>), dim3(1), dim3(1), 0, M, q, p, 2, st->iter));
+        MW_DISPATCH(c, hipLaunchKernelGGL((k_mwi_rows_fwd_so<KK, DD>), dim3(q.J), dim3(MW_NT), c->sm_fwd, M, q, p, o));
+        c->d.mark_word = nullptr;
+        MWCHECK(hipGetLastError());
+        c->fwd_rode = true;
+        if (aff_async) {
+            hipLaunchKernelGGL(k_mwi_wait<0>, dim3(1), dim3(64), 0, S, (const int *)(p.sync + 3), seq, q.info, q.J + 1);
+            MW_DISPATCH(c, hipLaunchKernelGGL((k_mwi_scalar<KK, DD>), dim3(1), dim3(1), 0, S, q, p, 2, st->iter));
+            hipLaunchKernelGGL(k_mwi_mark<0>, dim3(1), dim3(1), 0, S, p.sync + 4, seq);
+            MWCHECK(hipGetLastError());
+        }
+    } else if (aff_async) {
         c->d.mark_word = p.sync + 3; c->d.mark_value = seq;
         rc = mw_ipm_rhs(c, M, 2);
         c->d.mark_word = nullptr;
@@ -496,8 +531,8 @@
         MWCHECK(hipGetLastError());
         if ((rc = mw_ipm_rhs(c, M, aff ? 2 : 0))) return rc;
     }
-    if ((rc = mw_ipm_trace_rhs(c, M))) return rc;
-    {
+    if (!so && (rc = mw_ipm_trace_rhs(c, M))) return rc;
+    if (!so) {
         int mostb = 1;
         for (int j = 0; j < q.J; j++) mostb = std::max(mostb, c->clu[j].b1 - c->clu[j].b0);
         if (!c->wide_solve && mostb < 16 && q.J <= 64) {
diff --git a/clusteredlowranksolver.jl_amd/csrc/clrs_mw_tables.h b/clusteredlowranksolver.jl_amd/csrc/clrs_mw_tables.h
--- a/clusteredlowranksolver.jl_amd/csrc/clrs_mw_tables.h
+++ b/clusteredlowranksolver.jl_amd/csrc/clrs_mw_tables.h
@@ -24,6 +24,7 @@
     std::vector<int> lr_list, dn_list;
     std::vector<double> V, dA, st_lam, B;
     std::vector<int> vrow, tptr, st_a, st_b, st_orig, st_p, st_war, st_wac, st_trl, st_trd, st_flag, ay_a, ay_b, ay_blk;
+    std::vector<int> st_same;
     std::vector<int> dmap, dense_p, drow_ptr, drow_blk, drow_en;
     int maxU = 0, maxP = 0, maxn = 0, maxn_dense = 0, maxTb = 0, maxcnt = 0, dn_big = 0;
     int sa_lanes = 1;
@@ -56,6 +57,7 @@
     o.st_a.resize(T1); o.st_b.resize(T1); o.ay_a.assign(T1, 0); o.ay_b.assign(T1, 0); o.ay_blk.assign(T1, -1);
     o.st_lam.resize(T1 * DK);
     o.st_orig.resize(T1); o.st_war.resize(T1); o.st_wac.resize(T1); o.st_trl.resize(T1); o.st_trd.resize(T1); o.st_flag.resize(T1); o.st_p.resize(T1);
+    o.st_same.assign(T1, 0);
     std::vector<std::tuple<i64, int, int>> drow_pairs;
     std::vector<std::vector<double>> hVl(DK), hdAl(DK);
     i64 xyoff = 0, rdoff = 0, zoff = 0, goff = 0, sdoff = 0, woff = 0;
@@ -144,6 +146,7 @@
                 o.st_war[t0 + i] = Rt[t - t0]; o.st_wac[t0 + i] = Cs[t - t0];
                 o.st_trl[t0 + i] = Ls[t - t0]; o.st_trd[t0 + i] = Ds[t - t0];
                 o.st_flag[t0 + i] = (d->term_s[t] <= d->term_r[t] ? 1 : 0) | (d->term_s[t] != d->term_r[t] ? 2 : 0);
+                o.st_same[t0 + i] = Ls[t - t0] == Ds[t - t0] ? 1 : 0;
             }
             for (i64 t = t0; t < t1; t++) {
                 o.ay_blk[t] = b;
```

Result: faster. 2665 iterations/s (median of 6 runs) (+11.2%).
